# plumer/pbrs

Hardware: AMD Instinct MI355X
Metric: Msamples/s (higher is better)
Workload: dtype f32

## Files before the change

include/pbrs_gpu.h:

```cpp
#ifndef PBRS_GPU_H
#define PBRS_GPU_H

#include <stdint.h>

#ifdef __cplusplus
extern "C" {
#endif

#define PBRS_OK 0
#define PBRS_E_INVALID (-1)
#define PBRS_E_DEVICE (-2)
#define PBRS_E_NO_SCENE (-3)
#define PBRS_E_LIMIT (-4)

#define PBRS_LEAF_FLAG 0x80000000u
#define PBRS_TLAS_LEAF_KIND_SHIFT 8

typedef struct pbrs_node {
    float min[3];
    uint32_t a;
    float max[3];
    uint32_t b;
} pbrs_node;

// ... 97 lines not shown
} pbrs_area_light;

typedef struct pbrs_delta_light {
    uint32_t kind;
    float v[3];
    float color[3];
    float world_radius;
} pbrs_delta_light;

typedef struct pbrs_scene_desc {
    uint32_t n_tlas_nodes;
    const pbrs_node* tlas_nodes;
    uint32_t tlas_height;
    uint32_t n_instances;
    const pbrs_instance* instances;
    uint32_t n_shapes;
    const pbrs_shape* shapes;
    uint32_t n_meshes;
    const pbrs_mesh* meshes;
    uint32_t n_blas_nodes;
    const pbrs_node* blas_nodes;
    uint32_t n_triangles;
    const pbrs_tri_verts* tri_verts;
    const pbrs_tri_shade* tri_shade;
    uint32_t n_materials;
    const pbrs_material* materials;
    uint32_t n_bxdfs;
    const pbrs_bxdf* bxdfs;
    uint32_t n_area_lights;
    const pbrs_area_light* area_lights;
    uint32_t n_delta_lights;
    const pbrs_delta_light* delta_lights;
    float env_constant[3];
    uint32_t env_kind;
    uint32_t n_textures;
    const pbrs_texture* textures;
    uint32_t n_tex_floats;
    const float* tex_floats;
    uint32_t n_tex_words;
    const uint32_t* tex_words;
    uint32_t env_texture;
    float env_scale[3];
    uint32_t n_fourier_tables;
    const pbrs_fourier_table* fourier_tables;
} pbrs_scene_desc;

typedef struct pbrs_camera {
    float center[3];
    uint32_t width;
    float c[3];
    uint32_t height;
    float a[3];
    float pad0;
    float b[3];
    float pad1;
} pbrs_camera;

typedef struct pbrs_stats {
    uint64_t samples;
    uint64_t closest_rays;
    uint64_t shadow_rays;
    uint64_t shade_events;
    uint64_t tlas_nodes, blas_nodes, instances, instance_hits, triangles, tri_shading;
    uint64_t spheres, quads, cuboids, disks;
    uint64_t shadow_tlas_nodes, shadow_blas_nodes, shadow_instances, shadow_triangles, shadow_prims;
    uint64_t invalid_samples;
    float ms_raygen, ms_extend, ms_shade, ms_shadow, ms_accumulate, ms_total;
    uint32_t launches_extend, launches_shadow, launches_shade, passes;
    uint32_t kernel_features_extend, kernel_features_shadow;
    uint64_t paths_at_bounce[16];
    uint64_t shadow_rays_at_bounce[16];
} pbrs_stats;
#define PBRS_STATS_MAX_BOUNCES 16

typedef struct pbrs_ctx pbrs_ctx;

int pbrs_create(int device_ordinal, pbrs_ctx** out);
void pbrs_destroy(pbrs_ctx*);
const char* pbrs_last_error(const pbrs_ctx*);
int pbrs_set_stream(pbrs_ctx*, void* hip_stream);

int pbrs_set_pass_overlap(pbrs_ctx*, int enabled);

int pbrs_upload_scene(pbrs_ctx*, const pbrs_scene_desc*);

typedef struct pbrs_render_params {
    uint32_t x0, y0, w, h;
    uint32_t strata_x, strata_y;
    uint32_t max_depth;
    uint32_t samples_per_pass;
    uint64_t seed;
    uint32_t collect_counters;
    uint32_t time_stages;
    uint32_t band_rows, band_count, band_index;
    uint32_t integrator;
} pbrs_render_params;
#define PBRS_INTEGRATOR_PATH 0u
#define PBRS_INTEGRATOR_DIRECT 1u
#define PBRS_INTEGRATOR_MATERIALS 2u
#define PBRS_INTEGRATOR_NORMALS 3u

int pbrs_render_tile(pbrs_ctx*, const pbrs_camera*, const pbrs_render_params*, float* rgb_out_host, pbrs_stats* stats_out);
int pbrs_render_tile_device(pbrs_ctx*, const pbrs_camera*, const pbrs_render_params*, float* rgb_out_device, pbrs_stats* stats_out);
int pbrs_collect_stats(pbrs_ctx*, pbrs_stats* stats_out);

typedef struct pbrs_aov_buffers {
    float* albedo;
    float* normal;
    float* coverage;
    float* depth;
    uint32_t* instance;
    uint32_t* material;
    uint32_t* prim;
} pbrs_aov_buffers;
int pbrs_render_tile_aovs(pbrs_ctx*, const pbrs_camera*, const pbrs_render_params*, float* rgb_out_host, const pbrs_aov_buffers* aovs_host,
                          pbrs_stats* stats_out);
int pbrs_render_tile_aovs_device(pbrs_ctx*, const pbrs_camera*, const pbrs_render_params*, float* rgb_out_device,
                                 const pbrs_aov_buffers* aovs_device, pbrs_stats* stats_out);

enum pbrs_filter_kind { PBRS_FILTER_BOX = 0, PBRS_FILTER_TRIANGLE = 1, PBRS_FILTER_GAUSSIAN = 2, PBRS_FILTER_MITCHELL = 3, PBRS_FILTER_LANCZOS = 4 };
#define PBRS_FILTER_MAX_RADIUS 4.0f
typedef struct pbrs_pixel_filter {
    uint32_t kind;
    float radius[2];
    float a, b;
    uint32_t pad;
} pbrs_pixel_filter;
int pbrs_render_tile_filtered(pbrs_ctx*, const pbrs_camera*, const pbrs_render_params*, const pbrs_pixel_filter*, float* rgb_out_host,
                              pbrs_stats* stats_out);
int pbrs_render_tile_filtered_device(pbrs_ctx*, const pbrs_camera*, const pbrs_render_params*, const pbrs_pixel_filter*,
                                     float* rgb_out_device, pbrs_stats* stats_out);

#define PBRS_DENOISE_MAX_ITERATIONS 6
#define PBRS_DENOISE_DEMODULATE 1u
#define PBRS_DENOISE_ID_STOP 2u
typedef struct pbrs_denoise_params {
    uint32_t w, h;
    uint32_t iterations;
    uint32_t flags;
    float sigma_color, sigma_normal, sigma_depth;
    float albedo_floor;
} pbrs_denoise_params;
typedef struct pbrs_denoise_guides {
    const float* albedo;
    const float* normal;
    const float* depth;
    const uint32_t* instance;
} pbrs_denoise_guides;
int pbrs_denoise(pbrs_ctx*, const pbrs_denoise_params*, const float* rgb_in_host, const pbrs_denoise_guides* guides_host, float* rgb_out_host);
int pbrs_denoise_device(pbrs_ctx*, const pbrs_denoise_params*, const float* rgb_in_device, const pbrs_denoise_guides* guides_device,
                        float* rgb_out_device);

typedef struct pbrs_hit_record {
    float t;
    uint32_t inst;
    uint32_t prim;
    float b1, b2;
} pbrs_hit_record;
int pbrs_intersect_rays(pbrs_ctx*, uint32_t n, const float* origins, const float* dirs, const float* tmax,
                        pbrs_hit_record* hits_out, uint8_t* occluded_out);
typedef struct pbrs_intersect_info {
    uint32_t wide_any, wide_closest;
    uint32_t slow_any, slow_closest;
} pbrs_intersect_info;
int pbrs_last_intersect_info(const pbrs_ctx*, pbrs_intersect_info* out);
int pbrs_camera_rays(pbrs_ctx*, const pbrs_camera*, const pbrs_render_params*, uint32_t sample_index, float* origins_out,
// ... 344 lines not shown
```

pbrs_amd/api.py:

```python
import ctypes as C
import os
from types import SimpleNamespace

import numpy as np

from .abi import (AOV_NAMES, AOVS, BSDF_OPS, BSDF_QUERY_WORDS, BSDF_RESULT_WORDS, DENOISE_GUIDES, HIT_DTYPE, INTEGRATORS, MATTE_LAYERS, NUMERIC_FNS, NUMERIC_K_FNS, PASS_CHANNELS, PASSES,
                  SPATIAL_VARIANCE_PLANES, TEMPORAL_FRAME, TEMPORAL_GUIDES, TEMPORAL_HISTORY, VARIANCE, AovBuffers, BloomParams, Camera, CompareMaps, CompareParams, CompareResult,
                  DenoiseGuides, DenoiseParams, DespeckleIO, DespeckleParams, DespeckleResult, DofParams,
                  DenoiseVarGuides, DenoiseVarParams, DisplayIO, DisplayParams, HistoryClipParams, InstanceMotion, MatteBuffers, MatteParams, MotionBlurParams, Node, PassBuffers,
                  PixelFilter, RenderParams, SceneDesc, SpatialVarianceGuides, SpatialVarianceParams, Stats, TemporalFrame, TemporalGuides, TemporalHistory,
                  TemporalParams, UpsampleParams, _aov_names, _bloom_params, _DenoiseParamsMixin, _despeckle_params, _display_params, _dof_params, _history_clip, _matte_select, _motion_args, _motion_blur_params, _pass_names,
                  _reference_frame, _reference_frames, _temporal_struct, _upscale_params, lens, scaled_camera)
from .devmem import DeviceBuffers
from .libs import GPU_BLOOM_SYMBOLS, GPU_COMPARE_SYMBOLS, GPU_DESPECKLE_SYMBOLS, GPU_DOF_SYMBOLS, GPU_MOTION_BLUR_SYMBOLS, GPU_SYMBOLS, HOST_SYMBOLS, PbrsError, gpu_lib, hip_runtime, host_lib, lib_paths
from .spec import SceneSpec


def orbited(camera, about, axis, degrees):
    k = np.asarray(axis, dtype=np.float64)
    k = k / np.linalg.norm(k)
    t = np.radians(degrees)

    def rot(v):
        return v * np.cos(t) + np.cross(k, v) * np.sin(t) + k * np.dot(k, v) * (1.0 - np.cos(t))
    about = np.asarray(about, dtype=np.float64)
    out = Camera()
    out.width, out.height = camera.width, camera.height
    out.center[:] = [float(v) for v in about + rot(np.array(list(camera.center), dtype=np.float64) - about)]
    for n in ("c", "a", "b"):
        getattr(out, n)[:] = [float(v) for v in rot(np.array(list(getattr(camera, n)), dtype=np.float64))]
    return out


def instance_motion(scene, scene_prev):
    fwd, inv = scene.instance_transforms()
    fwd_p, inv_p = scene_prev.instance_transforms()
    if len(fwd) != len(fwd_p):
        raise ValueError(f"instance_motion: {len(fwd)} instances beside {len(fwd_p)} in the previous scene")
    table = (InstanceMotion * max(len(fwd), 1))()
    bottom = np.array([[0.0, 0.0, 0.0, 1.0]])
    for i in range(len(fwd)):
        r = table[i]
        if fwd[i].tobytes() == fwd_p[i].tobytes() and inv[i].tobytes() == inv_p[i].tobytes():
            m, n, r.flags = np.eye(3, 4), np.eye(3), InstanceMotion.IDENTITY
        else:
            m = (np.vstack([fwd_p[i].astype(np.float64), bottom]) @ np.vstack([inv[i].astype(np.float64), bottom]))[:3]
            n = (fwd[i, :, :3].astype(np.float64) @ inv_p[i, :, :3].astype(np.float64)).T
        for a in range(3):
            r.m[a][:] = [float(v) for v in m[a].astype(np.float32)]
            r.n[a][:] = [float(v) for v in n[a].astype(np.float32)]
    return table


def _guide_bytes(guides, w, h, suffix=""):
    return {n + suffix: DENOISE_GUIDES[n][0] * w * h * 4 for n in guides}


def _sequence_buffers(w, h, fw, fh, guides, motion_vectors, upscale, display, reference=False, despeckle=False, bloom=False, dof=False,
                      motion_blur=False):
    kept = [n for n in TEMPORAL_GUIDES if n in guides]
    sizes = {"rgb": 3 * w * h * 4, "out": 3 * w * h * 4, VARIANCE: w * h * 4, "acc_variance": w * h * 4}
    for k in ("0", "1"):
        sizes.update(_guide_bytes(kept, w, h, k))
        sizes.update({f"h_{n}{k}": ch * w * h * 4 for n, (ch, _) in TEMPORAL_HISTORY.items()})
    sizes.update(_guide_bytes([n for n in guides if n not in kept], w, h))
    if motion_vectors:
        sizes["motion"], sizes["prev_depth"] = 2 * w * h * 4, w * h * 4
    if upscale:
        sizes["up"] = 3 * fw * fh * 4
        sizes.update(_guide_bytes(guides, fw, fh, "_hi"))
    if display:
        sizes["display"], sizes["exposure"] = fw * fh * 4, 4
    if reference:
        sizes["reference"], sizes["compare"] = 3 * fw * fh * 4, C.sizeof(CompareResult)
    if despeckle:
        sizes["despeckled"], sizes["despeckle"] = 3 * w * h * 4, C.sizeof(DespeckleResult)
    if bloom:
        sizes["bloom"] = 3 * fw * fh * 4
    if dof:
        sizes["dof"] = 3 * fw * fh * 4
    if motion_blur:
        sizes["mblur"] = 3 * fw * fh * 4
        if upscale or not motion_vectors:
            sizes["mblur_motion"] = 2 * fw * fh * 4
    return sizes


class LoadedScene:

    def __init__(self, path):
        h = C.c_void_p()
        rc = host_lib().pbrs_host_load_pbrt(os.fsencode(path), C.byref(h))
        if rc != 0:
            raise PbrsError(f"pbrs_host_load_pbrt({path}) failed ({rc}): {host_lib().pbrs_host_load_error().decode()}")
        self._h = h
        self.spec = host_lib().pbrs_loaded_scene_spec(h).contents

# ... 37 lines not shown
    if ch == 3:
        img = np.concatenate([img, np.full((h, w, 1), 255, dtype=np.uint8)], axis=2)
    words = np.ascontiguousarray(img).view("<u4")
    rc = host_lib().pbrs_host_write_png_rgba8(os.fsencode(path), words.ctypes.data, w, h)
    if rc != 0:
        raise PbrsError(f"writing {path} failed ({rc}): {host_lib().pbrs_host_io_error().decode()}")


class HostScene:

    def __init__(self, scene_builder):
        self._sb = scene_builder
        self._spec = scene_builder.build()
        h = C.c_void_p()
        rc = host_lib().pbrs_host_scene_build(C.addressof(self._spec), C.byref(h))
        if rc != 0:
            raise PbrsError(f"pbrs_host_scene_build failed ({rc}): {host_lib().pbrs_host_last_error().decode()}")
        self._h = h
        self.desc = host_lib().pbrs_host_scene_desc(h).contents
        self.camera = host_lib().pbrs_host_scene_camera(h).contents
        self.width, self.height = self.camera.width, self.camera.height

    @property
    def stack_depth(self):
        return host_lib().pbrs_host_scene_stack_depth(self._h)

    @property
    def nbytes(self):
        d = self.desc
        return (32 * (d.n_tlas_nodes + d.n_blas_nodes) + 128 * d.n_instances + 48 * d.n_shapes + 32 * d.n_meshes +
                (48 + 64) * d.n_triangles + 32 * d.n_materials + 64 * d.n_bxdfs + 64 * d.n_area_lights + 32 * d.n_delta_lights +
                48 * d.n_textures + 4 * (d.n_tex_floats + d.n_tex_words) + 48 * d.n_fourier_tables)

    def instance_transforms(self):
        n = self.desc.n_instances
        if n == 0 or not self.desc.instances:
            return np.zeros((0, 3, 4), dtype=np.float32), np.zeros((0, 3, 4), dtype=np.float32)
        rec = np.ctypeslib.as_array(C.cast(self.desc.instances, C.POINTER(C.c_float)), shape=(n, 32))
        return rec[:, 12:24].reshape(n, 3, 4).copy(), rec[:, :12].reshape(n, 3, 4).copy()

    def nodes(self, which="tlas"):
        n, p = (self.desc.n_tlas_nodes, self.desc.tlas_nodes) if which == "tlas" else (self.desc.n_blas_nodes, self.desc.blas_nodes)
        if n == 0 or not p:
            return np.zeros((0, 8), dtype=np.uint32)
        return np.ctypeslib.as_array(C.cast(p, C.POINTER(C.c_uint32)), shape=(n, 8)).copy()

    def close(self):
        if getattr(self, "_h", None):
            host_lib().pbrs_host_scene_free(self._h)
            self._h = None

    def __del__(self):
        self.close()


class Context:

    def __init__(self, device=0):
        self._L = gpu_lib()
        h = C.c_void_p()
        rc = self._L.pbrs_create(device, C.byref(h))
        if rc != 0:
            raise PbrsError(f"pbrs_create(device={device}) failed ({rc}): no usable HIP device; there is no CPU fallback")
        self._h = h
        self.scene = None

    def _check(self, rc, what):
        if rc != 0:
            raise PbrsError(f"{what} failed ({rc}): {self._L.pbrs_last_error(self._h).decode()}")

    def close(self):
        if getattr(self, "_h", None):
            self._L.pbrs_destroy(self._h)
            self._h = None

    def __del__(self):
        self.close()

    def set_stream(self, hip_stream_ptr):
        self._check(self._L.pbrs_set_stream(self._h, C.c_void_p(hip_stream_ptr)), "pbrs_set_stream")

    def set_pass_overlap(self, enabled):
        self._check(self._L.pbrs_set_pass_overlap(self._h, int(bool(enabled))), "pbrs_set_pass_overlap")

    def upload(self, host_scene):
        self._check(self._L.pbrs_upload_scene(self._h, C.addressof(host_scene.desc)), "pbrs_upload_scene")
        self.scene = host_scene

    def _params(self, strata_x, strata_y, depth, seed, tile, samples_per_pass=0, counters=False, timing=False, bands=None,
                integrator="path"):
        x0, y0, w, h = tile or (0, 0, self.scene.width, self.scene.height)
        p = RenderParams()
        if bands:
            p.band_rows, p.band_count, p.band_index = bands
        p.x0, p.y0, p.w, p.h = x0, y0, w, h
        p.strata_x, p.strata_y, p.max_depth, p.samples_per_pass = strata_x, strata_y, depth, samples_per_pass
        p.seed, p.collect_counters, p.time_stages = seed, int(counters), int(timing)
        p.integrator = INTEGRATORS[integrator]
        return p

    def render(self, strata_x, strata_y, depth, seed, tile=None, samples_per_pass=0, counters=False, timing=False, bands=None,
               integrator="path"):
        p = self._params(strata_x, strata_y, depth, seed, tile, samples_per_pass, counters, timing, bands, integrator)
        out = np.empty((p.h, p.w, 3), dtype=np.float32)
        st = Stats()
        self._check(self._L.pbrs_render_tile(self._h, C.addressof(self.scene.camera), C.addressof(p), out.ctypes.data, C.addressof(st)),
                    "pbrs_render_tile")
        return out, st.as_dict()

    def render_device(self, rgb_device_ptr, strata_x, strata_y, depth, seed, tile=None, samples_per_pass=0, counters=False,
                      timing=False, bands=None, integrator="path"):
        p = self._params(strata_x, strata_y, depth, seed, tile, samples_per_pass, counters, timing, bands, integrator)
        self._check(self._L.pbrs_render_tile_device(self._h, C.addressof(self.scene.camera), C.addressof(p), C.c_void_p(rgb_device_ptr), None),
                    "pbrs_render_tile_device")

    @staticmethod
    def _aov_arrays(names, p):
        bufs, arrays = AovBuffers(), {}
        for n in names:
            ch, dt = AOVS.get(n, (1, np.float32))
            arrays[n] = np.empty((p.h, p.w, ch) if ch > 1 else (p.h, p.w), dtype=dt)
            if n != VARIANCE:
                setattr(bufs, n, arrays[n].ctypes.data)
        return bufs, arrays

    @staticmethod
    def _aov_device(aov_device_ptrs):
        ptrs = dict(aov_device_ptrs or {})
        _aov_names(ptrs)
        variance = ptrs.pop(VARIANCE, None)
        bufs = AovBuffers()
        for n, ptr in ptrs.items():
            setattr(bufs, n, ptr)
        return bufs, variance

    def _render_host(self, p, names, mp=None, mb=None, pb=None, camera=None):
        out = np.empty((p.h, p.w, 3), dtype=np.float32)
        bufs, arrays = self._aov_arrays(names, p)
        st = Stats()
        self._check(self._L.pbrs_render_tile_passes(self._h, C.addressof(camera or self.scene.camera), C.addressof(p), out.ctypes.data, C.addressof(bufs),
                                                    arrays[VARIANCE].ctypes.data if VARIANCE in names else None, C.addressof(mp) if mp else None,
                                                    C.addressof(mb) if mb else None, C.addressof(pb) if pb else None, C.addressof(st)),
                    "pbrs_render_tile_passes")
        return out, arrays, st.as_dict()

    def _render_device(self, p, rgb_device_ptr, bufs, variance, mp=None, mb=None, pb=None, camera=None):
        self._check(self._L.pbrs_render_tile_passes_device(self._h, C.addressof(camera or self.scene.camera), C.addressof(p), C.c_void_p(rgb_device_ptr),
                                                           C.addressof(bufs), C.c_void_p(variance), C.addressof(mp) if mp else None,
                                                           C.addressof(mb) if mb else None, C.addressof(pb) if pb else None, None),
                    "pbrs_render_tile_passes_device")

    def render_aovs(self, strata_x, strata_y, depth, seed, aovs=AOV_NAMES, tile=None, samples_per_pass=0, counters=False,
                    timing=False, bands=None, integrator="path", camera=None):
        names = _aov_names(aovs)
        return self._render_host(self._params(strata_x, strata_y, depth, seed, tile, samples_per_pass, counters, timing, bands, integrator), names,
                                 camera=camera)

    def render_aovs_device(self, rgb_device_ptr, aov_device_ptrs, strata_x, strata_y, depth, seed, tile=None, samples_per_pass=0,
                           counters=False, timing=False, bands=None, integrator="path"):
        bufs, variance = self._aov_device(aov_device_ptrs)
        self._render_device(self._params(strata_x, strata_y, depth, seed, tile, samples_per_pass, counters, timing, bands, integrator),
                            rgb_device_ptr, bufs, variance)

    def render_aovs_var_device(self, rgb_device_ptr, aov_device_ptrs, variance_device_ptr, strata_x, strata_y, depth, seed, tile=None,
                               samples_per_pass=0, counters=False, timing=False, bands=None, integrator="path"):
        unknown = [n for n in aov_device_ptrs if n not in AOVS]
# ... 780 lines not shown
```

pbrs_amd/csrc/device/extend.h:

```cpp
#pragma once
#include "path_state.h"
#include "traverse.h"

template <bool STATS>
PD void flush_counters(const Cnt<STATS>& cnt, GlobalCounters* g, bool valid, uint32_t rays, uint32_t hits) {
    if (!STATS) return;
    const WorkCounters& c = cnt.c;
    uint32_t v[12] = {c.tlas_nodes, c.blas_nodes, c.instances, c.instance_hits, c.triangles, c.tri_shading,
                      c.spheres,    c.quads,      c.cuboids,   c.disks,         rays,        hits};
    unsigned long long* out = reinterpret_cast<unsigned long long*>(g);
    for (int k = 0; k < 12; ++k) {
        uint32_t x = valid ? v[k] : 0u;
        for (int off = 32; off > 0; off >>= 1) x += __shfl_down(x, off, 64);
        if ((threadIdx.x & 63u) == 0 && x) atomicAdd(out + k, (unsigned long long)x);
    }
}

#ifndef PBRS_NODE_STEPS_LONG
#define PBRS_NODE_STEPS_LONG 3u
#endif
#ifndef PBRS_CHUNK_MAX
#define PBRS_CHUNK_MAX 512u
#endif
#ifndef PBRS_TRAV_WAVES
// ... 76 lines not shown
    const uint32_t want = (uint32_t)__popcll(mask), rank = lane_prefix(mask);
    const uint32_t avail = w.end - w.cur;
    uint32_t idx = (need && rank < avail) ? w.cur + rank : 0xffffffffu;
    if (want <= avail) {
        w.cur += want;
        return idx;
    }
    w.cur = w.end;
    const int leader = __ffsll((unsigned long long)mask) - 1;
    while (w.tried < PBRS_WORK_HEADS) {
        const uint32_t seg_lo = work_segment(n, w.head), seg_hi = work_segment(n, w.head + 1);
        uint32_t base = 0;
        if ((int)(threadIdx.x & 63u) == leader) base = atomicAdd(heads + w.head * PBRS_WORK_HEAD_STRIDE, w.chunk);
        base = __shfl(base, leader, 64);
        const uint32_t len = seg_hi - seg_lo;
        const uint32_t lo = seg_lo + (base < len ? base : len), hi = seg_lo + (base + w.chunk < len ? base + w.chunk : len);
        if (base + w.chunk >= len) {
            w.head = (w.head + 1u) % PBRS_WORK_HEADS;
            w.tried++;
        }
        if (lo == hi) continue;
        const uint32_t rest = want - avail, got = hi - lo;
        if (need && rank >= avail && rank - avail < got) idx = lo + (rank - avail);
        w.cur = lo + (rest < got ? rest : got);
        w.end = hi;
        break;
    }
    return idx;
}
PD void wave_append_slow(bool slow, uint32_t item, uint32_t* list, uint32_t* count) {
    const uint64_t m = __ballot(slow);
    if (m == 0) return;
    const int leader = __ffsll((unsigned long long)m) - 1;
    uint32_t base = 0;
    if ((int)(threadIdx.x & 63u) == leader) base = atomicAdd(count, (uint32_t)__popcll(m));
    base = __shfl(base, leader, 64);
    if (slow) list[base + lane_prefix(m)] = item;
}
#ifndef PBRS_WIDE_SHADOW_WAVES
#define PBRS_WIDE_SHADOW_WAVES 5
#endif
#ifndef PBRS_WIDE_NODE_STEPS
#define PBRS_WIDE_NODE_STEPS 2u
#endif
template <uint32_t ARITY, bool STATS, uint32_t FEAT>
struct AnySel {
    typedef AnyWalkW<FEAT> type;
};
template <bool STATS, uint32_t FEAT>
struct AnySel<0u, STATS, FEAT> {
    typedef AnyWalk<STATS, (FEAT & (PBRS_FEAT_ALL | PBRS_FEAT_LDS_TOP)), !STATS && !(FEAT & PBRS_FEAT_FLAT_TLAS)> type;
};
#define PBRS_WALK_ARITY(STATS, FEAT) ((STATS) ? 0u : ((FEAT) & PBRS_FEAT_WIDE) ? 4u : 0u)
#ifndef PBRS_NODE_STEPS_SHORT
#define PBRS_NODE_STEPS_SHORT 1u
#endif
#define PBRS_WALK_NSTEPS(FEAT, ARITY) \
    (!((FEAT) & PBRS_FEAT_LONG_WALKS) ? ((ARITY) == 0u ? PBRS_NODE_STEPS_SHORT : 1u) : (ARITY) == 4u ? PBRS_WIDE_NODE_STEPS : PBRS_NODE_STEPS_LONG)
PD DevScene stage_scene(const DevScene& G, uint32_t* lds_base) {
    DevScene S = G;
    uint4* dst = reinterpret_cast<uint4*>(__builtin_assume_aligned(lds_base + G.lds_off_words, 16));
    S.nodes = reinterpret_cast<const pbrs_node*>(dst);
    dst = stage_array(dst, G.nodes, G.lds_nodes * (uint32_t)(sizeof(pbrs_node) / 16));
    S.tv = reinterpret_cast<const pbrs_tri_verts*>(dst);
    dst = stage_array(dst, G.tv, G.lds_tris * (uint32_t)(sizeof(pbrs_tri_verts) / 16));
    S.inst = reinterpret_cast<const pbrs_instance*>(dst);
    dst = stage_array(dst, G.inst, G.lds_inst * (uint32_t)(sizeof(pbrs_instance) / 16));
    S.shapes = reinterpret_cast<const pbrs_shape*>(dst);
    stage_array(dst, G.shapes, G.lds_shapes * (uint32_t)(sizeof(pbrs_shape) / 16));
    __syncthreads();
    return S;
}
static_assert(sizeof(pbrs_node) % 16 == 0 && sizeof(pbrs_tri_verts) % 16 == 0 && sizeof(pbrs_instance) % 16 == 0 && sizeof(pbrs_shape) % 16 == 0, "stage_scene copies 16-byte pieces");

PD DevScene stage_top(const DevScene& G, uint32_t* lds_base) {
    DevScene S = G;
    uint4* dst = reinterpret_cast<uint4*>(__builtin_assume_aligned(lds_base + G.lds_off_words, 16));
    S.nodes_top = reinterpret_cast<const pbrs_node*>(dst);
    stage_array(dst, G.nodes, G.lds_nodes * (uint32_t)(sizeof(pbrs_node) / 16));
    __syncthreads();
    return S;
}

template <bool STATS, uint32_t FEAT>
__global__ void __launch_bounds__(256, STATS ? 3 : (FEAT & PBRS_FEAT_SHADING_CHECK) ? PBRS_TRAV_WAVES : PBRS_LEAN_EXTEND_WAVES)
    k_extend(DevScene G, PathState st, uint32_t set, const uint32_t* count, uint32_t n_direct, uint32_t* next, GlobalCounters* gc, const uint32_t* indirect,
             uint32_t* slow_list, uint32_t* slow_count, uint32_t split) {
    extern __shared__ __attribute__((aligned(16))) uint32_t lds_stack[];
    const DevScene S = (!STATS && (FEAT & PBRS_FEAT_LDS_SCENE)) ? stage_scene(G, lds_stack) : (!STATS && (FEAT & PBRS_FEAT_LDS_TOP)) ? stage_top(G, lds_stack) : G;
    const uint32_t n = count ? *count : n_direct;
    const float4* q0 = st.q[set][0];
    const float4* q1 = st.q[set][1];
    LaneStack stk{lds_stack + threadIdx.x, q0, q1, 0u};
    Cnt<STATS> cnt;
    cnt.init();
    uint32_t nrays = 0, nhit = 0;
    ClosestWalk<STATS, (FEAT & (PBRS_FEAT_ALL | PBRS_FEAT_LDS_TOP | PBRS_FEAT_EXTENT))> walk;
    walk.mode = PBRS_WALK_IDLE;
    PBRS_KP_DECL(walk);
    PBRS_TT_DECL;
    uint32_t item = 0;
    WaveWork work = wave_work_init(n);
    for (;;) {
        uint64_t live = __ballot(walk.mode == PBRS_WALK_NODE || walk.mode == PBRS_WALK_LEAF || walk.mode == PBRS_WALK_XFER);
        if ((uint32_t)__popcll(live) < S.refill_below) {
            PBRS_KP_WAVE(1);
            if (walk.mode == PBRS_WALK_DONE) {
                walk.finish(cnt);
                const Hit& h = walk.best;
                nhit += h.inst != 0xffffffffu ? 1u : 0u;
                uint32_t cls = (S.n_classes > 1u && h.inst != 0xffffffffu) ? S.inst[h.inst].pad[0] : 0u;
                if (split) {
                    cls = 1u;
                    if (h.inst == 0xffffffffu) {
                        const bool specular = (item >> 31) != 0u;
                        cls = (specular || ((split & PBRS_QSPLIT_ENV) && S.has_env != 0u)) ? 1u : 0u;
                    }
                }
                const uint32_t pos = item & 0x7fffffffu;
                if (!split || cls) st_stream(&st.hit[pos], make_float4(h.t, __uint_as_float(h.inst), __uint_as_float(h.prim), __uint_as_float(split ? 0u : cls)));
                if (S.n_classes > 1u || split) st.cls[pos] = (uint8_t)cls;
                walk.mode = PBRS_WALK_IDLE;
            }
            if (work.left()) {
                uint32_t idx = wave_fetch(work, walk.mode == PBRS_WALK_IDLE, next, n);
                if (idx != 0xffffffffu) {
                    if (indirect) idx = indirect[idx];
                    stk.item = idx;
                    const float4 a = q0[idx], b = q1[idx];
                    item = idx | (__float_as_uint(a.w) & 0x80000000u);
                    walk.start(S, xyz(a), xyz(b), pn_inf(), stk);
                    nrays++;
                    PBRS_KP_LANE(2, true);
                }
                walk.scan_wave(S, cnt);
                live = __ballot(walk.mode == PBRS_WALK_NODE || walk.mode == PBRS_WALK_LEAF || walk.mode == PBRS_WALK_XFER);
            }
            if (live == 0) break;
        }
        PBRS_TT(0);
        PBRS_STEP_WALK(walk, S, stk, cnt, PBRS_EXT_XFER_MIN, PBRS_EXT_LEAF_MIN, PBRS_WALK_NSTEPS(FEAT, 0u), ((FEAT & PBRS_FEAT_FULL_STEPS) != 0u));
    }
    flush_counters<STATS>(cnt, gc, true, nrays, nhit);
    if (!STATS) PBRS_KP_FLUSH(0, walk);
    if (!STATS) PBRS_TT_FLUSH(0);
}
```

pbrs_amd/csrc/device/path_state.h:

```cpp
#pragma once
#include "shapes.h"

struct PathState {
    float4* q[2][3];
    float4* hit;
    uint8_t* cls;
    uint32_t* perm;
    uint32_t* tile_hist;
    uint2* class_range;
    float4* L;
    float4* sr[3];
    float4* nee[3];
    uint8_t* occ[2];
};

struct RenderConst {
    pbrs_camera cam;
    uint32_t x0, y0, w, h;
    uint32_t strata_x, strata_y;
    uint32_t max_depth;
    uint32_t pass_first_sample;
    uint32_t n_pixels;
    uint32_t n_slots;
    uint32_t chunk_pixels;
    uint32_t tiles8_per_row;
    uint32_t band_rows, band_count, band_index;
    uint32_t integrator;
    uint64_t seed;
};

template <class T>
PD T& at(T* base, uint32_t slot) {
    static_assert(sizeof(T) == 4 || sizeof(T) == 1, "column element size");
    return *reinterpret_cast<T*>(reinterpret_cast<char*>(base) + (size_t)(uint32_t)(slot * (uint32_t)sizeof(T)));
}
PD float4 pack4(f3 v, uint32_t w) { return make_float4(v.x, v.y, v.z, __uint_as_float(w)); }
PD float4 pack4(f3 v, float w) { return make_float4(v.x, v.y, v.z, w); }
PD f3 xyz(float4 v) { return mk3(v.x, v.y, v.z); }
#define PBRS_SLOT_MASK 0x3fffffffu
PD float4 ld_stream(const float4* p) {
    const pbrs_f4v v = __builtin_nontemporal_load(reinterpret_cast<const pbrs_f4v*>(p));
    return make_float4(v.x, v.y, v.z, v.w);
}
PD void st_stream(float4* p, float4 v) {
    pbrs_f4v w;
    w.x = v.x, w.y = v.y, w.z = v.z, w.w = v.w;
    __builtin_nontemporal_store(w, reinterpret_cast<pbrs_f4v*>(p));
}

PD void sample_of_slot(uint32_t slot, uint32_t n_pixels, uint32_t k_count, uint32_t chunk, uint32_t& k, uint32_t& pix) {
    const uint32_t per_chunk = chunk * k_count;
    const uint32_t c = slot / per_chunk, rem = slot - c * per_chunk, first = c * chunk;
    const uint32_t size = n_pixels - first < chunk ? n_pixels - first : chunk;
    k = rem / size;
    pix = first + (rem - k * size);
}
PD uint32_t slot_of_sample(uint32_t k, uint32_t pix, uint32_t n_pixels, uint32_t k_count, uint32_t chunk) {
    const uint32_t c = pix / chunk, first = c * chunk;
    const uint32_t size = n_pixels - first < chunk ? n_pixels - first : chunk;
    return c * chunk * k_count + k * size + (pix - first);
}

PD uint32_t pixel_of_order(uint32_t q, uint32_t w, uint32_t tiles8_per_row) {
    if (tiles8_per_row == 0u) return q;
    const uint32_t t = q >> 6, r = q & 63u;
    const uint32_t ty = t / tiles8_per_row, tx = t - ty * tiles8_per_row;
    return (ty * 8u + (r >> 3)) * w + tx * 8u + (r & 7u);
}
PD uint32_t order_of_pixel(uint32_t pix, uint32_t w, uint32_t tiles8_per_row) {
    if (tiles8_per_row == 0u) return pix;
    const uint32_t y = pix / w, x = pix - y * w;
    return (((y >> 3) * tiles8_per_row + (x >> 3)) << 6) + ((y & 7u) << 3) + (x & 7u);
}

struct GlobalCounters {
    unsigned long long tlas_nodes, blas_nodes, instances, instance_hits, triangles, tri_shading, spheres, quads, cuboids, disks, rays, hits;
};

PD uint4* stage_array(uint4* dst, const void* src_, uint32_t n16) {
    const uint4* src = reinterpret_cast<const uint4*>(src_);
    for (uint32_t i = threadIdx.x; i < n16; i += PBRS_TRAVERSAL_BLOCK) dst[i] = src[i];
    return dst + n16;
}
```

pbrs_amd/csrc/device/raygen.h:

```cpp
#pragma once
#include "path_state.h"

__global__ void __launch_bounds__(256) k_raygen(PathState st, RenderConst rc, uint32_t* rng_hi0) {
    uint32_t slot = blockIdx.x * blockDim.x + threadIdx.x;
    if (slot >= rc.n_slots) return;
    uint32_t k, pix;
    sample_of_slot(slot, rc.n_pixels, rc.n_slots / rc.n_pixels, rc.chunk_pixels, k, pix);
    pix = pixel_of_order(pix, rc.w, rc.tiles8_per_row);
    uint32_t col = rc.x0 + pix % rc.w, vrow = pix / rc.w;
    uint32_t row = rc.y0 + (rc.band_count > 1 ? ((vrow / rc.band_rows) * rc.band_count + rc.band_index) * rc.band_rows + vrow % rc.band_rows : vrow);
    uint32_t i = rc.pass_first_sample + k;
    uint64_t rng = pn_rng_init(rc.seed, row * rc.cam.width + col, i);
    float r0 = pn_rng_f32(&rng), r1 = pn_rng_f32(&rng);
    float jx = ((float)(i / rc.strata_y) + r0) / (float)rc.strata_x;
    float jy = ((float)(i % rc.strata_y) + r1) / (float)rc.strata_y;
    if (rc.integrator >= PBRS_INTEGRATOR_MATERIALS) jx = jy = 0.0f;
    float x = (float)col + pn_fract(jx);
    float y = (float)row + pn_fract(jy);
    f3 dir = ld3(rc.cam.c) + ld3(rc.cam.a) * x + ld3(rc.cam.b) * y;
    st_stream(&st.q[0][0][slot], pack4(ld3(rc.cam.center), slot));
    st_stream(&st.q[0][1][slot], pack4(dir, (uint32_t)rng));
    __builtin_nontemporal_store((uint32_t)(rng >> 32), &rng_hi0[slot]);
}
```

pbrs_amd/csrc/device/scene.h:

```cpp
#pragma once
#include <stddef.h>
#include <stdint.h>

#include "../../../include/pbrs_gpu.h"

constexpr uint32_t kBlock = 256;
constexpr size_t kLdsBytesPerCU = 160 * 1024;

struct pbrs_wnode;
struct DevScene {
    const pbrs_node* nodes;
    const pbrs_instance* inst;
    const pbrs_shape* shapes;
    const pbrs_mesh* meshes;
    const pbrs_tri_verts* tv;
    const pbrs_tri_shade* ts;
    const pbrs_material* mats;
    const pbrs_bxdf* bxdfs;
    const pbrs_area_light* alights;
    const pbrs_delta_light* dlights;
    uint32_t n_area, n_delta;
    float env[3];
    uint32_t has_env;
    uint32_t fast_slab;
    uint32_t exact_extent;
    uint32_t flat_off, n_flat;
    uint32_t features;
    uint32_t refill_below;
    uint32_t refill_below_shadow;
    const pbrs_texture* textures;
    const float* tex_floats;
    const uint32_t* tex_words;
    uint32_t env_kind, env_texture;
    float env_scale[3];
    const pbrs_fourier_table* fourier;
    uint32_t n_classes;
    const pbrs_wnode* wnodes;
    uint32_t wide_cap;
    uint32_t lds_off_words, lds_nodes, lds_tris, lds_inst, lds_shapes;
    const pbrs_node* nodes_top;
    uint32_t n_inst, n_shapes, n_tris, n_mats, n_bxdfs;
    uint32_t n_wnodes;
};

#define PBRS_INSTANCE_TRANSLATION 0x100u
#define PBRS_FEAT_ANALYTIC 1u
#define PBRS_FEAT_SHADING_CHECK 2u
#define PBRS_FEAT_FLAT_TLAS 4u
#define PBRS_FEAT_ALL 7u
#define PBRS_FEAT_EXTENT 256u
#define PBRS_FEAT_LONG_WALKS 8u
#define PBRS_FEAT_WIDE 16u
#define PBRS_FEAT_LDS_TOP 128u
#define PBRS_FEAT_LDS_SCENE 64u
#define PBRS_FEAT_FULL_STEPS 32u
#define PBRS_SKIP_INST_MASK 0x00ffffffu
#define PBRS_SKIP_FLAT_SHIFT 24
#define PBRS_FLAT_TLAS_MIN 2u
#ifndef PBRS_FLAT_TLAS_MAX
#define PBRS_FLAT_TLAS_MAX 20u
#endif
#ifndef PBRS_FLAT_TLAS_MAX_ANYHIT
#define PBRS_FLAT_TLAS_MAX_ANYHIT 32u
#endif

struct pbrs_wnode {
    float lo[3][4];
    float hi[3][4];
    uint32_t child[4];
    uint32_t pad[4];
};
#ifndef PBRS_WIDE_STACK_MAX
#define PBRS_WIDE_STACK_MAX 16
#endif
#ifndef PBRS_WIDE_MIN_LEVELS
#define PBRS_WIDE_MIN_LEVELS 4u
#endif
#define PBRS_WREF_LEAF 0x80000000u
#define PBRS_WREF_NONE 0xffffffffu
#define PBRS_WREF_INDEX 0x07ffffffu
#define PBRS_WREF_AXIS_SHIFT 27
#define PBRS_WREF_PACKED 0x04000000u
#define PBRS_WREF_TRI_BITS 24
#define PBRS_WREF_TRI 0x00ffffffu
#define PBRS_WREF_COUNT_SHIFT 24
#define PBRS_WREF_COUNT_MAX 4u
static_assert((PBRS_WREF_PACKED & PBRS_WREF_INDEX) == PBRS_WREF_PACKED && PBRS_WREF_PACKED < (1u << PBRS_WREF_AXIS_SHIFT), "the packed flag lies inside the index bits, below the axes");
static_assert(PBRS_WREF_TRI == (1u << PBRS_WREF_TRI_BITS) - 1u && PBRS_WREF_COUNT_SHIFT == PBRS_WREF_TRI_BITS, "first triangle: the low bits, the count above them");
static_assert(((PBRS_WREF_COUNT_MAX - 1u) << PBRS_WREF_COUNT_SHIFT) < PBRS_WREF_PACKED && (PBRS_WREF_PACKED >> PBRS_WREF_COUNT_SHIFT) == PBRS_WREF_COUNT_MAX,
              "two bits of count - 1 between the triangle index and the flag");
static_assert((PBRS_WREF_PACKED | ((PBRS_WREF_COUNT_MAX - 1u) << PBRS_WREF_COUNT_SHIFT) | PBRS_WREF_TRI) == PBRS_WREF_INDEX, "flag, count and triangle fill the 27 bits exactly");
static_assert(PBRS_WREF_TRI_BITS >= 24, "a mesh of 2^24 triangles (indices 0 .. 2^24 - 1) packs");
static_assert((PBRS_WREF_LEAF | PBRS_WREF_INDEX | (15u << PBRS_WREF_AXIS_SHIFT)) == 0xffffffffu && PBRS_WREF_LEAF == (1u << 31), "leaf bit, four axis bits, 27 index bits");
#define PBRS_WIDE_UNUSED_PLANE 1152921504606846976.0f

#ifndef PBRS_REFILL_BELOW_SHORT
#define PBRS_REFILL_BELOW_SHORT 20u
#endif
#ifndef PBRS_REFILL_BELOW_LONG
#define PBRS_REFILL_BELOW_LONG 48u
#endif
#ifndef PBRS_REFILL_BELOW_LONG_SHADOW
#define PBRS_REFILL_BELOW_LONG_SHADOW 40u
#endif
#define PBRS_LONG_WALK_HEIGHT 12u

#define PBRS_SHADE_LAMBERT 1u
#define PBRS_SHADE_LIGHT_SPHERE 2u
#define PBRS_SHADE_LIGHT_TRIANGLE 4u
#define PBRS_SHADE_FOURIER 8u
#define PBRS_SHADE_FOURIER_ONLY 16u
#define PBRS_SHADE_LDS_RECORDS 32u
// ... 12 lines not shown
```

pbrs_amd/csrc/device/traverse.h:

```cpp
#pragma once
#include "shapes.h"

#include "probes.h"

struct RaySpace {
    f3 o, d;
    f3 nr;
    bool fast;
};
PD uint32_t dir_in_range(float x) {
    uint32_t e = (pn_bits(x) >> 23) & 0xffu;
    return (e - (127u - 40u) <= 80u) ? 1u : 0u;
}
PD uint32_t origin_in_range(float x) {
    uint32_t u = pn_bits(x) & 0x7fffffffu;
    uint32_t e = u >> 23;
    return ((u == 0u) | (e - (127u - 60u) <= 100u)) ? 1u : 0u;
}
PD RaySpace make_space(f3 o, f3 d, bool scene_ok) {
    RaySpace r;
    r.o = o;
    r.d = d;
    r.fast = ((scene_ok ? 1u : 0u) & dir_in_range(d.x) & dir_in_range(d.y) & dir_in_range(d.z) & origin_in_range(o.x) &
              origin_in_range(o.y) & origin_in_range(o.z)) != 0u;
    r.nr = gray(0.0f);
    if (r.fast) r.nr = mk3(-(1.0f / d.x), -(1.0f / d.y), -(1.0f / d.z));
    return r;
}
PD RaySpace reload_world(const DevScene& S, LaneStack stk) {
    const float4 a = stk.ro[stk.item], b = stk.rd[stk.item];
    return make_space(mk3(a.x, a.y, a.z), mk3(b.x, b.y, b.z), S.fast_slab != 0);
}
#define PBRS_SPACE_WORLD 0u
#define PBRS_SPACE_MOVED 1u
#define PBRS_SPACE_TRANSLATED 2u
PD void leave_instance(const DevScene& S, LaneStack stk, uint32_t moved, RaySpace& C) {
    if (moved == PBRS_SPACE_TRANSLATED && C.fast) {
        const float4 a = stk.ro[stk.item];
        C.o = mk3(a.x, a.y, a.z);
    } else if (moved != PBRS_SPACE_WORLD) {
        C = reload_world(S, stk);
    }
}
PD bool slab_rs(const pbrs_node& n, const RaySpace& R, float t_max, float& t_low, float& hi_el) {
    if (!R.fast) return slab_test(nmin(n), nmax(n), R.o, R.d, t_max);
    float t0x = qdiv(R.o.x - n.min[0], R.d.x, R.nr.x), t0y = qdiv(R.o.y - n.min[1], R.d.y, R.nr.y), t0z = qdiv(R.o.z - n.min[2], R.d.z, R.nr.z);
    float t1x = qdiv(R.o.x - n.max[0], R.d.x, R.nr.x), t1y = qdiv(R.o.y - n.max[1], R.d.y, R.nr.y), t1z = qdiv(R.o.z - n.max[2], R.d.z, R.nr.z);
    float lo_el = __builtin_fmaxf(__builtin_fmaxf(__builtin_fminf(t0x, t1x), __builtin_fminf(t0y, t1y)), __builtin_fminf(t0z, t1z));
    hi_el = __builtin_fminf(__builtin_fminf(__builtin_fmaxf(t0x, t1x), __builtin_fmaxf(t0y, t1y)), __builtin_fmaxf(t0z, t1z));
    t_low = __builtin_fmaxf(lo_el, 0.0f);
    float t_high = __builtin_fminf(hi_el, t_max);
    return t_low <= t_high;
}
PD bool slab_rs(const pbrs_node& n, const RaySpace& R, float t_max) {
    float t_low = 0.0f, hi_el = 0.0f;
    return slab_rs(n, R, t_max, t_low, hi_el);
}
#include "split_planes.h"
#include "wide.h"

struct InstHead {
    uint32_t flags, blas_root, mesh_flags, wide_root;
};
static_assert(offsetof(pbrs_instance, flags) == 108 && offsetof(pbrs_instance, blas_root) == 112 && offsetof(pbrs_instance, mesh_flags) == 116 &&
                  offsetof(pbrs_instance, pad) == 120 && sizeof(pbrs_instance) == 128 && alignof(pbrs_instance) <= 16,
              "pbrs_instance layout (load_inst_head, wide root in pad[1], shading class in pad[0])");
static_assert(sizeof(pbrs_node) == 32 && offsetof(pbrs_node, a) == 12 && offsetof(pbrs_node, max) == 16 && offsetof(pbrs_node, b) == 28, "pbrs_node layout (load_node)");
static_assert(sizeof(pbrs_wnode) == 128 && offsetof(pbrs_wnode, hi) == 48 && offsetof(pbrs_wnode, child) == 96, "pbrs_wnode layout (wide_test)");
static_assert(sizeof(pbrs_tri_verts) == 48, "pbrs_tri_verts layout (load_tri)");
PD InstHead load_inst_head(const pbrs_instance& in) {
    uint32_t f = in.flags;
    uint4 r = *reinterpret_cast<const uint4*>(&in.blas_root);
    asm volatile("" : "+v"(f), "+v"(r.x), "+v"(r.y), "+v"(r.w));
    return {f, r.x, r.y, r.w};
}
PD uint32_t enter_instance(const DevScene& S, const pbrs_instance& in, uint32_t in_flags, RaySpace& C, bool need_slab, LaneStack stk) {
    if ((in_flags & PBRS_INSTANCE_IDENTITY) && C.fast && C.o.x != 0.0f && C.o.y != 0.0f && C.o.z != 0.0f) return PBRS_SPACE_WORLD;
    f3 oo = xf_apply(in.inv, C.o, 1.0f);
    if (need_slab && (in_flags & PBRS_INSTANCE_TRANSLATION) && C.fast) {
        C.o = oo;
        if (!(origin_in_range(oo.x) & origin_in_range(oo.y) & origin_in_range(oo.z))) {
            C.fast = false;
            C.nr = gray(0.0f);
        }
// ... 51 lines not shown
    PD uint32_t k() const { return (tag >> 8) & 3u; }
    PD uint32_t pos(uint32_t j) const { return off[j] + lane_prefix(has[j]); }
    PD uint32_t from_owner(uint32_t v) const { return (uint32_t)__builtin_amdgcn_ds_bpermute((int)(tag << 2), (int)v); }
    PD float from_owner(float v) const { return __uint_as_float(from_owner(__float_as_uint(v))); }
    PD f3 from_owner(f3 v) const { return mk3(from_owner(v.x), from_owner(v.y), from_owner(v.z)); }
    PD float from_helper(uint32_t at, float v) const {
        return __uint_as_float((uint32_t)__builtin_amdgcn_ds_bpermute((int)(at << 2), (int)__float_as_uint(v)));
    }
};

struct FlatScan {
    PD static uint32_t pull(uint32_t from, uint32_t v) { return (uint32_t)__builtin_amdgcn_ds_bpermute((int)(from << 2), (int)v); }
    PD static float pull(uint32_t from, float v) { return __uint_as_float(pull(from, __float_as_uint(v))); }
    struct Exact {
        RaySpace O;
        float t;
        PD Exact(const RaySpace& R, float t_max) : O(R), t(t_max) {}
        PD Exact from(uint32_t owner) const {
            Exact y = *this;
            y.O.o = mk3(pull(owner, O.o.x), pull(owner, O.o.y), pull(owner, O.o.z));
            y.O.d = mk3(pull(owner, O.d.x), pull(owner, O.d.y), pull(owner, O.d.z));
            y.O.nr = mk3(pull(owner, O.nr.x), pull(owner, O.nr.y), pull(owner, O.nr.z));
            y.O.fast = true;
            y.t = pull(owner, t);
            return y;
        }
        PD bool test(const pbrs_node& n) const { return slab_rs(n, O, t); }
    };
    struct Filter {
        f3 o, r;
        PD Filter(const RaySpace& R, float) : o(R.o), r(-R.nr) {}
        PD Filter from(uint32_t owner) const {
            Filter y = *this;
            y.o = mk3(pull(owner, o.x), pull(owner, o.y), pull(owner, o.z));
            y.r = mk3(pull(owner, r.x), pull(owner, r.y), pull(owner, r.z));
            return y;
        }
        PD bool test(const pbrs_node& n) const {
            return pn_slab_filter(r.x > 0.0f ? n.min[0] : n.max[0], r.y > 0.0f ? n.min[1] : n.max[1], r.z > 0.0f ? n.min[2] : n.max[2],
                                  r.x > 0.0f ? n.max[0] : n.min[0], r.y > 0.0f ? n.max[1] : n.min[1], r.z > 0.0f ? n.max[2] : n.min[2], o.x, o.y, o.z,
                                  r.x, r.y, r.z, pn_inf()) != 0;
        }
    };
    template <class Ray>
    PD static uint32_t scan(const DevScene& S, bool fresh, const RaySpace& R, float t_max, uint32_t& tested) {
        const uint64_t m = __ballot(fresh);
        if (m == 0) return 0u;
        const uint32_t lane = threadIdx.x & 63u;
        const uint32_t H = (S.n_flat + 1u) >> 1;
        const uint32_t total = (uint32_t)__popcll(m) * H;
        const uint32_t rank = lane_prefix(m);
        const uint32_t list = (uint32_t)__builtin_amdgcn_ds_permute((int)((fresh ? rank : 63u) << 2), (int)lane);
        const uint32_t magic = (65536u + H - 1u) / H;
        const Ray mine_ray(R, t_max);
        uint32_t mine = 0;
        for (uint32_t base = 0; base < total; base += 64u) {
            const uint32_t p = base + lane;
            const bool valid = p < total;
            const uint32_t r = (p * magic) >> 16, h = p - r * H;
            const Ray O = mine_ray.from(pull(r, list));
            bool pass0 = false, pass1 = false;
            if (valid) {
                pass0 = O.test(load_node(S.nodes + S.flat_off + h));
                tested += 1u;
                if (h + H < S.n_flat) {
                    pass1 = O.test(load_node(S.nodes + S.flat_off + h + H));
                    tested += 1u;
                }
            }
            const uint64_t w0 = __ballot(pass0), w1 = __ballot(pass1);
            const int sft = (int)(rank * H) - (int)base;
            if (fresh && sft > -(int)H && sft < 64) {
                const uint64_t a = sft >= 0 ? w0 >> sft : w0 << -sft, b = sft >= 0 ? w1 >> sft : w1 << -sft;
                const uint32_t keep = (1u << H) - 1u;
                mine |= ((uint32_t)a & keep) | (((uint32_t)b & keep) << H);
            }
        }
        return mine;
    }
    PD static uint32_t run(const DevScene& S, bool fresh, const RaySpace& R, float t_max, uint32_t& tested) { return scan<Exact>(S, fresh, R, t_max, tested); }
    PD static uint32_t run_filter(const DevScene& S, bool fresh, const RaySpace& R, uint32_t& tested) { return scan<Filter>(S, fresh, R, pn_inf(), tested); }
};

template <bool STATS, uint32_t FEAT>
struct ClosestWalk {
    RaySpace C;
    Hit best;
    float t_max, lt, mt, mb1, mb2;
    uint32_t mprim, cur_inst;
    uint32_t inst_info;
    uint32_t leaf_a, leaf_end;
    int sp, blas_base;
    uint32_t cand;
    bool in_blas, moved;
    uint32_t mode;
    static constexpr bool EXT = (FEAT & PBRS_FEAT_EXTENT) != 0u;
    float win;
    bool win_has;
    PBRS_TP_FIELDS

    PD void start(const DevScene& S, f3 o, f3 d, float tmax, LaneStack stk) {
        C = make_space(o, d, S.fast_slab != 0);
        win = 0.0f;
        win_has = false;
        moved = false;
        best.t = pn_inf();
        best.inst = 0xffffffffu;
        best.prim = 0;
        best.b1 = best.b2 = 0.0f;
        in_blas = false;
        t_max = tmax;
        lt = tmax;
        mt = pn_inf();
        mprim = cur_inst = inst_info = leaf_a = leaf_end = 0;
        mb1 = mb2 = 0.0f;
        blas_base = 0;
        cand = 0;
        if ((FEAT & PBRS_FEAT_FLAT_TLAS) && !EXT && S.n_flat != 0u && C.fast) {
            sp = 0;
            mode = PBRS_WALK_SCAN;
        } else {
            stk.put(0, 0u);
            sp = 1;
            mode = PBRS_WALK_NODE;
        }
    }
    PD void scan_wave(const DevScene& S, Cnt<STATS>& cnt) {
        if (!(FEAT & PBRS_FEAT_FLAT_TLAS) || EXT) return;
        uint32_t tested = 0;
        const uint32_t mine = FlatScan::run_filter(S, mode == PBRS_WALK_SCAN, C, tested);
        if (STATS) cnt.c.tlas_nodes += tested;
        if (mode == PBRS_WALK_SCAN) {
            cand = mine;
            mode = PBRS_WALK_NODE;
        }
    }

    static constexpr bool CULL = PBRS_SPLIT_PLANE_CULL != 0 && !STATS && !EXT && !(FEAT & PBRS_FEAT_LDS_TOP);
    PD uint32_t cull_children(const pbrs_node& X, float dk, float t_low, float hi_el) const {
        const int k = (int)(X.b & 3u);
        const float lo = comp(nmin(X), k), hi = comp(nmax(X), k);
        const float step = pbrs_plane_step(lo, hi);
        const float pd = pbrs_plane_down(pbrs_plane_qd(X.b), step, lo), pu = pbrs_plane_up(pbrs_plane_qu(X.b), step, hi);
        const bool pos = dk > 0.0f;
        const float ok = comp(C.o, k), nrk = comp(C.nr, k);
        const float e_near = qdiv(ok - (pos ? pu : pd), dk, nrk), e_far = qdiv(ok - (pos ? pd : pu), dk, nrk);
        const float T = __builtin_fminf(hi_el, mt);
        return (e_near < t_low ? 0u : 1u) | (e_far > T ? 0u : 2u);
    }
    PD void push_children(LaneStack stk, bool left_first, uint32_t left, uint32_t right, uint32_t keep) {
        const uint32_t far = left_first ? right : left, near = left_first ? left : right;
        if constexpr (!CULL) {
            stk.put(sp++, far);
            stk.put(sp++, near);
        } else {
            stk.put(sp, far);
            sp += (int)(keep >> 1);
            stk.put(sp, near);
            sp += (int)(keep & 1u);
        }
    }

    PD void node_step(const DevScene& S, LaneStack stk, Cnt<STATS>& cnt) {
        PBRS_TP(0);
        if (in_blas && sp == blas_base) {
            mode = exit_mode();
            return;
        }
// ... 78 lines not shown
        float t_low = 0.0f, hi_el = 0.0f;
        if (!slab_rs(node, F, lt, t_low, hi_el)) {
            PBRS_TP(2);
            return;
        }
        if (!(node.b & PBRS_LEAF_FLAG)) {
            const float dk = comp(C.d, (int)(node.b & 3u));
            bool left_first = !in_blas || dk > 0.0f;
            uint32_t left = ni + 1, right = node.a;
            uint32_t keep = 3u;
            if constexpr (CULL) {
                if (in_blas) keep = cull_children(node, dk, t_low, hi_el);
            }
            push_children(stk, left_first, left, right, keep);
            lt = in_blas ? mt : lt;
        } else if (in_blas) {
            PBRS_TP(3);
            PBRS_TP(4);
            leaf_a = node.a;
            leaf_end = node.a + (node.b & ~PBRS_LEAF_FLAG);
            if (leaf_end != leaf_a) mode = PBRS_WALK_LEAF;
            else lt = mt;
        } else {
            cur_inst = node.a;
            inst_info = (node.b >> PBRS_TLAS_LEAF_KIND_SHIFT) & 7u;
            mode = PBRS_WALK_XFER;
        }
    }

    PD void meet_best(Cnt<STATS>& cnt) {
        if (mt < pn_inf() || (inst_info & 0x80000000u)) {
            CNT(instance_hits);
            if constexpr (EXT) {
                if (!win_has || !(win < mt)) win = mt;
                win_has = true;
            }
            if (!(best.t < mt)) {
                best.t = mt;
                best.inst = cur_inst;
                best.prim = mprim;
                best.b1 = mb1;
                best.b2 = mb2;
                if constexpr (!EXT) t_max = mt;
            }
        }
    }
    PD uint32_t exit_mode() const {
        const bool nothing_above = blas_base == 0 && (!(FEAT & PBRS_FEAT_FLAT_TLAS) || cand == 0u);
        return nothing_above ? PBRS_WALK_DONE : PBRS_WALK_XFER;
    }
    PD void finish(Cnt<STATS>& cnt) {
        if (in_blas) {
            in_blas = false;
            meet_best(cnt);
        }
    }
    PD void xfer_step(const DevScene& S, LaneStack stk, Cnt<STATS>& cnt) {
        mode = PBRS_WALK_NODE;
        if (in_blas) {
            PBRS_TP(7);
            in_blas = false;
            leave_instance(S, stk, !moved ? PBRS_SPACE_WORLD : (inst_info & 0x40000000u) ? PBRS_SPACE_TRANSLATED : PBRS_SPACE_MOVED, C);
            meet_best(cnt);
            lt = t_max;
            return;
        }
        const pbrs_instance& in = S.inst[cur_inst];
        CNT(instances);
        PBRS_TP(6);
        const uint32_t kind = inst_info;
        if ((FEAT & PBRS_FEAT_ANALYTIC) && kind != PBRS_SHAPE_MESH && kind != PBRS_SHAPE_TRIANGLE) {
            analytic_visit(S, in, kind, cnt);
            return;
        }
        const InstHead H = load_inst_head(in);
        const uint32_t space = enter_instance(S, in, H.flags, C, kind == PBRS_SHAPE_MESH, stk);
        moved = space != PBRS_SPACE_WORLD;
        in_blas = true;
        blas_base = sp;
        lt = t_max;
        mt = pn_inf();
        if (kind == PBRS_SHAPE_MESH) {
            inst_info = kind | (H.mesh_flags << 3) | (space == PBRS_SPACE_TRANSLATED ? 0x40000000u : 0u);
            stk.put(sp++, H.blas_root);
        } else if (kind == PBRS_SHAPE_TRIANGLE) {
            inst_info = kind | (PBRS_MESH_SHADING_OK_MASK << 3);
            leaf_a = H.blas_root;
            leaf_end = H.blas_root + 1u;
            mode = PBRS_WALK_LEAF;
        }
    }

    PD void analytic_visit(const DevScene& S, const pbrs_instance& in, uint32_t kind, Cnt<STATS>& cnt) {
        if (!(FEAT & PBRS_FEAT_ANALYTIC)) return;
        const f3 o = xf_apply(in.inv, C.o, 1.0f), d = xf_apply(in.inv, C.d, 0.0f);
        const float ext = t_max;
        const float* p = S.shapes[in.shape_index].p;
        float t = 0.0f, b1 = 0.0f, b2 = 0.0f;
        bool hit = false;
        switch (kind) {
            case PBRS_SHAPE_SPHERE:
                CNT(spheres);
                hit = sphere_hit_t(ld3(p), p[3], o, d, ext, t);
                break;
            case PBRS_SHAPE_QUAD: {
                CNT(quads);
                float u, v;
                f3 n;
                hit = quad_hit(ld3(p), ld3(p + 3), ld3(p + 6), o, d, ext, t, u, v, n);
                break;
            }
            case PBRS_SHAPE_CUBOID: {
                CNT(cuboids);
                int axis;
                float bound;
                hit = cuboid_hit(ld3(p), ld3(p + 3), o, d, ext, t, axis, bound);
                break;
            }
            case PBRS_SHAPE_DISK:
                CNT(disks);
                hit = disk_hit_t(ld3(p), ld3(p + 3), ld3(p + 6), o, d, ext, t);
                break;
            default:
                break;
        }
        inst_info = kind | (hit ? 0x80000000u : 0u);
        mt = hit ? t : pn_inf();
        mprim = 0;
        mb1 = b1;
        mb2 = b2;
        meet_best(cnt);
        lt = t_max;
    }

    PD void leaf_wave(const DevScene& S, Cnt<STATS>& cnt) {
        const bool tri_leaf = mode == PBRS_WALK_LEAF;
        TriShare sh;
        sh.build(tri_leaf ? leaf_end - leaf_a : 0u);
        if (sh.has[0] == 0) return;
        const f3 ho = sh.from_owner(C.o), hd = sh.from_owner(C.d);
        const float hlt = sh.from_owner(lt);
        const uint32_t hti = sh.from_owner(leaf_a) + sh.k();
        const uint32_t hinfo = (STATS || (FEAT & PBRS_FEAT_SHADING_CHECK)) ? sh.from_owner(inst_info) : 0u;
        const float hmt = (FEAT & PBRS_FEAT_SHADING_CHECK) ? sh.from_owner(mt) : 0.0f;
        float rt = pn_inf(), rb1 = 0.0f, rb2 = 0.0f;
        if (sh.helper()) {
            PBRS_TP(5);
            pbrs_tri_verts tv = load_tri(S.tv + hti);
            CNT(triangles);
            TriHit h;
            constexpr bool need_bary = STATS || (FEAT & PBRS_FEAT_SHADING_CHECK) != 0u;
            bool hit = mesh_tri_hit_t<need_bary>(tv, ho, hd, hlt, S.fast_slab != 0u, h);
            if (hit && (hinfo & 7u) == PBRS_SHAPE_MESH) CNT(tri_shading);
            if ((FEAT & PBRS_FEAT_SHADING_CHECK) && hit && h.t < hmt && !((hinfo >> 3) & PBRS_MESH_SHADING_OK_MASK)) {
                f3 n, dpdu;
                hit = mesh_tri_shading(tv, S.ts[hti], hd, h, n, dpdu);
            }
            if (hit) {
                rt = h.t;
                rb1 = h.b1;
                rb2 = h.b2;
            }
        }
        uint32_t win = 0xffffffffu, win_tri = 0;
#pragma unroll
        for (uint32_t j = 0; j < 4u; ++j) {
// ... 440 lines not shown
```

pbrs_amd/csrc/host/kernel_choice.cpp:

```cpp
#include "kernel_choice.h"

#include <algorithm>

namespace pbrs {

KernelChoice choose_kernels(const SceneFacts& f, const DevOverrides& dev) {
    KernelChoice p;
    const bool long_walks = dev.long_walks.value_or(f.long_walks);
    const bool full_steps = dev.full_steps.value_or(f.full_steps);
    const uint32_t steps = long_walks ? PBRS_FEAT_LONG_WALKS | (full_steps ? PBRS_FEAT_FULL_STEPS : 0u) : 0u;
    p.wide_shadow = f.tlas_scanned && f.wide_ok && dev.wide_shadow;
    const bool lds_scene = dev.lds_scene && !p.wide_shadow && !full_steps && f.stack_bytes + f.scene_bytes <= kLdsBytesPerCU / 8;
    const bool lds_top = dev.lds_top && !lds_scene && !f.tlas_scanned && !full_steps && f.stack_bytes + f.top_bytes + 512 <= kLdsBytesPerCU / 7;
    p.lds_staging = lds_scene ? PBRS_FEAT_LDS_SCENE : lds_top ? PBRS_FEAT_LDS_TOP : 0u;
    const size_t stack = std::max(f.stack_bytes, dev.lds_min);
    const size_t staged = stack + (lds_scene ? f.scene_bytes : lds_top ? f.top_bytes : 0u);
    if (f.exact_extent) {
        p.extend[0] = {kExtentFeatures, stack};
        p.extend[1] = {kStatsKey | kExtentFeatures, stack};
    } else {
        p.extend[0] = {(f.features & PBRS_FEAT_ALL) | steps | p.lds_staging, staged};
        p.extend[1] = {kStatsKey | PBRS_FEAT_ALL, stack};
    }
    const uint32_t shadow_feat = (f.features & PBRS_FEAT_ANALYTIC) | (f.tlas_scanned ? PBRS_FEAT_FLAT_TLAS : 0u) | steps;
    if (p.wide_shadow) {
        p.shadow[0] = {shadow_feat | PBRS_FEAT_WIDE, f.wide_stack_bytes};
        p.shadow_slow = {shadow_feat, stack};
    } else {
        p.shadow[0] = {shadow_feat | p.lds_staging, staged};
    }
    p.shadow[1] = {kStatsKey | kShadowStatsFeatures, stack};
    p.split_queue = f.n_classes <= 1u && dev.split_queue;

    const uint32_t shade_lds = f.shade_lds & dev.shade_lds;
    const uint32_t path_lds = (shade_lds == PBRS_SHADE_LDS_ALL || shade_lds == PBRS_SHADE_LDS_RECORDS) ? shade_lds : 0u;
    const size_t path_lds_bytes = path_lds == PBRS_SHADE_LDS_ALL ? f.shade_rec_bytes + f.shade_tri_bytes : path_lds ? f.shade_rec_bytes : 0u;
    uint32_t spec = f.lambert ? (PBRS_SHADE_LAMBERT | f.light_spec) & dev.shade_spec : 0u;
    if (!(spec & PBRS_SHADE_LAMBERT)) spec = 0u;
    auto shade = [](IntegratorChoice& ip, uint32_t integ, bool tex, uint32_t sp, size_t lds, uint32_t range) {
        ip.shade[ip.n_shade++] = ShadeKey{integ, tex, sp, lds, range};
    };
    auto path_untextured = [&](IntegratorChoice& ip, uint32_t sp, uint32_t range) { shade(ip, PBRS_INTEGRATOR_PATH, false, sp | path_lds, path_lds_bytes, range); };
    const bool sorted = f.n_classes > 1u && dev.sort_classes;
    for (uint32_t i = PBRS_INTEGRATOR_PATH; i <= PBRS_INTEGRATOR_DIRECT; ++i) {
        IntegratorChoice& ip = p.integ[i];
        const bool path = i == PBRS_INTEGRATOR_PATH;
        const bool split = sorted && path && f.lambert_class && dev.split_lambert && !f.textured && !f.fourier;
        const bool fsplit = sorted && f.fourier && f.fourier_class && dev.split_fourier;
        ip.order = (split || fsplit) ? IntegratorChoice::CLASS_MAJOR : sorted ? IntegratorChoice::CLASS_SORT : IntegratorChoice::NO_ORDER;
        ip.last_class = split ? f.lambert_class : fsplit ? f.fourier_class : 0u;
        if (fsplit) {
            shade(ip, i, false, PBRS_SHADE_FOURIER_ALONE, 0, f.fourier_class);
            shade(ip, i, f.textured, 0u, 0, PBRS_MAX_CLASSES);
        } else if (f.fourier && f.fourier_class && f.n_classes == 1u) {
            shade(ip, i, false, PBRS_SHADE_FOURIER_ALONE, 0, 0u);
        } else if (f.fourier) {
            shade(ip, i, true, PBRS_SHADE_FOURIER, 0, 0u);
        } else if (f.textured) {
            shade(ip, i, true, 0u, 0, 0u);
        } else if (!path) {
            shade(ip, i, false, 0u, 0, 0u);
        } else if (split) {
            path_untextured(ip, PBRS_SHADE_LAMBERT | f.light_spec, f.lambert_class);
            path_untextured(ip, 0u, PBRS_MAX_CLASSES);
        } else {
            path_untextured(ip, spec, 0u);
        }
    }
    shade(p.integ[PBRS_INTEGRATOR_MATERIALS], PBRS_INTEGRATOR_MATERIALS, false, 0u, 0, 0u);
    shade(p.integ[PBRS_INTEGRATOR_NORMALS], PBRS_INTEGRATOR_NORMALS, false, 0u, 0, 0u);
    return p;
}

}
```

pbrs_amd/csrc/host/kernel_choice.h:

```cpp
#pragma once
#include <cstddef>
#include <cstdint>
#include <optional>

#include "../device/scene.h"

namespace pbrs {

struct DevOverrides {
    bool overlap_passes = true;
    bool sort_classes = true;
    bool split_lambert = true;
    bool split_fourier = true;
    bool split_queue = true;
    bool wide_shadow = true;
    bool lds_scene = true;
    bool lds_top = true;
    bool raygen_tiles8 = true;
    uint32_t shade_spec = ~0u;
    uint32_t shade_lds = ~0u;
    std::optional<bool> long_walks, full_steps;
    std::optional<uint32_t> overlap_from, refill_below;
    std::optional<uint32_t> raygen_chunk;
    size_t lds_min = 0;
};

struct SceneFacts {
    uint32_t features = 0;
    bool tlas_scanned = false;
    bool exact_extent = false;
    bool long_walks = false;
    bool full_steps = false;
    bool wide_ok = false;
    size_t stack_bytes = 0;
    size_t wide_stack_bytes = 0;
    size_t scene_bytes = 0;
    size_t top_bytes = 0;
    uint32_t n_classes = 0;
    uint32_t lambert_class = 0;
    uint32_t fourier_class = 0;
    bool textured = false;
    bool fourier = false;
    bool lambert = false;
    uint32_t light_spec = 0;
    uint32_t shade_lds = 0;
    size_t shade_rec_bytes = 0, shade_tri_bytes = 0;
};

constexpr uint32_t kStatsKey = 512u;
constexpr uint32_t kTraversalKeys = 2u * kStatsKey;
constexpr uint32_t kExtentFeatures = PBRS_FEAT_ANALYTIC | PBRS_FEAT_SHADING_CHECK | PBRS_FEAT_EXTENT;
constexpr uint32_t kShadowStatsFeatures = PBRS_FEAT_ANALYTIC | PBRS_FEAT_FLAT_TLAS;
constexpr bool extend_key_ok(uint32_t k) {
    const uint32_t f = k & ~kStatsKey;
    if (f & PBRS_FEAT_EXTENT) return f == kExtentFeatures;
    if (k & kStatsKey) return f == PBRS_FEAT_ALL;
    if (f & PBRS_FEAT_WIDE) return false;
    if ((f & PBRS_FEAT_FULL_STEPS) && !(f & PBRS_FEAT_LONG_WALKS)) return false;
    if ((f & PBRS_FEAT_LDS_SCENE) && (f & PBRS_FEAT_FULL_STEPS)) return false;
    if ((f & PBRS_FEAT_LDS_TOP) && (f & (PBRS_FEAT_LDS_SCENE | PBRS_FEAT_FULL_STEPS | PBRS_FEAT_FLAT_TLAS))) return false;
    return true;
}
constexpr bool shadow_key_ok(uint32_t k) {
    const uint32_t f = k & ~kStatsKey;
    if (k & kStatsKey) return f == kShadowStatsFeatures;
    if (f & (PBRS_FEAT_SHADING_CHECK | PBRS_FEAT_EXTENT)) return false;
    if ((f & PBRS_FEAT_FULL_STEPS) && !(f & PBRS_FEAT_LONG_WALKS)) return false;
    if ((f & PBRS_FEAT_LDS_SCENE) && (f & (PBRS_FEAT_WIDE | PBRS_FEAT_FULL_STEPS))) return false;
    if ((f & PBRS_FEAT_LDS_TOP) && (f & (PBRS_FEAT_LDS_SCENE | PBRS_FEAT_WIDE | PBRS_FEAT_FULL_STEPS | PBRS_FEAT_FLAT_TLAS))) return false;
    if ((f & PBRS_FEAT_WIDE) && !(f & PBRS_FEAT_FLAT_TLAS)) return false;
    return true;
}

#define PBRS_SHADE_LDS_ALL (PBRS_SHADE_LDS_RECORDS | PBRS_SHADE_LDS_TRIS)
#define PBRS_SHADE_FOURIER_ALONE (PBRS_SHADE_FOURIER | PBRS_SHADE_FOURIER_ONLY)
#define PBRS_SHADE_KERNELS(X)                                                                                                            \
                                                                                         \
    X(PBRS_INTEGRATOR_PATH, false, 0u)                                                                                                   \
    X(PBRS_INTEGRATOR_PATH, false, PBRS_SHADE_LAMBERT)                                                                                   \
    X(PBRS_INTEGRATOR_PATH, false, PBRS_SHADE_LAMBERT | PBRS_SHADE_LIGHT_SPHERE)                                                         \
    X(PBRS_INTEGRATOR_PATH, false, PBRS_SHADE_LAMBERT | PBRS_SHADE_LIGHT_TRIANGLE)                                                       \
    X(PBRS_INTEGRATOR_PATH, false, PBRS_SHADE_LDS_RECORDS)                                                                               \
    X(PBRS_INTEGRATOR_PATH, false, PBRS_SHADE_LDS_RECORDS | PBRS_SHADE_LAMBERT)                                                          \
    X(PBRS_INTEGRATOR_PATH, false, PBRS_SHADE_LDS_RECORDS | PBRS_SHADE_LAMBERT | PBRS_SHADE_LIGHT_SPHERE)                                \
    X(PBRS_INTEGRATOR_PATH, false, PBRS_SHADE_LDS_RECORDS | PBRS_SHADE_LAMBERT | PBRS_SHADE_LIGHT_TRIANGLE)                              \
    X(PBRS_INTEGRATOR_PATH, false, PBRS_SHADE_LDS_ALL)                                                                                   \
    X(PBRS_INTEGRATOR_PATH, false, PBRS_SHADE_LDS_ALL | PBRS_SHADE_LAMBERT)                                                              \
    X(PBRS_INTEGRATOR_PATH, false, PBRS_SHADE_LDS_ALL | PBRS_SHADE_LAMBERT | PBRS_SHADE_LIGHT_SPHERE)                                    \
    X(PBRS_INTEGRATOR_PATH, false, PBRS_SHADE_LDS_ALL | PBRS_SHADE_LAMBERT | PBRS_SHADE_LIGHT_TRIANGLE)                                  \
                                                                    \
    X(PBRS_INTEGRATOR_PATH, true, 0u)                                                                                                    \
    X(PBRS_INTEGRATOR_PATH, true, PBRS_SHADE_FOURIER)                                                                                    \
    X(PBRS_INTEGRATOR_PATH, false, PBRS_SHADE_FOURIER_ALONE)                                                                             \
    X(PBRS_INTEGRATOR_DIRECT, false, 0u)                                                                                                 \
    X(PBRS_INTEGRATOR_DIRECT, true, 0u)                                                                                                  \
    X(PBRS_INTEGRATOR_DIRECT, true, PBRS_SHADE_FOURIER)                                                                                  \
    X(PBRS_INTEGRATOR_DIRECT, false, PBRS_SHADE_FOURIER_ALONE)                                                                           \
                                                                                                                   \
    X(PBRS_INTEGRATOR_MATERIALS, false, 0u)                                                                                              \
    X(PBRS_INTEGRATOR_NORMALS, false, 0u)

struct TraversalKey {
    uint32_t key = 0;
    size_t lds = 0;
};
struct ShadeKey {
    uint32_t integ = 0;
    bool tex = false;
    uint32_t spec = 0;
    size_t lds = 0;
    uint32_t range = 0;
};
struct IntegratorChoice {
    enum Order { NO_ORDER, CLASS_SORT, CLASS_MAJOR } order = NO_ORDER;
    uint32_t last_class = 0;
    uint32_t n_shade = 0;
    ShadeKey shade[2];
};
struct KernelChoice {
    TraversalKey extend[2];
    TraversalKey shadow[2];
    bool wide_shadow = false;
    TraversalKey shadow_slow;
    bool split_queue = false;
    uint32_t lds_staging = 0;
    IntegratorChoice integ[PBRS_INTEGRATOR_NORMALS + 1];
};

KernelChoice choose_kernels(const SceneFacts& f, const DevOverrides& dev);

}
```

pbrs_amd/csrc/host/scene_prepare.cpp:

```cpp
#include "scene_prepare.h"

#include <algorithm>
#include <cstring>
#include <map>
#include <string>

#include "../../../include/pbrs_numeric.h"
#include "../../../include/pbrs_scene_spec.h"
#include "../device/split_planes.h"

namespace pbrs {
namespace {

SceneCheck refuse(int code, const char* message) { return SceneCheck{code, message, SceneLevels{}}; }

void tree_heights(const pbrs_node* nodes, uint32_t n, std::vector<uint32_t>& h) {
    h.assign(n, 1u);
    for (uint32_t i = n; i-- > 0;)
        if (!(nodes[i].b & PBRS_LEAF_FLAG)) h[i] = std::max(h[i + 1], h[nodes[i].a]) + 1u;
}

SceneLevels scene_levels(const pbrs_scene_desc& d) {
    SceneLevels l;
    std::vector<uint32_t> th, bh;
    tree_heights(d.tlas_nodes, d.n_tlas_nodes, th);
    tree_heights(d.blas_nodes, d.n_blas_nodes, bh);
    l.tlas = th[0];
    for (uint32_t i = 0; i < d.n_meshes; ++i) l.max_blas = std::max(l.max_blas, bh[d.meshes[i].root]);
    for (uint32_t i = 0; i < d.n_instances; ++i)
        if (d.instances[i].shape_kind == PBRS_SHAPE_MESH) l.max_blas = std::max(l.max_blas, bh[d.instances[i].blas_root]);
    l.stack = std::max(l.tlas, l.tlas - 1u + l.max_blas);
    bool has_quad = false, has_mesh = false;
    for (uint32_t i = 0; i < d.n_instances; ++i) {
        has_quad = has_quad || d.instances[i].shape_kind == PBRS_SHAPE_QUAD;
        has_mesh = has_mesh || d.instances[i].shape_kind == PBRS_SHAPE_MESH;
    }
    l.exact_extent = has_quad && has_mesh;
    if (l.exact_extent) l.stack += l.tlas + 1u;
    return l;
}

bool tlas_scanned(const pbrs_scene_desc& d) { return d.n_instances >= PBRS_FLAT_TLAS_MIN && d.n_instances <= PBRS_FLAT_TLAS_MAX_ANYHIT; }

uint32_t build_wide(const std::vector<pbrs_node>& nodes, uint32_t x, std::vector<pbrs_wnode>& out, uint32_t level, uint32_t& levels) {
    const uint32_t me = (uint32_t)out.size();
    out.push_back(pbrs_wnode{});
    levels = std::max(levels, level + 1u);
    uint32_t slot_node[4] = {0, 0, 0, 0};
    uint32_t used = 0, info = nodes[x].b & 3u;
    const uint32_t child[2] = {x + 1u, nodes[x].a};
    for (uint32_t s = 0; s < 2; ++s) {
        const pbrs_node& ch = nodes[child[s]];
        if (ch.b & PBRS_LEAF_FLAG) {
            slot_node[2 * s] = child[s];
            used |= 1u << (2 * s);
        } else {
            info |= (ch.b & 3u) << (2 + 2 * s);
            slot_node[2 * s] = child[s] + 1u;
            slot_node[2 * s + 1] = ch.a;
            used |= 3u << (2 * s);
        }
    }
    pbrs_wnode w{};
    for (uint32_t k = 0; k < 4; ++k) {
        w.child[k] = PBRS_WREF_NONE;
        if (!((used >> k) & 1u)) {
            for (int a = 0; a < 3; ++a) w.lo[a][k] = PBRS_WIDE_UNUSED_PLANE, w.hi[a][k] = -PBRS_WIDE_UNUSED_PLANE;
            continue;
        }
        const pbrs_node& n = nodes[slot_node[k]];
        for (int a = 0; a < 3; ++a) {
            w.lo[a][k] = n.min[a];
            w.hi[a][k] = n.max[a];
        }
        w.child[k] = (n.b & PBRS_LEAF_FLAG) ? (PBRS_WREF_LEAF | slot_node[k]) : build_wide(nodes, slot_node[k], out, level + 1u, levels);
    }
    w.child[0] |= (info & 15u) << PBRS_WREF_AXIS_SHIFT;
    w.child[2] |= ((info >> 4) & 3u) << PBRS_WREF_AXIS_SHIFT;
    out[me] = w;
    return me;
}

bool coord_ok(float b) {
    const uint32_t u = pn_bits(b) & 0x7fffffffu, e = u >> 23;
    return u == 0u || (e >= 127u - 60u && e <= 127u + 40u);
}

uint32_t split_planes(const std::vector<pbrs_node>& nodes, uint32_t x) {
    const pbrs_node &X = nodes[x], &L = nodes[x + 1u], &R = nodes[X.a];
    for (int a = 0; a < 3; ++a) {
        const bool inside = X.min[a] <= L.min[a] && L.min[a] <= L.max[a] && L.max[a] <= X.max[a] && X.min[a] <= R.min[a] && R.min[a] <= R.max[a] && R.max[a] <= X.max[a];
        if (!inside) return 0u;
    }
    const uint32_t k = X.b & 3u;
    const float lo = X.min[k], hi = X.max[k], step = pbrs_plane_step(lo, hi);
    if (!(step > 0.0f) || !pn_isfinite(step)) return 0u;
    uint32_t qd = 0u, qu = 0u;
    for (uint32_t bit = 1u << (PBRS_PLANE_BITS - 1u); bit; bit >>= 1) {
        if (pbrs_plane_down(qd | bit, step, lo) <= R.min[k]) qd |= bit;
        if (pbrs_plane_up(qu | bit, step, hi) >= L.max[k]) qu |= bit;
    }
    if (!coord_ok(pbrs_plane_down(qd, step, lo))) qd = 0u;
    if (!coord_ok(pbrs_plane_up(qu, step, hi))) qu = 0u;
    return pbrs_plane_pack(qd, qu);
}

bool is_light_instance(const pbrs_scene_desc& d, const pbrs_area_light& L, const pbrs_instance& in) {
    const uint32_t k = L.shape_kind;
    if (!(k == PBRS_SHAPE_SPHERE || k == PBRS_SHAPE_DISK || k == PBRS_SHAPE_QUAD) || in.shape_kind != k || in.shape_index >= d.n_shapes) return false;
    for (int r = 0; r < 3; ++r)
        for (int c = 0; c < 4; ++c) {
            const uint32_t one = pn_bits(r == c ? 1.0f : 0.0f);
            if (pn_bits(in.inv[r][c]) != one || pn_bits(in.fwd[r][c]) != one) return false;
        }
    const float* p = d.shapes[in.shape_index].p;
    for (uint32_t j = 0, n = k == PBRS_SHAPE_SPHERE ? 4u : 9u; j < n; ++j)
        if (pn_bits(p[j]) != pn_bits(L.p[j])) return false;
    return true;
}

}

SceneCheck check_scene(const pbrs_scene_desc& d) {
    if (d.n_tlas_nodes == 0 || d.n_instances == 0) return refuse(PBRS_E_INVALID, "scene without instances");
    for (uint32_t i = 0; i < d.n_tlas_nodes; ++i) {
        const pbrs_node& n = d.tlas_nodes[i];
        if (n.b & PBRS_LEAF_FLAG) {
            if (n.a >= d.n_instances) return refuse(PBRS_E_INVALID, "tlas leaf references a missing instance");
        } else if (n.a >= d.n_tlas_nodes || i + 1 >= d.n_tlas_nodes) {
            return refuse(PBRS_E_INVALID, "tlas child out of range");
        } else if (n.a <= i) {
            return refuse(PBRS_E_INVALID, "tlas nodes are not in pre-order");
        }
    }
    for (uint32_t i = 0; i < d.n_blas_nodes; ++i) {
        const pbrs_node& n = d.blas_nodes[i];
        if (n.b & PBRS_LEAF_FLAG) {
            uint32_t cnt = n.b & ~PBRS_LEAF_FLAG;
            if ((uint64_t)n.a + cnt > d.n_triangles) return refuse(PBRS_E_INVALID, "blas leaf range out of range");
        } else if (n.a >= d.n_blas_nodes || i + 1 >= d.n_blas_nodes || (n.b & 3u) > 2u) {
            return refuse(PBRS_E_INVALID, "blas child out of range");
        } else if (n.a <= i) {
            return refuse(PBRS_E_INVALID, "blas nodes are not in pre-order");
        }
    }
    for (uint32_t i = 0; i < d.n_meshes; ++i)
        if (d.meshes[i].root >= d.n_blas_nodes) return refuse(PBRS_E_INVALID, "mesh root out of range");
    for (uint32_t i = 0; i < d.n_instances; ++i) {
        const pbrs_instance& in = d.instances[i];
        if (in.material >= d.n_materials) return refuse(PBRS_E_INVALID, "instance material out of range");
        if (in.shape_kind > PBRS_SHAPE_MESH) return refuse(PBRS_E_INVALID, "unknown shape kind");
        if (in.shape_kind == PBRS_SHAPE_MESH ? in.shape_index >= d.n_meshes : in.shape_index >= d.n_shapes)
            return refuse(PBRS_E_INVALID, "instance shape out of range");
        if (in.shape_kind == PBRS_SHAPE_MESH ? in.blas_root >= d.n_blas_nodes : (in.shape_kind == PBRS_SHAPE_TRIANGLE && in.blas_root >= d.n_triangles))
            return refuse(PBRS_E_INVALID, "instance blas_root out of range");
    }
    for (uint32_t i = 0; i < d.n_materials; ++i) {
        const pbrs_material& m = d.materials[i];
        if (m.n_bxdfs > PBRS_MAX_BXDFS || (uint64_t)m.first_bxdf + m.n_bxdfs > d.n_bxdfs) return refuse(PBRS_E_INVALID, "material lobes out of range");
        if (m.vis_bxdf > d.n_bxdfs) return refuse(PBRS_E_INVALID, "material visualiser record out of range");
    }
    for (uint32_t i = 0; i < d.n_bxdfs; ++i) {
        const uint32_t t = d.bxdfs[i].tex & ~PBRS_BXDF_TEX_DROP_IF_BLACK;
        if (t > d.n_textures) return refuse(PBRS_E_INVALID, "lobe texture out of range");
        if (d.bxdfs[i].kind > PBRS_BXDF_FOURIER) return refuse(PBRS_E_INVALID, "unknown lobe kind");
        if (d.bxdfs[i].kind == PBRS_BXDF_FOURIER && d.bxdfs[i].intrusion >= d.n_fourier_tables) return refuse(PBRS_E_INVALID, "Fourier lobe table out of range");
    }
    for (uint32_t i = 0; i < d.n_fourier_tables; ++i) {
        const pbrs_fourier_table& t = d.fourier_tables[i];
        const uint64_t n = t.n_mu, nn = n * n, nf = d.n_tex_floats, nw = d.n_tex_words;
        if (n < 3 || (t.n_channels != 1 && t.n_channels != 3)) return refuse(PBRS_E_INVALID, "Fourier table: sizes");
        if (t.mu + n > nf || t.cdf + nn > nf || t.a0 + nn > nf || (uint64_t)t.a + t.n_coeffs > nf || (uint64_t)t.recip + t.m_max > nf ||
            t.a_offset + nn > nw || t.m_lookup + nn > nw)
            return refuse(PBRS_E_INVALID, "Fourier table: arrays out of range");
        for (uint64_t k = 0; k < n; ++k) {
            const float m0 = d.tex_floats[t.mu + k];
            if (!pn_isfinite(m0) || (k + 1 < n && !(m0 < d.tex_floats[t.mu + k + 1]))) return refuse(PBRS_E_INVALID, "Fourier table: mu is not finite and strictly ascending");
        }
        for (uint64_t k = 0; k < nn; ++k) {
            const uint64_t off = d.tex_words[t.a_offset + k], len = d.tex_words[t.m_lookup + k];
            if (len > t.m_max || off + len * t.n_channels > t.n_coeffs) return refuse(PBRS_E_INVALID, "Fourier table: series out of range");
        }
    }
    for (uint32_t i = 0; i < d.n_textures; ++i) {
        const pbrs_texture& t = d.textures[i];
        if (t.kind == PBRS_TEX_PERLIN) {
            if ((uint64_t)t.data + 768 > d.n_tex_floats || (uint64_t)t.perm + 768 > d.n_tex_words) return refuse(PBRS_E_INVALID, "perlin tables out of range");
// ... 67 lines not shown
            if (mt.n_bxdfs == 0) continue;
            std::string sig;
            for (uint32_t k = 0; k < mt.n_bxdfs; ++k) {
                const pbrs_bxdf& bx = d.bxdfs[mt.first_bxdf + k];
                sig += (char)('a' + bx.kind);
                sig += (char)('a' + (bx.kind == PBRS_BXDF_SPECULAR ? bx.intrusion : 0u));
                sig += (char)('a' + (bx.kind == PBRS_BXDF_DIFFUSE ? bx.oren_nayar : bx.fresnel));
                sig += (char)('a' + (bx.kind == PBRS_BXDF_MICROFACET && bx.alpha_x != bx.alpha_y ? 1 : 0));
                sig += bx.tex ? 't' : '-';
            }
            size_t at = 0;
            while (at < sigs.size() && sigs[at] != sig) ++at;
            if (at == sigs.size()) sigs.push_back(sig);
            mat_class[m] = (uint32_t)std::min<size_t>(at + 1, PBRS_MAX_CLASSES - 1);
        }
        S.n_classes = (uint32_t)std::min<size_t>(sigs.size(), PBRS_MAX_CLASSES - 1);
        const std::string lam_sig = {(char)('a' + PBRS_BXDF_DIFFUSE), 'a', 'a', 'a', '-'};
        for (size_t at = 0; at < sigs.size() && at + 1 < PBRS_MAX_CLASSES - 1; ++at)
            if (sigs[at] == lam_sig) f.lambert_class = (uint32_t)at + 1;
        const std::string fou_sig = {(char)('a' + PBRS_BXDF_FOURIER), 'a', 'a', 'a', '-'};
        for (size_t at = 0; at < sigs.size() && at + 1 < PBRS_MAX_CLASSES - 1; ++at)
            if (sigs[at] == fou_sig) f.fourier_class = (uint32_t)at + 1;
    }
    for (pbrs_instance& in : inst) {
        in.pad[0] = mat_class[in.material];
        if (in.shape_kind == PBRS_SHAPE_MESH) in.blas_root += (uint32_t)blas_off;
        bool linear_identity = true;
        for (int r = 0; r < 3; ++r)
            for (int k = 0; k < 3; ++k) linear_identity = linear_identity && pn_bits(in.inv[r][k]) == pn_bits(r == k ? 1.0f : 0.0f);
        in.flags &= ~PBRS_INSTANCE_TRANSLATION;
        if (linear_identity) in.flags |= PBRS_INSTANCE_TRANSLATION;
    }
    for (pbrs_instance& in : inst) in.pad[1] = PBRS_WREF_NONE;
    S.wide_cap = 4u;
    if (scan && S.fast_slab != 0u) {
        std::vector<pbrs_wnode>& wide = P.wide;
        std::map<uint32_t, uint32_t> wide_of_root;
        uint32_t levels = 0;
        for (pbrs_instance& in : inst) {
            if (in.shape_kind != PBRS_SHAPE_MESH || (nodes[in.blas_root].b & PBRS_LEAF_FLAG)) continue;
            auto it = wide_of_root.find(in.blas_root);
            if (it == wide_of_root.end()) it = wide_of_root.emplace(in.blas_root, build_wide(nodes, in.blas_root, wide, 0u, levels)).first;
            in.pad[1] = it->second;
        }
        if (levels >= PBRS_WIDE_MIN_LEVELS && wide.size() * sizeof(pbrs_wnode) < (1ull << 32) && nodes.size() <= PBRS_WREF_PACKED) {
            P.walk_bytes += wide.size() * sizeof(pbrs_wnode);
            P.tri_leaf.assign(d.n_triangles, 0xffffffffu);
            for (size_t i = blas_off; i < nodes.size(); ++i)
                if (nodes[i].b & PBRS_LEAF_FLAG)
                    for (uint32_t t = nodes[i].a, end = t + (nodes[i].b & ~PBRS_LEAF_FLAG); t < end; ++t) P.tri_leaf[t] = (uint32_t)i;
            P.walk_bytes += P.tri_leaf.size() * sizeof(uint32_t);
            S.n_wnodes = (uint32_t)wide.size();
            S.wide_cap = std::max(4u, std::min(3u * levels + 1u, (uint32_t)PBRS_WIDE_STACK_MAX));
            P.wide_levels = levels;
        } else {
            wide.clear();
            for (pbrs_instance& in : inst) in.pad[1] = PBRS_WREF_NONE;
        }
    }

    S.n_area = d.n_area_lights;
    S.n_delta = d.n_delta_lights;
    S.env_kind = d.env_kind;
    S.env_texture = d.env_texture;
    std::memcpy(S.env_scale, d.env_scale, sizeof S.env_scale);
    std::memcpy(S.env, d.env_constant, sizeof S.env);
    S.has_env = (d.env_kind != PBRS_ENV_CONSTANT || !(S.env[0] <= 0.0f && S.env[1] <= 0.0f && S.env[2] <= 0.0f)) ? 1u : 0u;
    S.refill_below = lv.max_blas >= PBRS_LONG_WALK_HEIGHT ? PBRS_REFILL_BELOW_LONG : PBRS_REFILL_BELOW_SHORT;
    S.refill_below_shadow = lv.max_blas >= PBRS_LONG_WALK_HEIGHT ? PBRS_REFILL_BELOW_LONG_SHADOW : PBRS_REFILL_BELOW_SHORT;
    if (dev.refill_below) S.refill_below = S.refill_below_shadow = *dev.refill_below;
    f.long_walks = (S.n_flat ? 0u : lv.tlas) + lv.max_blas >= PBRS_LONG_WALK_HEIGHT;
    f.full_steps = S.fast_slab == 0u;
    f.tlas_scanned = S.n_flat != 0u;
    S.features = (S.n_flat != 0u && d.n_instances <= PBRS_FLAT_TLAS_MAX) ? PBRS_FEAT_FLAT_TLAS : 0u;
    f.wide_ok = S.fast_slab != 0u && P.wide_levels >= PBRS_WIDE_MIN_LEVELS;
    for (uint32_t i = 0; i < d.n_instances; ++i) {
        const pbrs_instance& in = d.instances[i];
        if (in.shape_kind == PBRS_SHAPE_MESH) {
            if (!(in.mesh_flags & PBRS_MESH_SHADING_OK_MASK)) S.features |= PBRS_FEAT_SHADING_CHECK;
        } else if (in.shape_kind != PBRS_SHAPE_TRIANGLE) {
            S.features |= PBRS_FEAT_ANALYTIC;
        }
    }
    f.features = S.features;
    f.exact_extent = lv.exact_extent;
    f.n_classes = S.n_classes;
    P.has_vis_records = d.n_materials > 0;
    for (uint32_t i = 0; i < d.n_materials; ++i) P.has_vis_records = P.has_vis_records && d.materials[i].vis_bxdf != 0;
    for (uint32_t i = 0; i < d.n_bxdfs; ++i) {
        f.textured = f.textured || (d.bxdfs[i].tex & ~PBRS_BXDF_TEX_DROP_IF_BLACK) != 0;
        f.fourier = f.fourier || d.bxdfs[i].kind == PBRS_BXDF_FOURIER;
    }
    f.lambert = !f.textured;
    for (uint32_t i = 0; i < d.n_materials && f.lambert; ++i) {
        const pbrs_material& m = d.materials[i];
        f.lambert = m.n_bxdfs <= 1;
        for (uint32_t k = 0; k < m.n_bxdfs && f.lambert; ++k) {
            const pbrs_bxdf& bx = d.bxdfs[m.first_bxdf + k];
            f.lambert = bx.kind == PBRS_BXDF_DIFFUSE && bx.oren_nayar == 0 && bx.tex == 0;
        }
    }
    if (d.n_area_lights) {
        const uint32_t k0 = d.area_lights[0].shape_kind;
        bool same = true;
        for (uint32_t i = 1; i < d.n_area_lights; ++i) same = same && d.area_lights[i].shape_kind == k0;
        if (same && k0 == PBRS_SHAPE_SPHERE) f.light_spec = PBRS_SHADE_LIGHT_SPHERE;
        if (same && k0 == PBRS_SHAPE_TRIANGLE) f.light_spec = PBRS_SHADE_LIGHT_TRIANGLE;
    }
    P.light_link.assign(d.n_area_lights, 0u);
    for (uint32_t l = 0; l < d.n_area_lights; ++l)
        for (uint32_t i = 0; i < d.n_instances && i + 1u <= PBRS_SKIP_INST_MASK; ++i) {
            if (!is_light_instance(d, d.area_lights[l], d.instances[i])) continue;
            uint32_t leaf = 0u;
            for (uint32_t k = S.n_flat; k-- > 0u;)
                if (nodes[S.flat_off + k].a == i) leaf = k + 1u;
            P.light_link[l] = (i + 1u) | leaf << PBRS_SKIP_FLAT_SHIFT;
            break;
        }
    f.stack_bytes = (size_t)lv.stack * kBlock * sizeof(uint32_t);
    f.wide_stack_bytes = (size_t)S.wide_cap * kBlock * sizeof(uint32_t);
    f.scene_bytes = nodes.size() * sizeof(pbrs_node) + (size_t)d.n_triangles * sizeof(pbrs_tri_verts) + (size_t)d.n_instances * sizeof(pbrs_instance) +
                    (size_t)d.n_shapes * sizeof(pbrs_shape);
    f.top_bytes = (size_t)d.n_tlas_nodes * sizeof(pbrs_node);
    S.n_inst = d.n_instances; S.n_shapes = d.n_shapes; S.n_tris = d.n_triangles; S.n_mats = d.n_materials; S.n_bxdfs = d.n_bxdfs;
    f.shade_rec_bytes = (size_t)d.n_instances * sizeof(pbrs_instance) + (size_t)d.n_shapes * sizeof(pbrs_shape) + (size_t)d.n_materials * sizeof(pbrs_material) +
                        (size_t)d.n_bxdfs * sizeof(pbrs_bxdf) + (size_t)d.n_area_lights * sizeof(pbrs_area_light) + (size_t)d.n_delta_lights * sizeof(pbrs_delta_light);
    f.shade_tri_bytes = (size_t)d.n_triangles * (sizeof(pbrs_tri_verts) + sizeof(pbrs_tri_shade));
    const size_t budget = 16u << 10;
    f.shade_lds = f.shade_rec_bytes + f.shade_tri_bytes <= budget ? PBRS_SHADE_LDS_ALL : f.shade_rec_bytes <= budget ? PBRS_SHADE_LDS_RECORDS : 0u;
    return P;
}

uint32_t pack_wide_leaves(PreparedScene& P) {
    uint32_t packed = 0;
    for (pbrs_wnode& w : P.wide)
        for (uint32_t k = 0; k < 4; ++k) {
            const uint32_t ref = w.child[k];
            if (ref == PBRS_WREF_NONE || !(ref & PBRS_WREF_LEAF)) continue;
            const uint32_t ni = ref & PBRS_WREF_INDEX;
            const pbrs_node& n = P.nodes[ni];
            const uint32_t cnt = n.b & ~PBRS_LEAF_FLAG;
            if (cnt == 0u || cnt > PBRS_WREF_COUNT_MAX || n.a > PBRS_WREF_TRI) continue;
            bool own = true;
            for (uint32_t j = 0; j < cnt; ++j) own = own && P.tri_leaf[n.a + j] == ni;
            if (!own) continue;
            w.child[k] = (ref & ~PBRS_WREF_INDEX) | PBRS_WREF_PACKED | (cnt - 1u) << PBRS_WREF_COUNT_SHIFT | n.a;
            ++packed;
        }
    return packed;
}

void write_light_links(const PreparedScene& P, std::vector<pbrs_area_light>& lights) {
    for (size_t l = 0; l < lights.size() && l < P.light_link.size(); ++l) {
        const uint32_t inst = P.light_link[l] & PBRS_SKIP_INST_MASK, leaf = P.light_link[l] >> PBRS_SKIP_FLAT_SHIFT;
        std::memcpy(&lights[l].pad[0], &inst, sizeof inst);
        std::memcpy(&lights[l].pad[1], &leaf, sizeof leaf);
    }
}

}
```

pbrs_amd/csrc/host/scene_prepare.h:

```cpp
#pragma once
#include <cstdint>
#include <vector>

#include "../device/scene.h"
#include "kernel_choice.h"

namespace pbrs {

struct SceneLevels {
    uint32_t tlas = 0;
    uint32_t max_blas = 0;
    uint32_t stack = 0;
    bool exact_extent = false;
};
struct SceneCheck {
    int code = PBRS_OK;
    const char* message = nullptr;
    SceneLevels levels;
};
SceneCheck check_scene(const pbrs_scene_desc& d);

struct PreparedScene {
    DevScene S{};
    std::vector<pbrs_node> nodes;
    std::vector<uint32_t> node_planes;
    std::vector<pbrs_instance> inst;
    std::vector<pbrs_wnode> wide;
    std::vector<uint32_t> tri_leaf;
    std::vector<uint32_t> light_link;
    uint32_t wide_levels = 0;
    SceneFacts facts;
    uint32_t stack_depth = 0;
    bool has_vis_records = false;
    uint64_t walk_bytes = 0;
};
PreparedScene prepare_scene(const pbrs_scene_desc& d, const SceneLevels& levels, const DevOverrides& dev);
uint32_t pack_wide_leaves(PreparedScene& P);
void write_light_links(const PreparedScene& P, std::vector<pbrs_area_light>& lights);

}
```

pbrs_amd/csrc/kernel_tables.h:

```cpp
#pragma once
#include <cstdint>

#include "device/path_state.h"
#include "host/kernel_choice.h"

#pragma GCC visibility push(hidden)
namespace pbrs {

typedef void (*extend_fn_t)(DevScene, PathState, uint32_t, const uint32_t*, uint32_t, uint32_t*, GlobalCounters*, const uint32_t*, uint32_t*, uint32_t*, uint32_t);
typedef void (*shadow_fn_t)(DevScene, PathState, const uint32_t*, uint32_t*, GlobalCounters*, const uint32_t*, uint32_t*, uint32_t*);
typedef void (*shade_fn_t)(DevScene, PathState, RenderConst, uint32_t, const uint32_t*, uint32_t, uint32_t*, uint32_t*, unsigned long long*, uint32_t, const uint2*,
                           const uint32_t*);
typedef void (*intersect_fn_t)(DevScene, uint32_t, const float4*, const float4*, const float*, pbrs_hit_record*, uint8_t*, uint32_t*);
typedef void (*bsdf_eval_fn_t)(DevScene, uint32_t, uint32_t, const uint32_t*, uint32_t*);

const extend_fn_t* extend_fns();
const shadow_fn_t* shadow_fns();
intersect_fn_t intersect_fn(bool wide_any);

shade_fn_t shade_fn(const ShadeKey& key);
bsdf_eval_fn_t bsdf_eval_fn(bool lambert, bool fourier);

}
#pragma GCC visibility pop
```

pbrs_amd/csrc/pbrs_gpu.hip:

```cpp
#include <hip/hip_runtime.h>

#include <algorithm>
#include <cmath>
#include <cstdio>
#include <cstdlib>
#include <cstring>
#include <utility>
#include <mutex>
#include <optional>
#include <string>
#include <vector>

#include "../../include/pbrs_gpu.h"
#include "device/raygen.h"
#include "device/class_sort.h"
#include "device/accumulate.h"
#include "device/dev_kernels.h"
#include "kernel_tables.h"
#include "host/scene_prepare.h"
#include "host/arg_checks.h"
#include "host/pass_plan.h"
#include "device/aov.h"
#include "device/film.h"
#include "device/denoise.h"
#include "device/moments.h"
#include "device/matte.h"
#include "device/passes.h"
#include "device/temporal.h"
#include "device/spatial_variance.h"
#include "device/display.h"
#include "device/upsample.h"
#include "device/compare.h"
#include "device/despeckle.h"
#include "device/bloom.h"
#include "device/dof.h"
#include "device/motion_blur.h"

using namespace pbrs;

namespace {

#ifndef PBRS_SPLIT_KEEP_PERCENT
#define PBRS_SPLIT_KEEP_PERCENT 85u
#endif

struct StageEvent {
    int stage;
    hipEvent_t a, b;
};

#ifdef PBRS_DEV_OVERRIDES
const char* dev_env(const char* name) { return std::getenv(name); }

DevOverrides read_dev_overrides() {
    DevOverrides o;
    auto flag = [](const char* name, bool& v) {
        if (const char* e = dev_env(name)) v = std::atoi(e) != 0;
    };
    flag("PBRS_OVERLAP_PASSES", o.overlap_passes);
    flag("PBRS_SORT_CLASSES", o.sort_classes);
    flag("PBRS_SPLIT_LAMBERT", o.split_lambert);
    flag("PBRS_SPLIT_FOURIER", o.split_fourier);
    flag("PBRS_SPLIT_QUEUE", o.split_queue);
    flag("PBRS_LDS_SCENE", o.lds_scene);
    flag("PBRS_LDS_TOP", o.lds_top);
    flag("PBRS_RAYGEN_TILES8", o.raygen_tiles8);
    if (const char* e = dev_env("PBRS_WIDE")) o.wide_shadow = (std::atoi(e) & 2) != 0;
    if (const char* e = dev_env("PBRS_SHADE_SPEC")) o.shade_spec = (uint32_t)std::atoi(e);
    if (const char* e = dev_env("PBRS_SHADE_LDS")) o.shade_lds = (uint32_t)std::atoi(e);
    if (const char* e = dev_env("PBRS_LONG_WALKS")) o.long_walks = std::atoi(e) != 0;
    if (const char* e = dev_env("PBRS_FULL_STEPS")) o.full_steps = std::atoi(e) != 0;
    if (const char* e = dev_env("PBRS_OVERLAP_FROM")) o.overlap_from = (uint32_t)std::atoi(e);
    if (const char* e = dev_env("PBRS_REFILL_BELOW")) o.refill_below = (uint32_t)std::atoi(e);
    if (const char* e = dev_env("PBRS_RAYGEN_CHUNK")) {
        const long v = std::atol(e);
        o.raygen_chunk = v > 0 ? (uint32_t)v : 0xffffffffu;
    }
    if (const char* e = dev_env("PBRS_LDS_MIN")) o.lds_min = (size_t)std::atol(e);
    return o;
}
#endif

struct IntegratorPlan {
    IntegratorChoice choice;
    shade_fn_t shade[2] = {};
};
struct KernelPlan {
    KernelChoice choice;
    extend_fn_t extend[2] = {};
    shadow_fn_t shadow[2] = {};
    shadow_fn_t shadow_slow = nullptr;
    IntegratorPlan integ[PBRS_INTEGRATOR_NORMALS + 1];
};
uint32_t reported_features(const TraversalKey& k) { return (k.key & ~kStatsKey) | ((k.key & kStatsKey) ? 0x80000000u : 0u); }

struct DeviceBuffer {
    void* p = nullptr;
    size_t cap_bytes = 0;
    int grow(pbrs_ctx* c, size_t bytes, const char* what);
    template <class T>
    T* as() const { return static_cast<T*>(p); }
};
enum BufferId {
    BUF_AOV_STATE, BUF_AOV_OUT,
    BUF_FILTER_SUM,
    BUF_DENOISE, BUF_DENOISE_VAR, BUF_DENOISE_STAGE, BUF_DENOISE_VAR_STAGE,
    BUF_MOMENT_STATE, BUF_VARIANCE_OUT,
    BUF_MATTE_STATE, BUF_MATTE_OUT, BUF_MATTE_SELECT,
    BUF_PASS_STATE, BUF_PASS_OUT, BUF_PASS_DIRECT, BUF_PASS_DIRECT_SET1,
    BUF_TEMPORAL_STAGE,
    BUF_MOTION_TABLE, BUF_MOTION_STAGE,
    BUF_SPATIAL_STAGE,
    BUF_DISPLAY, BUF_DISPLAY_STAGE,
    BUF_UPSAMPLE_STAGE,
    BUF_COMPARE, BUF_COMPARE_STAGE,
    BUF_DESPECKLE_STAGE,
    BUF_DESPECKLE,
    BUF_BLOOM, BUF_BLOOM_STAGE,
    BUF_DOF_STAGE,
    BUF_MOTION_BLUR_STAGE,
    N_BUFFERS
};

}

struct pbrs_ctx {
    int device = 0;
    hipStream_t own_stream = nullptr;
    hipStream_t stream = nullptr;
    std::string error;

    bool has_scene = false;
    std::vector<void*> scene_allocs;
    DevScene S{};
    uint32_t stack_depth = 0;

    struct PassSet {
        void* state_mem = nullptr;
        size_t cap_slots = 0;
        PathState st{};
        uint32_t* neeq = nullptr;
        uint32_t* rng_hi0 = nullptr;
        uint32_t* slow = nullptr;
        uint32_t* counters = nullptr;
        float4* direct = nullptr;
        hipEvent_t accumulated = nullptr;
        hipEvent_t late = nullptr;
        bool in_flight = false;
    } pass_set[2];
    int cur_set = 0;
    hipStream_t main_stream = nullptr;
    hipStream_t second_stream = nullptr;
    bool overlap_passes = true;
    uint32_t overlap_from = 2;
    size_t cap_pixels = 0;
    float* sum = nullptr;
    float* rgb_dev = nullptr;
    GlobalCounters* gcnt = nullptr;
    unsigned long long* nonfinite = nullptr;
    unsigned long long* bounce_acc = nullptr;

    std::vector<StageEvent> events;
    size_t events_used = 0;
    std::vector<hipEvent_t> total_ev;
    pbrs_stats pending{};
    bool pending_counters = false, pending_times = false;
    DevOverrides dev;
    KernelPlan plan;
    int split_decision = 0;
    unsigned long long* split_host = nullptr;
    hipEvent_t split_ev = nullptr;
    bool split_probe_in_flight = false;
    bool has_vis_records = false;
    bool lambert_scene = false, fourier_scene = false;
    std::vector<uint32_t> material_flags;
    uint64_t pending_closest = 0;
    pbrs_intersect_info last_intersect{};
    DeviceBuffer buf[N_BUFFERS];
};

namespace {

#define HIPCHK(ctx, expr)                                                                             \
    do {                                                                                              \
        hipError_t e_ = (expr);                                                                       \
        if (e_ != hipSuccess) {                                                                       \
            (ctx)->error = std::string(#expr) + ": " + hipGetErrorString(e_);                         \
            (void)hipGetLastError();  \
            return PBRS_E_DEVICE;                                                                     \
        }                                                                                             \
    } while (0)

struct CallAllocs {
    std::vector<void*> held;
    CallAllocs() = default;
    CallAllocs(const CallAllocs&) = delete;
    CallAllocs& operator=(const CallAllocs&) = delete;
    ~CallAllocs() {
        for (void* p : held) (void)hipFree(p);
    }
    template <class T>
    hipError_t alloc(T** p, size_t bytes) {
        void* q = nullptr;
        const hipError_t e = hipMalloc(&q, bytes);
        if (e == hipSuccess) held.push_back(q);
        *p = static_cast<T*>(q);
        return e;
    }
};

int fail(pbrs_ctx* c, int code, const char* msg) {
    c->error = msg;
    return code;
}
int fail(pbrs_ctx* c, const Refusal& r) { return r.code ? fail(c, r.code, r.message) : PBRS_OK; }

int enter(pbrs_ctx* c, const Refusal& r) {
    if (!c) return PBRS_E_INVALID;
    if (r.code) return fail(c, r);
    HIPCHK(c, hipSetDevice(c->device));
    return PBRS_OK;
}

template <class T>
int upload(pbrs_ctx* c, const T* src, size_t n, const T** dst) {
    *dst = nullptr;
    size_t bytes = (n ? n : 1) * sizeof(T);
    void* p = nullptr;
    HIPCHK(c, hipMalloc(&p, bytes));
    c->scene_allocs.push_back(p);
    if (n) HIPCHK(c, hipMemcpy(p, src, n * sizeof(T), hipMemcpyHostToDevice));
    *dst = static_cast<const T*>(p);
    return PBRS_OK;
}

// ... 170 lines not shown
    if (rc) return rc;
    HIPCHK(c, hipStreamSynchronize(c->stream));
    return PBRS_OK;
}

constexpr size_t kDenoiseBytesPerPixel = 3 * sizeof(float4) + sizeof(uint32_t);

struct RenderTargets {
    float* rgb = nullptr;
    pbrs_aov_buffers aovs{};
    float* variance = nullptr;
    bool want_matte = false;
    const pbrs_matte_params* matte = nullptr;
    pbrs_matte_buffers matte_out{};
    pbrs_pass_buffers passes{};
    const FilterConst* filt = nullptr;

    bool want_aovs() const {
        const pbrs_aov_buffers& a = aovs;
        return a.albedo || a.normal || a.coverage || a.depth || a.instance || a.material || a.prim;
    }
    bool want_passes() const { return passes.direct || passes.indirect || passes.direct_variance || passes.indirect_variance; }
    WantedOutputs wanted() const { return {want_aovs(), variance != nullptr, want_passes(), want_matte, matte, matte_out.ids && matte_out.coverage}; }
};

SceneState scene_state(const pbrs_ctx* c) { return {c->has_scene, c->has_vis_records}; }

int pass_size(pbrs_ctx* c, const pbrs_render_params* p, uint32_t& K, bool with_direct = false) {
    std::optional<uint64_t> free_bytes;
    size_t free_b = 0, total_b = 0;
    if (p->samples_per_pass == 0 && hipMemGetInfo(&free_b, &total_b) == hipSuccess) free_bytes = free_b;
    K = samples_per_pass((uint64_t)p->w * p->h, (uint64_t)p->strata_x * p->strata_y, p->samples_per_pass, with_direct,
                         (uint64_t)c->pass_set[0].cap_slots + c->pass_set[1].cap_slots,
                         (uint64_t)c->buf[BUF_PASS_DIRECT].cap_bytes + c->buf[BUF_PASS_DIRECT_SET1].cap_bytes, free_bytes);
    if ((uint64_t)p->w * p->h * K >= (1ull << 28)) return fail(c, PBRS_E_LIMIT, "tile x samples_per_pass above 2^28 paths");
    return PBRS_OK;
}

struct Timer {
    pbrs_ctx* c;
    bool on;
    int begin(int stage) {
        if (!on) return 0;
        if (c->events_used == c->events.size()) {
            StageEvent e{};
            if (hipEventCreate(&e.a) != hipSuccess || hipEventCreate(&e.b) != hipSuccess) return -1;
            c->events.push_back(e);
        }
        StageEvent& e = c->events[c->events_used];
        e.stage = stage;
        return hipEventRecord(e.a, c->stream) == hipSuccess ? 0 : -1;
    }
    int end() {
        if (!on) return 0;
        StageEvent& e = c->events[c->events_used++];
        return hipEventRecord(e.b, c->stream) == hipSuccess ? 0 : -1;
    }
};

RenderConst make_const(const pbrs_ctx* c, const pbrs_camera* cam, const pbrs_render_params* p) {
    RenderConst rc{};
    rc.cam = *cam;
    rc.x0 = p->x0; rc.y0 = p->y0; rc.w = p->w; rc.h = p->h;
    rc.strata_x = p->strata_x; rc.strata_y = p->strata_y;
    rc.max_depth = p->max_depth;
    rc.n_pixels = p->w * p->h;
    rc.band_rows = p->band_rows; rc.band_count = p->band_count; rc.band_index = p->band_index;
    rc.seed = p->seed;
    rc.integrator = p->integrator;
    rc.chunk_pixels = c->dev.raygen_chunk.value_or(4096u);
    if (rc.chunk_pixels > rc.n_pixels) rc.chunk_pixels = rc.n_pixels;
    rc.tiles8_per_row = (c->dev.raygen_tiles8 && p->w % 8u == 0u && p->h % 8u == 0u) ? p->w / 8u : 0u;
    return rc;
}

bool bind_kernels(const KernelChoice& ch, KernelPlan& p) {
    p = KernelPlan{};
    p.choice = ch;
    for (int s = 0; s < 2; ++s) {
        p.extend[s] = extend_fns()[ch.extend[s].key];
        p.shadow[s] = shadow_fns()[ch.shadow[s].key];
    }
    if (ch.wide_shadow) p.shadow_slow = shadow_fns()[ch.shadow_slow.key];
    bool ok = p.extend[0] && p.extend[1] && p.shadow[0] && p.shadow[1] && (!ch.wide_shadow || p.shadow_slow);
    for (uint32_t i = 0; i <= PBRS_INTEGRATOR_NORMALS; ++i) {
        IntegratorPlan& ip = p.integ[i];
        ip.choice = ch.integ[i];
        for (uint32_t k = 0; k < ip.choice.n_shade; ++k) {
            ip.shade[k] = shade_fn(ip.choice.shade[k]);
            ok = ok && ip.shade[k];
        }
    }
    return ok;
}

void poll_split_probe(pbrs_ctx* c) {
    if (!c->split_probe_in_flight || hipEventQuery(c->split_ev) != hipSuccess) {
        (void)hipGetLastError();
        return;
    }
    c->split_probe_in_flight = false;
    c->split_decision = (c->split_host[0] * 100ull <= c->split_host[1] * PBRS_SPLIT_KEEP_PERCENT) ? 1 : 2;
}

struct MatteKernels {
    void (*fold)(const pbrs_instance*, PathState, uint32_t*, uint32_t, uint32_t, uint32_t, uint32_t, uint32_t);
    void (*finalize)(const uint32_t*, uint32_t, uint32_t, uint32_t, float, uint32_t*, float*, float*);
};
#define PBRS_MATTE_KERNELS(N) {k_matte<N>, k_matte_finalize<N>}
constexpr MatteKernels kMatte[PBRS_MATTE_MAX_SLOTS] = {PBRS_MATTE_KERNELS(1), PBRS_MATTE_KERNELS(2), PBRS_MATTE_KERNELS(3), PBRS_MATTE_KERNELS(4),
                                                       PBRS_MATTE_KERNELS(5), PBRS_MATTE_KERNELS(6), PBRS_MATTE_KERNELS(7), PBRS_MATTE_KERNELS(8)};
#undef PBRS_MATTE_KERNELS

int run_pass(pbrs_ctx* c, RenderConst rc, uint32_t first, uint32_t kc, bool stats, Timer& tm, bool handoff, const RenderTargets& t) {
    pbrs_ctx::PassSet& set = cur(c);
    if (handoff && set.in_flight) HIPCHK(c, hipStreamWaitEvent(c->stream, set.accumulated, 0));
    auto to_late_stream = [&]() -> hipError_t {
        hipError_t e = hipEventRecord(set.late, c->stream);
        c->stream = c->second_stream;
        return e != hipSuccess ? e : hipStreamWaitEvent(c->stream, set.late, 0);
    };
    const uint32_t P = rc.n_pixels;
    const PassShape shape = pass_shape(P, kc);
    const uint32_t N = shape.n_slots, grid = shape.grid, pgrid = shape.pgrid, n_tiles = shape.n_tiles;
    rc.pass_first_sample = first;
    rc.n_slots = N;
    uint32_t* act = set.counters + kCounters.act;
    unsigned long long* ns = reinterpret_cast<unsigned long long*>(set.counters + kCounters.ns);
    uint32_t* slows = set.counters + kCounters.slows;
    uint32_t* xhead = set.counters + kCounters.xhead;
    uint32_t* shead = set.counters + kCounters.shead;
    uint32_t* shead2 = set.counters + kCounters.shead2;
    uint32_t* neeq = set.neeq;
    const KernelPlan& plan = c->plan;
    const KernelChoice& choice = plan.choice;
    const IntegratorPlan& ip = plan.integ[rc.integrator];
    const TraversalKey &xk = choice.extend[stats], &sk = choice.shadow[stats];
    DevScene xS = c->S;
    if (!(xS.features & PBRS_FEAT_FLAT_TLAS)) xS.n_flat = 0u;
    HIPCHK(c, hipMemsetAsync(set.counters, 0, kCounters.words * sizeof(uint32_t), c->stream));
    if (tm.begin(0)) return fail(c, PBRS_E_DEVICE, "event record failed");
    hipLaunchKernelGGL(k_raygen, dim3(grid), dim3(kBlock), 0, c->stream, set.st, rc, set.rng_hi0);
    tm.end();
    poll_split_probe(c);
    const uint32_t n_bounces = bounce_count(rc.integrator, rc.max_depth);
    if (n_bounces == 0) HIPCHK(c, hipMemsetAsync(set.st.L, 0, (size_t)N * sizeof(float4), c->stream));
    const bool probe_split = c->split_decision == 0 && !c->split_probe_in_flight && rc.integrator == PBRS_INTEGRATOR_PATH && choice.split_queue && n_bounces > 0;
    for (uint32_t b = 0; b < n_bounces; ++b) {
        if (handoff && b == c->overlap_from) HIPCHK(c, to_late_stream());
        const uint32_t* cnt_in = b == 0 ? nullptr : act + b;
        const BouncePlan bp = bounce_plan(rc.integrator, choice.split_queue, ip.choice, c->split_decision, b);
        const uint32_t qsplit = bp.split;
        if (tm.begin(1)) return fail(c, PBRS_E_DEVICE, "event record failed");
        hipLaunchKernelGGL(plan.extend[stats], dim3(pgrid), dim3(kBlock), xk.lds, c->stream, xS, set.st, b & 1u, cnt_in, N, xhead + b * kHeadWords, c->gcnt, nullptr,
                           nullptr, nullptr, qsplit);
        c->pending.kernel_features_extend = reported_features(xk);
        tm.end();
        if (b == 0 && t.want_aovs())
            hipLaunchKernelGGL(k_aov, dim3((P + kBlock - 1) / kBlock), dim3(kBlock), 0, c->stream, c->S, set.st, c->buf[BUF_AOV_STATE].as<float>(), P, kc,
                               rc.chunk_pixels, qsplit);
        if (b == 0 && t.want_matte)
            hipLaunchKernelGGL(kMatte[t.matte->slots - 1u].fold, dim3((P + kBlock - 1) / kBlock), dim3(kBlock), 0, c->stream, c->S.inst, set.st,
                               c->buf[BUF_MATTE_STATE].as<uint32_t>(), P, kc, rc.chunk_pixels, qsplit, t.matte->key);
        if (tm.begin(2)) return fail(c, PBRS_E_DEVICE, "event record failed");
        if (bp.order == IntegratorChoice::CLASS_MAJOR) {
            const bool two = bp.n_classes == 2u;
            if (two) hipLaunchKernelGGL(k_class_count<2u>, dim3(n_tiles), dim3(kBlock), 0, c->stream, set.st, cnt_in, N);
            else hipLaunchKernelGGL(k_class_count<PBRS_MAX_CLASSES>, dim3(n_tiles), dim3(kBlock), 0, c->stream, set.st, cnt_in, N);
            hipLaunchKernelGGL(k_class_scan, dim3(1), dim3(64 * PBRS_MAX_CLASSES), 0, c->stream, set.st, cnt_in, N, bp.last,
                               (qsplit && probe_split) ? c->bounce_acc + 2 * PBRS_STATS_MAX_BOUNCES : nullptr);
            if (two) hipLaunchKernelGGL(k_class_scatter<2u>, dim3(n_tiles), dim3(kBlock), 0, c->stream, set.st, cnt_in, N, bp.zero_dropped);
            else hipLaunchKernelGGL(k_class_scatter<PBRS_MAX_CLASSES>, dim3(n_tiles), dim3(kBlock), 0, c->stream, set.st, cnt_in, N, bp.zero_dropped);
        } else if (bp.order == IntegratorChoice::CLASS_SORT) {
            hipLaunchKernelGGL(k_class_sort, dim3(n_tiles), dim3(kBlock), 0, c->stream, set.st, cnt_in, N);
        }
        for (uint32_t k = 0; k < ip.choice.n_shade; ++k) {
            const uint2* range = bp.shade_range[k] ? set.st.class_range + bp.shade_range[k] : nullptr;
            hipLaunchKernelGGL(ip.shade[k], dim3(grid), dim3(kBlock), ip.choice.shade[k].lds, c->stream, c->S, set.st, rc, b, cnt_in, N, act + b + 1, neeq, ns + b,
                               bp.sorted, range, set.rng_hi0);
        }
        tm.end();
        if (tm.begin(3)) return fail(c, PBRS_E_DEVICE, "event record failed");
        hipLaunchKernelGGL(plan.shadow[stats], dim3(pgrid), dim3(kBlock), sk.lds, c->stream, c->S, set.st, reinterpret_cast<const uint32_t*>(ns + b),
                           shead + b * kHeadWords, c->gcnt + 1, nullptr, set.slow, slows + b);
        c->pending.kernel_features_shadow = reported_features(sk);
        if (choice.wide_shadow && !stats)
            hipLaunchKernelGGL(plan.shadow_slow, dim3(shape.slow_grid), dim3(kBlock), choice.shadow_slow.lds, c->stream, c->S, set.st, slows + b, shead2 + b * kHeadWords,
                               c->gcnt + 1, set.slow, nullptr, nullptr);
        hipLaunchKernelGGL(k_nee_resolve, dim3(shape.sgrid), dim3(kBlock), 0, c->stream, set.st, neeq, reinterpret_cast<const uint32_t*>(ns + b));
        tm.end();
        if (b == 0 && t.want_passes()) hipLaunchKernelGGL(k_pass_direct, dim3(grid), dim3(kBlock), 0, c->stream, set.st.L, set.direct, N);
    }
    if (probe_split) {
        unsigned long long* acc = c->bounce_acc + 2 * PBRS_STATS_MAX_BOUNCES;
        HIPCHK(c, hipMemcpyAsync(c->split_host, acc, 2 * sizeof(unsigned long long), hipMemcpyDeviceToHost, c->stream));
        HIPCHK(c, hipEventRecord(c->split_ev, c->stream));
        HIPCHK(c, hipMemsetAsync(acc, 0, 2 * sizeof(unsigned long long), c->stream));
        c->split_probe_in_flight = true;
    }
    if (stats)
        hipLaunchKernelGGL(k_sum_bounce_counts, dim3(1), dim3(64), 0, c->stream, act, ns, N, n_bounces, c->bounce_acc);
    if (handoff && c->stream != c->second_stream) HIPCHK(c, to_late_stream());
    if (tm.begin(4)) return fail(c, PBRS_E_DEVICE, "event record failed");
    if (const FilterConst* filt = t.filt)
        hipLaunchKernelGGL(k_filter_accumulate, dim3((filt->w + PBRS_FILTER_CELL - 1) / PBRS_FILTER_CELL, (filt->h + PBRS_FILTER_CELL - 1) / PBRS_FILTER_CELL),
                           dim3(kBlock), filter_lds_bytes(filt->hx, filt->hy), c->stream, set.st, c->buf[BUF_FILTER_SUM].as<float>(), rc, *filt, kc, c->nonfinite);
    else
        hipLaunchKernelGGL(k_accumulate, dim3((P + kBlock - 1) / kBlock), dim3(kBlock), 0, c->stream, set.st, c->sum, P, kc, rc.chunk_pixels, rc.w, rc.tiles8_per_row, c->nonfinite);
    if (t.variance)
        hipLaunchKernelGGL(k_moments, dim3((P + kBlock - 1) / kBlock), dim3(kBlock), 0, c->stream, set.st, c->buf[BUF_MOMENT_STATE].as<float>(), P, kc, rc.chunk_pixels);
    if (t.want_passes())
        hipLaunchKernelGGL(k_pass_fold, dim3((P + kBlock - 1) / kBlock), dim3(kBlock), 0, c->stream, set.st.L, set.direct,
                           c->buf[BUF_PASS_STATE].as<float>(), P, kc, rc.chunk_pixels);
    tm.end();
    if (handoff) {
        HIPCHK(c, hipEventRecord(set.accumulated, c->stream));
        set.in_flight = true;
    }
    HIPCHK(c, hipGetLastError());
    return PBRS_OK;
}

int render_common(pbrs_ctx* c, const pbrs_camera* cam, const pbrs_render_params* p, uint32_t K, const RenderTargets& t) {
    const uint32_t P = p->w * p->h;
    const uint32_t spp = p->strata_x * p->strata_y;
    const FilterConst* filt = t.filt;
    float* aov = t.want_aovs() ? c->buf[BUF_AOV_STATE].as<float>() : nullptr;
    float* moments = t.variance ? c->buf[BUF_MOMENT_STATE].as<float>() : nullptr;
    uint32_t* matte = t.want_matte ? c->buf[BUF_MATTE_STATE].as<uint32_t>() : nullptr;
    float* pass_state = t.want_passes() ? c->buf[BUF_PASS_STATE].as<float>() : nullptr;
    float* filter_sum = c->buf[BUF_FILTER_SUM].as<float>();
    RenderConst rc = make_const(c, cam, p);
    const bool stats = p->collect_counters != 0;
    Timer tm{c, p->time_stages != 0};
    c->events_used = 0;
    c->pending = pbrs_stats{};
    c->pending_counters = stats;
    c->pending_times = p->time_stages != 0;
    c->pending.samples = (uint64_t)P * spp;
    if (stats) HIPCHK(c, hipMemsetAsync(c->gcnt, 0, 2 * sizeof(GlobalCounters), c->stream));
    if (stats) HIPCHK(c, hipMemsetAsync(c->bounce_acc, 0, 2 * PBRS_STATS_MAX_BOUNCES * sizeof(unsigned long long), c->stream));
    HIPCHK(c, hipMemsetAsync(c->nonfinite, 0, sizeof(unsigned long long), c->stream));
    if (c->pending_times) HIPCHK(c, hipEventRecord(c->total_ev[0], c->stream));
    if (filt) HIPCHK(c, hipMemsetAsync(filter_sum, 0, 4 * (size_t)filt->w * filt->h * sizeof(float), c->stream));
    else HIPCHK(c, hipMemsetAsync(c->sum, 0, 3 * (size_t)P * sizeof(float), c->stream));
    if (aov) HIPCHK(c, hipMemsetAsync(aov, 0, PBRS_AOV_STATE_WORDS * (size_t)P * sizeof(float), c->stream));
    if (moments) HIPCHK(c, hipMemsetAsync(moments, 0, PBRS_MOMENT_STATE_WORDS * (size_t)P * sizeof(float), c->stream));
    if (matte) HIPCHK(c, hipMemsetAsync(matte, 0, PBRS_MATTE_STATE_WORDS(t.matte->slots) * (size_t)P * sizeof(uint32_t), c->stream));
    if (pass_state) HIPCHK(c, hipMemsetAsync(pass_state, 0, PBRS_PASS_STATE_WORDS * (size_t)P * sizeof(float), c->stream));
    uint32_t passes = 0;
    bool two = c->overlap_passes && !stats && spp > K;
    if (two && (ensure_work(c, c->pass_set[1], (size_t)P * K, P) || ensure_direct(c, 1, (size_t)P * K, pass_state != nullptr))) {
        two = false;
        c->error.clear();
    }
    for (uint32_t first = 0; first < spp; first += K) {
        uint32_t kc = spp - first < K ? spp - first : K;
        if (two) use_pass_set(c, (int)(passes & 1u));
        const int rcode = run_pass(c, rc, first, kc, stats, tm, two, t);
        if (rcode) {
            use_pass_set(c, 0);
            return rcode;
        }
        ++passes;
    }
    if (two) {
        const hipEvent_t last = cur(c).accumulated;
        use_pass_set(c, 0);
        HIPCHK(c, hipStreamWaitEvent(c->main_stream, last, 0));
    }
    if (filt) {
        const uint32_t PT = filt->w * filt->h;
        hipLaunchKernelGGL(k_filter_finalize, dim3((PT + kBlock - 1) / kBlock), dim3(kBlock), 0, c->stream, filter_sum, t.rgb, PT);
    } else {
        hipLaunchKernelGGL(k_finalize, dim3((P + kBlock - 1) / kBlock), dim3(kBlock), 0, c->stream, c->sum, t.rgb, P, 1.0f / (float)spp);
    }
    if (aov)
        hipLaunchKernelGGL(k_aov_finalize, dim3((P + kBlock - 1) / kBlock), dim3(kBlock), 0, c->stream, aov, c->S.inst, P, rc.w, rc.tiles8_per_row,
                           1.0f / (float)spp, t.aovs);
    if (moments)
        hipLaunchKernelGGL(k_moments_finalize, dim3((P + kBlock - 1) / kBlock), dim3(kBlock), 0, c->stream, moments, P, rc.w, rc.tiles8_per_row, t.variance);
    if (matte)
        hipLaunchKernelGGL(kMatte[t.matte->slots - 1u].finalize, dim3((P + kBlock - 1) / kBlock), dim3(kBlock), 0, c->stream, matte, P, rc.w,
                           rc.tiles8_per_row, 1.0f / (float)spp, t.matte_out.ids, t.matte_out.coverage, t.matte_out.residual);
    if (pass_state)
        hipLaunchKernelGGL(k_pass_finalize, dim3((P + kBlock - 1) / kBlock), dim3(kBlock), 0, c->stream, pass_state, P, rc.w, rc.tiles8_per_row,
                           1.0f / (float)spp, t.passes);
    if (c->pending_times) HIPCHK(c, hipEventRecord(c->total_ev[1], c->stream));
    HIPCHK(c, hipGetLastError());
    c->pending.passes = passes;
    c->pending.launches_extend = c->pending.launches_shade = c->pending.launches_shadow = passes * bounce_count(rc.integrator, rc.max_depth);
    return PBRS_OK;
}

int collect(pbrs_ctx* c, pbrs_stats* out) {
    HIPCHK(c, hipStreamSynchronize(c->stream));
    pbrs_stats s = c->pending;
    {
        unsigned long long bad = 0;
        HIPCHK(c, hipMemcpy(&bad, c->nonfinite, sizeof bad, hipMemcpyDeviceToHost));
        s.invalid_samples = bad;
    }
    if (c->pending_counters) {
        GlobalCounters g[2];
        HIPCHK(c, hipMemcpy(g, c->gcnt, sizeof g, hipMemcpyDeviceToHost));
        s.closest_rays = g[0].rays;
        s.shade_events = g[0].hits;
        s.tlas_nodes = g[0].tlas_nodes; s.blas_nodes = g[0].blas_nodes; s.instances = g[0].instances;
        s.instance_hits = g[0].instance_hits; s.triangles = g[0].triangles; s.tri_shading = g[0].tri_shading;
        s.spheres = g[0].spheres; s.quads = g[0].quads; s.cuboids = g[0].cuboids; s.disks = g[0].disks;
        s.shadow_rays = g[1].rays;
        s.shadow_tlas_nodes = g[1].tlas_nodes; s.shadow_blas_nodes = g[1].blas_nodes; s.shadow_instances = g[1].instances;
        s.shadow_triangles = g[1].triangles;
        s.shadow_prims = g[1].spheres + g[1].quads + g[1].cuboids + g[1].disks;
        unsigned long long per_bounce[2 * PBRS_STATS_MAX_BOUNCES];
        HIPCHK(c, hipMemcpy(per_bounce, c->bounce_acc, sizeof per_bounce, hipMemcpyDeviceToHost));
        for (uint32_t b = 0; b < PBRS_STATS_MAX_BOUNCES; ++b) {
            s.paths_at_bounce[b] = per_bounce[b];
            s.shadow_rays_at_bounce[b] = per_bounce[PBRS_STATS_MAX_BOUNCES + b];
        }
    }
    if (c->pending_times) {
        float* acc[5] = {&s.ms_raygen, &s.ms_extend, &s.ms_shade, &s.ms_shadow, &s.ms_accumulate};
        for (size_t i = 0; i < c->events_used; ++i) {
            float ms = 0.0f;
            HIPCHK(c, hipEventElapsedTime(&ms, c->events[i].a, c->events[i].b));
            *acc[c->events[i].stage] += ms;
        }
        HIPCHK(c, hipEventElapsedTime(&s.ms_total, c->total_ev[0], c->total_ev[1]));
    }
    if (out) *out = s;
    return PBRS_OK;
}

std::mutex g_kernel_cfg_mutex;
bool g_kernel_cfg_done[64] = {};
int configure_kernels(pbrs_ctx* c) {
    std::lock_guard<std::mutex> lock(g_kernel_cfg_mutex);
    if (c->device < 64 && g_kernel_cfg_done[c->device]) return PBRS_OK;
    const int cap = (int)(kLdsBytesPerCU / 2);
    std::vector<const void*> traversal_kernels = {reinterpret_cast<const void*>(intersect_fn(false)), reinterpret_cast<const void*>(intersect_fn(true))};
    for (uint32_t k = 0; k < kTraversalKeys; ++k) {
        if (extend_fns()[k]) traversal_kernels.push_back(reinterpret_cast<const void*>(extend_fns()[k]));
        if (shadow_fns()[k]) traversal_kernels.push_back(reinterpret_cast<const void*>(shadow_fns()[k]));
    }
    for (const void* k : traversal_kernels) HIPCHK(c, hipFuncSetAttribute(k, hipFuncAttributeMaxDynamicSharedMemorySize, cap));
    if (c->device < 64) g_kernel_cfg_done[c->device] = true;
    return PBRS_OK;
}

int filter_setup(pbrs_ctx* c, const pbrs_camera* cam, const pbrs_render_params* p, const pbrs_pixel_filter* f, FilterConst& fc, pbrs_render_params& region) {
    const int rc = fail(c, check_filter(p, f));
    if (rc) return rc;
    fc = FilterConst{};
    fc.kind = f->kind;
    fc.rx = f->radius[0], fc.ry = f->radius[1], fc.a = f->a, fc.b = f->b;
    fc.hx = pf_halo(fc.rx), fc.hy = pf_halo(fc.ry);
    fc.x0 = p->x0, fc.y0 = p->y0, fc.w = p->w, fc.h = p->h;
    region = *p;
    region.x0 = p->x0 > fc.hx ? p->x0 - fc.hx : 0u;
    region.y0 = p->y0 > fc.hy ? p->y0 - fc.hy : 0u;
    region.w = std::min(p->x0 + p->w + fc.hx, cam->width) - region.x0;
    region.h = std::min(p->y0 + p->h + fc.hy, cam->height) - region.y0;
    return fail(c, check_params(scene_state(c), cam, &region));
}

int render(pbrs_ctx* c, const pbrs_camera* cam, const pbrs_render_params* p, const pbrs_pixel_filter* filter, RenderTargets t, bool host, pbrs_stats* stats_out) {
    HIPCHK(c, hipSetDevice(c->device));
    FilterConst fc;
    pbrs_render_params region;
    int rc = fail(c, check_params(scene_state(c), cam, p));
    if (rc) return rc;
    const size_t PT = (size_t)p->w * p->h;
    if (filter) {
        if ((rc = filter_setup(c, cam, p, filter, fc, region))) return rc;
        t.filt = &fc;
        p = &region;
    }
    if ((rc = fail(c, check_targets(p, t.wanted())))) return rc;
    const size_t P = (size_t)p->w * p->h;
    const pbrs_aov_buffers& a = t.aovs;
    Staged aovs[] = {{nullptr, 3, a.albedo}, {nullptr, 3, a.normal}, {nullptr, 1, a.coverage}, {nullptr, 1, a.depth}, {nullptr, 1, a.instance},
                     {nullptr, 1, a.material}, {nullptr, 1, a.prim}};
    Staged variance[] = {{nullptr, 1, t.variance}};
    const size_t slots = t.want_matte ? t.matte->slots : 0;
    Staged matte[] = {{nullptr, slots, t.matte_out.ids}, {nullptr, slots, t.matte_out.coverage}, {nullptr, 1, t.matte_out.residual}};
    Staged passes[] = {{nullptr, 3, t.passes.direct}, {nullptr, 3, t.passes.indirect}, {nullptr, 1, t.passes.direct_variance},
                       {nullptr, 1, t.passes.indirect_variance}};
    float* const rgb_host = t.rgb;
    if (t.filt) rc = c->buf[BUF_FILTER_SUM].grow(c, 4 * PT * sizeof(float), "the filter sums");
    if (t.want_aovs()) {
        if (!rc) rc = c->buf[BUF_AOV_STATE].grow(c, PBRS_AOV_STATE_WORDS * P * sizeof(float), "the AOV state");
        if (!rc && host) rc = stage(c, BUF_AOV_OUT, "the AOV buffers", aovs, P);
    }
    if (t.variance) {
        if (!rc) rc = c->buf[BUF_MOMENT_STATE].grow(c, PBRS_MOMENT_STATE_WORDS * P * sizeof(float), "the variance AOV's moments");
        if (!rc && host) rc = stage(c, BUF_VARIANCE_OUT, "the variance buffer", variance, P);
    }
    if (t.want_matte) {
        if (!rc) rc = c->buf[BUF_MATTE_STATE].grow(c, PBRS_MATTE_STATE_WORDS(slots) * P * sizeof(uint32_t), "the matte state");
        if (!rc && host) rc = stage(c, BUF_MATTE_OUT, "the matte buffers", matte, P);
    }
    if (t.want_passes()) {
        if (!rc) rc = c->buf[BUF_PASS_STATE].grow(c, PBRS_PASS_STATE_WORDS * P * sizeof(float), "the light passes' state");
        if (!rc && host) rc = stage(c, BUF_PASS_OUT, "the light pass buffers", passes, P);
    }
    uint32_t K = 0;
    if (!rc) rc = pass_size(c, p, K, t.want_passes());
    if (!rc) rc = ensure_work(c, cur(c), P * K, P);
    if (!rc) rc = ensure_direct(c, c->cur_set, P * K, t.want_passes());
    if (rc) return rc;
    if (host) {
        t.rgb = c->rgb_dev;
        t.aovs = {aovs[0].as<float>(), aovs[1].as<float>(), aovs[2].as<float>(), aovs[3].as<float>(), aovs[4].as<uint32_t>(), aovs[5].as<uint32_t>(), aovs[6].as<uint32_t>()};
        t.variance = variance[0].as<float>();
        t.matte_out = {matte[0].as<uint32_t>(), matte[1].as<float>(), matte[2].as<float>()};
        t.passes = {passes[0].as<float>(), passes[1].as<float>(), passes[2].as<float>(), passes[3].as<float>()};
    }
    rc = render_common(c, cam, p, K, t);
    if (rc) return rc;
    if (!host) return stats_out ? collect(c, stats_out) : PBRS_OK;
    HIPCHK(c, hipMemcpyAsync(rgb_host, t.rgb, 3 * PT * sizeof(float), hipMemcpyDeviceToHost, c->stream));
    if ((rc = copy_staged(c, variance, P, hipMemcpyDeviceToHost))) return rc;
    if ((rc = copy_staged(c, aovs, P, hipMemcpyDeviceToHost))) return rc;
    if ((rc = copy_staged(c, matte, P, hipMemcpyDeviceToHost))) return rc;
    if ((rc = copy_staged(c, passes, P, hipMemcpyDeviceToHost))) return rc;
// ... 23 lines not shown
    int n = 0;
    if (hipGetDeviceCount(&n) != hipSuccess || n <= 0 || device_ordinal < 0 || device_ordinal >= n) return PBRS_E_DEVICE;
    pbrs_ctx* c = new pbrs_ctx();
    c->device = device_ordinal;
    bool ok = hipSetDevice(device_ordinal) == hipSuccess && hipStreamCreateWithFlags(&c->own_stream, hipStreamNonBlocking) == hipSuccess;
    c->stream = c->main_stream = c->own_stream;
    {
        int least = 0, greatest = 0;
        ok = ok && hipDeviceGetStreamPriorityRange(&least, &greatest) == hipSuccess &&
             hipStreamCreateWithPriority(&c->second_stream, hipStreamNonBlocking, greatest) == hipSuccess;
    }
    ok = ok && hipEventCreateWithFlags(&c->pass_set[0].accumulated, hipEventDisableTiming) == hipSuccess &&
         hipEventCreateWithFlags(&c->pass_set[1].accumulated, hipEventDisableTiming) == hipSuccess &&
         hipEventCreateWithFlags(&c->pass_set[0].late, hipEventDisableTiming) == hipSuccess &&
         hipEventCreateWithFlags(&c->pass_set[1].late, hipEventDisableTiming) == hipSuccess;
#ifdef PBRS_DEV_OVERRIDES
    c->dev = read_dev_overrides();
#endif
    c->overlap_passes = c->dev.overlap_passes;
    for (int k = 0; ok && k < 2; ++k) {
        hipEvent_t ev = nullptr;
        ok = hipEventCreate(&ev) == hipSuccess;
        if (ok) c->total_ev.push_back(ev);
    }
    for (pbrs_ctx::PassSet& set : c->pass_set) ok = ok && hipMalloc(reinterpret_cast<void**>(&set.counters), kCounters.words * sizeof(uint32_t)) == hipSuccess;
    ok = ok && hipMalloc(reinterpret_cast<void**>(&c->gcnt), 2 * sizeof(GlobalCounters)) == hipSuccess &&
         hipMalloc(reinterpret_cast<void**>(&c->nonfinite), sizeof(unsigned long long)) == hipSuccess &&
         hipMalloc(reinterpret_cast<void**>(&c->bounce_acc), (2 * PBRS_STATS_MAX_BOUNCES + 2) * sizeof(unsigned long long)) == hipSuccess &&
         hipMemset(c->bounce_acc, 0, (2 * PBRS_STATS_MAX_BOUNCES + 2) * sizeof(unsigned long long)) == hipSuccess &&
         hipMemset(c->nonfinite, 0, sizeof(unsigned long long)) == hipSuccess &&
         hipHostMalloc(reinterpret_cast<void**>(&c->split_host), 2 * sizeof(unsigned long long), hipHostMallocDefault) == hipSuccess &&
         hipEventCreateWithFlags(&c->split_ev, hipEventDisableTiming) == hipSuccess;
    ok = ok && configure_kernels(c) == PBRS_OK;
    if (!ok) {
        pbrs_destroy(c);
        return PBRS_E_DEVICE;
    }
    *out = c;
    return PBRS_OK;
}

void pbrs_destroy(pbrs_ctx* c) {
    if (!c) return;
    (void)hipSetDevice(c->device);
    if (c->stream) (void)hipStreamSynchronize(c->stream);
    if (c->second_stream) (void)hipStreamSynchronize(c->second_stream);
    free_scene(c);
    free_work(c);
    for (DeviceBuffer& b : c->buf)
        if (b.p) (void)hipFree(b.p);
    for (pbrs_ctx::PassSet& set : c->pass_set)
        if (set.counters) (void)hipFree(set.counters);
    for (int k = 0; k < 2; ++k)
        if (c->pass_set[k].accumulated) (void)hipEventDestroy(c->pass_set[k].accumulated);
    for (int k = 0; k < 2; ++k)
        if (c->pass_set[k].late) (void)hipEventDestroy(c->pass_set[k].late);
    if (c->second_stream) (void)hipStreamDestroy(c->second_stream);
    if (c->gcnt) (void)hipFree(c->gcnt);
    if (c->nonfinite) (void)hipFree(c->nonfinite);
    if (c->bounce_acc) (void)hipFree(c->bounce_acc);
    if (c->split_host) (void)hipHostFree(c->split_host);
    if (c->split_ev) (void)hipEventDestroy(c->split_ev);
    for (auto& e : c->events) {
        (void)hipEventDestroy(e.a);
        (void)hipEventDestroy(e.b);
    }
    for (auto& e : c->total_ev) (void)hipEventDestroy(e);
    if (c->own_stream) (void)hipStreamDestroy(c->own_stream);
    delete c;
}

const char* pbrs_last_error(const pbrs_ctx* c) { return c ? c->error.c_str() : "null context"; }

int pbrs_set_stream(pbrs_ctx* c, void* hip_stream) {
    if (!c) return PBRS_E_INVALID;
    c->main_stream = hip_stream ? static_cast<hipStream_t>(hip_stream) : c->own_stream;
    c->stream = c->main_stream;
    return PBRS_OK;
}

int pbrs_set_pass_overlap(pbrs_ctx* c, int enabled) {
    if (!c) return PBRS_E_INVALID;
    c->overlap_passes = enabled != 0;
    return PBRS_OK;
}

int pbrs_upload_scene(pbrs_ctx* c, const pbrs_scene_desc* d) {
    if (!c || !d) return PBRS_E_INVALID;
    HIPCHK(c, hipSetDevice(c->device));
    const SceneCheck chk = check_scene(*d);
    if (chk.code != PBRS_OK) return fail(c, chk.code, chk.message);
    PreparedScene P = prepare_scene(*d, chk.levels, c->dev);
    const KernelChoice choice = choose_kernels(P.facts, c->dev);
    KernelPlan plan;
    if (!bind_kernels(choice, plan)) return fail(c, PBRS_E_DEVICE, "no kernel instantiation for this scene's feature set");
    (void)hipStreamSynchronize(c->stream);
    (void)hipStreamSynchronize(c->second_stream);
    free_scene(c);
    c->plan = plan;
    DevScene S = P.S;
    int rc;
    for (size_t i = 0; i < P.nodes.size(); ++i) P.nodes[i].b |= P.node_planes[i];
    if ((rc = upload(c, P.nodes.data(), P.nodes.size(), &S.nodes))) return rc;
    pack_wide_leaves(P);
    if (!P.wide.empty() && (rc = upload_wide(c, P, &S.wnodes))) return rc;
    if ((rc = upload(c, P.inst.data(), P.inst.size(), &S.inst))) return rc;
    if ((rc = upload(c, d->shapes, d->n_shapes, &S.shapes))) return rc;
    if ((rc = upload(c, d->meshes, d->n_meshes, &S.meshes))) return rc;
    if ((rc = upload(c, d->tri_verts, d->n_triangles, &S.tv))) return rc;
    if ((rc = upload(c, d->tri_shade, d->n_triangles, &S.ts))) return rc;
    if ((rc = upload(c, d->materials, d->n_materials, &S.mats))) return rc;
    if ((rc = upload(c, d->bxdfs, d->n_bxdfs, &S.bxdfs))) return rc;
    {
        std::vector<pbrs_area_light> lights(d->area_lights, d->area_lights + d->n_area_lights);
        write_light_links(P, lights);
        if ((rc = upload(c, lights.data(), lights.size(), &S.alights))) return rc;
    }
    if ((rc = upload(c, d->delta_lights, d->n_delta_lights, &S.dlights))) return rc;
    if ((rc = upload(c, d->textures, d->n_textures, &S.textures))) return rc;
    if ((rc = upload(c, d->tex_floats, d->n_tex_floats, &S.tex_floats))) return rc;
    if ((rc = upload(c, d->tex_words, d->n_tex_words, &S.tex_words))) return rc;
    if ((rc = upload(c, d->fourier_tables, d->n_fourier_tables, &S.fourier))) return rc;
    const bool lds_scene = choice.lds_staging == PBRS_FEAT_LDS_SCENE;
    S.lds_off_words = P.stack_depth * kBlock;
    S.lds_nodes = lds_scene ? (uint32_t)P.nodes.size() : choice.lds_staging == PBRS_FEAT_LDS_TOP ? d->n_tlas_nodes : 0u;
    S.lds_tris = lds_scene ? d->n_triangles : 0u;
    S.lds_inst = lds_scene ? d->n_instances : 0u;
    S.lds_shapes = lds_scene ? d->n_shapes : 0u;
    c->S = S;
    c->overlap_from = c->dev.overlap_from.value_or(P.walk_bytes <= (4ull << 20) ? 2u : 4u);
    c->has_vis_records = P.has_vis_records;
    c->lambert_scene = P.facts.lambert;
    c->fourier_scene = P.facts.fourier;
    c->material_flags.resize(d->n_materials);
    for (uint32_t i = 0; i < d->n_materials; ++i) c->material_flags[i] = d->materials[i].flags;
    c->stack_depth = P.stack_depth;
    c->has_scene = true;
    c->split_decision = 0;
    c->split_probe_in_flight = false;
    return PBRS_OK;
}

int pbrs_render_tile_passes_device(pbrs_ctx* c, const pbrs_camera* cam, const pbrs_render_params* p, float* rgb_out_device,
                                   const pbrs_aov_buffers* aovs_device, float* variance_device, const pbrs_matte_params* params,
                                   const pbrs_matte_buffers* matte_device, const pbrs_pass_buffers* passes_device, pbrs_stats* stats_out) {
    if (!c) return PBRS_E_INVALID;
    if (!rgb_out_device) return fail(c, PBRS_E_INVALID, "null output");
    return render(c, cam, p, nullptr, make_targets(rgb_out_device, aovs_device, variance_device, params, matte_device, passes_device), false, stats_out);
}

int pbrs_render_tile_matte_device(pbrs_ctx* c, const pbrs_camera* cam, const pbrs_render_params* p, float* rgb_out_device,
                                  const pbrs_aov_buffers* aovs_device, float* variance_device, const pbrs_matte_params* params,
                                  const pbrs_matte_buffers* matte_device, pbrs_stats* stats_out) {
    return pbrs_render_tile_passes_device(c, cam, p, rgb_out_device, aovs_device, variance_device, params, matte_device, nullptr, stats_out);
}

int pbrs_render_tile_aovs_var_device(pbrs_ctx* c, const pbrs_camera* cam, const pbrs_render_params* p, float* rgb_out_device,
                                     const pbrs_aov_buffers* aovs_device, float* variance_device, pbrs_stats* stats_out) {
    return pbrs_render_tile_matte_device(c, cam, p, rgb_out_device, aovs_device, variance_device, nullptr, nullptr, stats_out);
}

int pbrs_render_tile_aovs_device(pbrs_ctx* c, const pbrs_camera* cam, const pbrs_render_params* p, float* rgb_out_device, const pbrs_aov_buffers* aovs_device,
                                 pbrs_stats* stats_out) {
    return pbrs_render_tile_matte_device(c, cam, p, rgb_out_device, aovs_device, nullptr, nullptr, nullptr, stats_out);
}

int pbrs_render_tile_device(pbrs_ctx* c, const pbrs_camera* cam, const pbrs_render_params* p, float* rgb_out_device, pbrs_stats* stats_out) {
    return pbrs_render_tile_matte_device(c, cam, p, rgb_out_device, nullptr, nullptr, nullptr, nullptr, stats_out);
}

int pbrs_render_tile_passes(pbrs_ctx* c, const pbrs_camera* cam, const pbrs_render_params* p, float* rgb_out_host, const pbrs_aov_buffers* aovs_host,
                            float* variance_host, const pbrs_matte_params* params, const pbrs_matte_buffers* matte_host, const pbrs_pass_buffers* passes_host,
                            pbrs_stats* stats_out) {
    if (!c) return PBRS_E_INVALID;
    if (!rgb_out_host) return fail(c, PBRS_E_INVALID, "null output");
    return render(c, cam, p, nullptr, make_targets(rgb_out_host, aovs_host, variance_host, params, matte_host, passes_host), true, stats_out);
}

int pbrs_render_tile_matte(pbrs_ctx* c, const pbrs_camera* cam, const pbrs_render_params* p, float* rgb_out_host, const pbrs_aov_buffers* aovs_host,
                           float* variance_host, const pbrs_matte_params* params, const pbrs_matte_buffers* matte_host, pbrs_stats* stats_out) {
    return pbrs_render_tile_passes(c, cam, p, rgb_out_host, aovs_host, variance_host, params, matte_host, nullptr, stats_out);
}

int pbrs_render_tile_aovs_var(pbrs_ctx* c, const pbrs_camera* cam, const pbrs_render_params* p, float* rgb_out_host, const pbrs_aov_buffers* aovs_host,
                              float* variance_host, pbrs_stats* stats_out) {
    return pbrs_render_tile_matte(c, cam, p, rgb_out_host, aovs_host, variance_host, nullptr, nullptr, stats_out);
}

int pbrs_render_tile_aovs(pbrs_ctx* c, const pbrs_camera* cam, const pbrs_render_params* p, float* rgb_out_host, const pbrs_aov_buffers* aovs_host,
                          pbrs_stats* stats_out) {
    return pbrs_render_tile_matte(c, cam, p, rgb_out_host, aovs_host, nullptr, nullptr, nullptr, stats_out);
}

int pbrs_render_tile(pbrs_ctx* c, const pbrs_camera* cam, const pbrs_render_params* p, float* rgb_out_host, pbrs_stats* stats_out) {
    return pbrs_render_tile_matte(c, cam, p, rgb_out_host, nullptr, nullptr, nullptr, nullptr, stats_out);
}

int pbrs_render_tile_filtered_device(pbrs_ctx* c, const pbrs_camera* cam, const pbrs_render_params* p, const pbrs_pixel_filter* f,
                                     float* rgb_out_device, pbrs_stats* stats_out) {
    if (!c) return PBRS_E_INVALID;
    if (!rgb_out_device) return fail(c, PBRS_E_INVALID, "null output");
    if (!f) return fail(c, PBRS_E_INVALID, "null pixel filter");
    return render(c, cam, p, f, make_targets(rgb_out_device, nullptr, nullptr, nullptr, nullptr, nullptr), false, stats_out);
}

int pbrs_render_tile_filtered(pbrs_ctx* c, const pbrs_camera* cam, const pbrs_render_params* p, const pbrs_pixel_filter* f, float* rgb_out_host,
                              pbrs_stats* stats_out) {
    if (!c) return PBRS_E_INVALID;
    if (!rgb_out_host) return fail(c, PBRS_E_INVALID, "null output");
    if (!f) return fail(c, PBRS_E_INVALID, "null pixel filter");
    return render(c, cam, p, f, make_targets(rgb_out_host, nullptr, nullptr, nullptr, nullptr, nullptr), true, stats_out);
}

static_assert(sizeof(pbrs_denoise_params) == 32, "pbrs_denoise_params is 32 B");
static_assert(sizeof(pbrs_denoise_var_params) == 32, "pbrs_denoise_var_params is 32 B");

namespace {

using DenoiseKernel = void (*)(const float4*, const float4*, const uint32_t*, float4*, DenoiseConst);
// ... 897 lines not shown
    float *d_x = nullptr, *d_y = nullptr, *d_r = nullptr;
    CallAllocs mem;
    HIPCHK(c, mem.alloc(&d_x, (size_t)n * 4));
    HIPCHK(c, mem.alloc(&d_r, (size_t)n * 4));
    HIPCHK(c, hipMemcpyAsync(d_x, x, (size_t)n * 4, hipMemcpyHostToDevice, c->stream));
    if (y) {
        HIPCHK(c, mem.alloc(&d_y, (size_t)n * 4));
        HIPCHK(c, hipMemcpyAsync(d_y, y, (size_t)n * 4, hipMemcpyHostToDevice, c->stream));
    }
    hipLaunchKernelGGL(k_numeric_eval, dim3((n + kBlock - 1) / kBlock), dim3(kBlock), 0, c->stream, fn, n, d_x, d_y, d_r);
    HIPCHK(c, hipGetLastError());
    HIPCHK(c, hipMemcpyAsync(out, d_r, (size_t)n * 4, hipMemcpyDeviceToHost, c->stream));
    HIPCHK(c, hipStreamSynchronize(c->stream));
    return PBRS_OK;
}

int pbrs_numeric_eval_k(pbrs_ctx* c, uint32_t fn, uint32_t n, uint32_t k, const uint32_t* ops, uint32_t* out) {
    if (!c) return PBRS_E_INVALID;
    if (n == 0) return PBRS_OK;
    if (!ops || !out || fn > PN_PROBE_K_LAST || k > PN_PROBE_MAX_K || k < pn_probe_k_operands(fn))
        return fail(c, PBRS_E_INVALID, "bad numeric_eval_k arguments");
    HIPCHK(c, hipSetDevice(c->device));
    uint32_t *d_ops = nullptr, *d_r = nullptr;
    CallAllocs mem;
    HIPCHK(c, mem.alloc(&d_ops, (size_t)n * k * 4));
    HIPCHK(c, mem.alloc(&d_r, (size_t)n * 4));
    HIPCHK(c, hipMemcpyAsync(d_ops, ops, (size_t)n * k * 4, hipMemcpyHostToDevice, c->stream));
    hipLaunchKernelGGL(k_numeric_eval_k, dim3((n + kBlock - 1) / kBlock), dim3(kBlock), 0, c->stream, fn, n, k, d_ops, d_r);
    HIPCHK(c, hipGetLastError());
    HIPCHK(c, hipMemcpyAsync(out, d_r, (size_t)n * 4, hipMemcpyDeviceToHost, c->stream));
    HIPCHK(c, hipStreamSynchronize(c->stream));
    return PBRS_OK;
}

int pbrs_bsdf_eval(pbrs_ctx* c, uint32_t op, uint32_t lambert, uint32_t n, const uint32_t* queries, uint32_t* results) {
    if (!c) return PBRS_E_INVALID;
    if (n == 0) return PBRS_OK;
    if (!c->has_scene) return fail(c, PBRS_E_INVALID, "bsdf_eval: no scene uploaded");
    if (!queries || !results) return fail(c, PBRS_E_INVALID, "bsdf_eval: null queries or results");
    if (op > PBRS_BSDF_SAMPLE_SPECULAR) return fail(c, PBRS_E_INVALID, "bsdf_eval: unknown op");
    if (lambert && !c->lambert_scene) return fail(c, PBRS_E_INVALID, "bsdf_eval: the Lambert variant needs a scene whose every lobe is an untextured Lambertian");
    for (uint32_t i = 0; i < n; ++i) {
        const uint32_t m = queries[(size_t)i * PBRS_BSDF_QUERY_WORDS];
        if (m >= c->material_flags.size()) return fail(c, PBRS_E_INVALID, "bsdf_eval: material index out of range");
        if (c->material_flags[m] & PBRS_MATERIAL_TEXTURED)
            return fail(c, PBRS_E_INVALID, "bsdf_eval: textured materials are out of scope (a query carries no uv or position)");
        if (op == PBRS_BSDF_SAMPLE) {
            float u;
            std::memcpy(&u, queries + (size_t)i * PBRS_BSDF_QUERY_WORDS + 13, sizeof u);
            if (!(u >= 0.0f && u < 1.0f)) return fail(c, PBRS_E_INVALID, "bsdf_eval: u outside [0, 1) would pick a lobe the material does not have");
        }
    }
    const bsdf_eval_fn_t fn = bsdf_eval_fn(lambert != 0, c->fourier_scene);
    if (!fn) return fail(c, PBRS_E_DEVICE, "bsdf_eval: no kernel instantiation for this scene");
    HIPCHK(c, hipSetDevice(c->device));
    uint32_t *d_q = nullptr, *d_r = nullptr;
    CallAllocs mem;
    const size_t q_bytes = (size_t)n * PBRS_BSDF_QUERY_WORDS * 4, r_bytes = (size_t)n * PBRS_BSDF_RESULT_WORDS * 4;
    HIPCHK(c, mem.alloc(&d_q, q_bytes));
    HIPCHK(c, mem.alloc(&d_r, r_bytes));
    HIPCHK(c, hipMemcpyAsync(d_q, queries, q_bytes, hipMemcpyHostToDevice, c->stream));
    hipLaunchKernelGGL(fn, dim3((n + kBlock - 1) / kBlock), dim3(kBlock), 0, c->stream, c->S, op, n, d_q, d_r);
    HIPCHK(c, hipGetLastError());
    HIPCHK(c, hipMemcpyAsync(results, d_r, r_bytes, hipMemcpyDeviceToHost, c->stream));
    HIPCHK(c, hipStreamSynchronize(c->stream));
    return PBRS_OK;
}

int pbrs_render_sample_radiance(pbrs_ctx* c, const pbrs_camera* cam, const pbrs_render_params* p, uint32_t sample_index, float* rgb_out_host) {
    if (!c) return PBRS_E_INVALID;
    HIPCHK(c, hipSetDevice(c->device));
    int rc = fail(c, check_params(scene_state(c), cam, p));
    if (rc) return rc;
    if (!rgb_out_host) return fail(c, PBRS_E_INVALID, "null output");
    const uint32_t P = p->w * p->h;
    uint32_t K;
    if ((rc = pass_size(c, p, K))) return rc;
    rc = ensure_work(c, cur(c), P, P);
    if (rc) return rc;
    RenderConst k = make_const(c, cam, p);
    k.tiles8_per_row = 0u;
    Timer tm{c, false};
    HIPCHK(c, hipMemsetAsync(c->sum, 0, 3 * (size_t)P * sizeof(float), c->stream));
    rc = run_pass(c, k, sample_index, 1, false, tm, false, RenderTargets{});
    if (rc) return rc;
    hipLaunchKernelGGL(k_export_radiance, dim3((P + kBlock - 1) / kBlock), dim3(kBlock), 0, c->stream, cur(c).st, P, c->rgb_dev);
    HIPCHK(c, hipGetLastError());
    HIPCHK(c, hipMemcpyAsync(rgb_out_host, c->rgb_dev, 3 * (size_t)P * sizeof(float), hipMemcpyDeviceToHost, c->stream));
    HIPCHK(c, hipStreamSynchronize(c->stream));
    return PBRS_OK;
}

}
```

pbrs_amd/csrc/traverse.hip:

```cpp
#include <hip/hip_runtime.h>

#include <utility>

#include "kernel_tables.h"

#ifdef PBRS_PROBE_TIME
__device__ unsigned long long g_trav_time[2][8];
#endif
#ifdef PBRS_PROBE_TRAV
__device__ unsigned long long g_trav_probe[2][24];
#endif
#define PBRS_TRAVERSAL_PROBES_DEFINED
#include "device/extend.h"
#include "device/intersect.h"
#include "device/shadow.h"

using namespace pbrs;

namespace {

template <uint32_t K>
constexpr extend_fn_t extend_fn_of() {
    if constexpr (extend_key_ok(K)) return &k_extend<(K & kStatsKey) != 0u, (K & ~kStatsKey)>;
    else return nullptr;
}
template <uint32_t K>
constexpr shadow_fn_t shadow_fn_of() {
    if constexpr (shadow_key_ok(K)) return &k_shadow<(K & kStatsKey) != 0u, (K & ~kStatsKey)>;
    else return nullptr;
}
template <uint32_t... K>
const extend_fn_t* extend_table(std::integer_sequence<uint32_t, K...>) {
    static const extend_fn_t t[sizeof...(K)] = {extend_fn_of<K>()...};
    return t;
}
template <uint32_t... K>
const shadow_fn_t* shadow_table(std::integer_sequence<uint32_t, K...>) {
    static const shadow_fn_t t[sizeof...(K)] = {shadow_fn_of<K>()...};
    return t;
}

}

namespace pbrs {

const extend_fn_t* extend_fns() { return extend_table(std::make_integer_sequence<uint32_t, kTraversalKeys>{}); }
const shadow_fn_t* shadow_fns() { return shadow_table(std::make_integer_sequence<uint32_t, kTraversalKeys>{}); }
intersect_fn_t intersect_fn(bool wide_any) { return wide_any ? &k_intersect_rays<true> : &k_intersect_rays<false>; }

}

extern "C" {

#ifdef PBRS_PROBE_TIME
int pbrs_debug_trav_time(unsigned long long* out16) {
    if (hipDeviceSynchronize() != hipSuccess) return -1;
    if (hipMemcpyFromSymbol(out16, HIP_SYMBOL(g_trav_time), 16 * sizeof(unsigned long long)) != hipSuccess) return -1;
    unsigned long long zero[16] = {0};
    return hipMemcpyToSymbol(HIP_SYMBOL(g_trav_time), zero, sizeof zero) == hipSuccess ? 0 : -1;
}
#endif
#ifdef PBRS_PROBE_TRAV
int pbrs_debug_trav_probe(unsigned long long* out48) {
    if (hipDeviceSynchronize() != hipSuccess) return -1;
    if (hipMemcpyFromSymbol(out48, HIP_SYMBOL(g_trav_probe), 48 * sizeof(unsigned long long)) != hipSuccess) return -1;
    unsigned long long zero[48] = {0};
    return hipMemcpyToSymbol(HIP_SYMBOL(g_trav_probe), zero, sizeof zero) == hipSuccess ? 0 : -1;
}
#endif

}
```

pbrs_amd/libs.py:

```python
import ctypes as C
import os

from .abi import Camera, SceneDesc
from .spec import SceneSpec

_LIBDIR = os.path.join(os.path.dirname(os.path.abspath(__file__)), "lib")


class PbrsError(RuntimeError):
    pass


P, U32, INT, STR = C.c_void_p, C.c_uint32, C.c_int, C.c_char_p


def _table(functions, with_device=()):
    full = {n: v if isinstance(v, tuple) else (v, INT) for n, v in {**functions, **dict(with_device)}.items()}
    return {**full, **{n + "_device": full[n] for n in with_device}}


GPU_FUNCTIONS = _table({
    "pbrs_create": [INT, C.POINTER(P)],
    "pbrs_destroy": [P],
    "pbrs_last_error": ([P], STR),
    "pbrs_set_stream": [P, P],
    "pbrs_set_pass_overlap": [P, INT],
    "pbrs_upload_scene": [P, P],
    "pbrs_collect_stats": [P, P],
    "pbrs_intersect_rays": [P, U32] + [P] * 5,
    "pbrs_last_intersect_info": [P, P],
    "pbrs_camera_rays": [P, P, P, U32, P, P],
    "pbrs_numeric_eval": [P, U32, U32, P, P, P],
    "pbrs_numeric_eval_k": [P, U32, U32, U32, P, P],
    "pbrs_bsdf_eval": [P, U32, U32, U32, P, P],
    "pbrs_render_sample_radiance": [P, P, P, U32, P],
    "pbrs_display_params_default": ([U32, U32, P], None),
    "pbrs_upsample_params_default": ([U32, U32, U32, P], None),
}, with_device={
    "pbrs_render_tile": [P] * 5,
    "pbrs_render_tile_aovs": [P] * 6,
    "pbrs_render_tile_filtered": [P] * 6,
    "pbrs_denoise": [P] * 5,
    "pbrs_render_tile_aovs_var": [P] * 7,
    "pbrs_denoise_var": [P] * 6,
    "pbrs_render_tile_matte": [P] * 9,
    "pbrs_matte_mask": [P, U32, U32, U32, P, P, P, U32, P],
    "pbrs_render_tile_passes": [P] * 10,
    "pbrs_combine_passes": [P, U32, U32, P, P, P],
    "pbrs_temporal_accumulate": [P] * 9,
    "pbrs_temporal_accumulate_motion": [P] * 10 + [U32],
    "pbrs_temporal_accumulate_clip": [P] * 10 + [U32, P],
    "pbrs_motion_vectors": [P, U32, U32] + [P] * 5 + [U32, P, P],
    "pbrs_spatial_variance": [P] * 7,
    "pbrs_display": [P] * 5,
    "pbrs_upsample": [P] * 7,
})
GPU_COMPARE_FUNCTIONS = _table({
    "pbrsx_compare_params_default": ([U32, U32, P], None),
}, with_device={
    "pbrsx_compare": [P] * 6,
})
GPU_DESPECKLE_FUNCTIONS = _table({
    "pbrsi_despeckle_params_default": ([U32, U32, P], None),
}, with_device={
    "pbrsi_despeckle": [P] * 4,
})
GPU_BLOOM_FUNCTIONS = _table({
    "pbrsb_bloom_params_default": ([U32, U32, P], None),
}, with_device={
    "pbrsb_bloom": [P] * 4,
})
GPU_DOF_FUNCTIONS = _table({
    "pbrsf_dof_params_default": ([U32, U32, P], None),
}, with_device={
    "pbrsf_dof": [P] * 6,
})
GPU_MOTION_BLUR_FUNCTIONS = _table({
    "pbrsm_motion_blur_params_default": ([U32, U32, P], None),
}, with_device={
    "pbrsm_motion_blur": [P] * 7,
})
HOST_FUNCTIONS = _table({
    "pbrs_host_scene_build": [P, C.POINTER(P)],
    "pbrs_host_scene_free": [P],
    "pbrs_host_scene_desc": ([P], C.POINTER(SceneDesc)),
    "pbrs_host_scene_camera": ([P], C.POINTER(Camera)),
    "pbrs_host_scene_stack_depth": ([P], U32),
    "pbrs_host_last_error": ([], STR),
    "pbrs_host_load_pbrt": [STR, C.POINTER(P)],
    "pbrs_loaded_scene_spec": ([P], C.POINTER(SceneSpec)),
    "pbrs_loaded_scene_free": [P],
    "pbrs_host_load_error": ([], STR),
    "pbrs_loaded_scene_filter": [P, P],
    "pbrs_host_write_exr": [STR, P, U32, U32],
    "pbrs_host_write_png": [STR, P, U32, U32],
    "pbrs_host_write_png_rgba8": [STR, P, U32, U32],
    "pbrs_host_io_error": ([], STR),
})
GPU_SYMBOLS, HOST_SYMBOLS = list(GPU_FUNCTIONS), list(HOST_FUNCTIONS)
GPU_COMPARE_SYMBOLS = list(GPU_COMPARE_FUNCTIONS)
GPU_DESPECKLE_SYMBOLS = list(GPU_DESPECKLE_FUNCTIONS)
GPU_BLOOM_SYMBOLS = list(GPU_BLOOM_FUNCTIONS)
GPU_DOF_SYMBOLS = list(GPU_DOF_FUNCTIONS)
GPU_MOTION_BLUR_SYMBOLS = list(GPU_MOTION_BLUR_FUNCTIONS)
_host = _gpu = _hip = None


def _load(path, functions):
    L = C.CDLL(path)
    for name, (argtypes, restype) in functions.items():
        fn = getattr(L, name)
        fn.argtypes, fn.restype = argtypes, restype
    return L


def lib_paths():
    return os.path.join(_LIBDIR, "libpbrs_host.so"), os.path.join(_LIBDIR, "libpbrs_gpu.so")


def host_lib():
    global _host
    if _host is None:
        path = os.environ.get("PBRS_HOST_LIB") or lib_paths()[0]
        if not os.path.exists(path):
            raise PbrsError(f"{path} is missing: run `python -c 'import __graft_entry__ as g; g.build()'` (make -C pbrs_amd/csrc)")
        _host = _load(path, HOST_FUNCTIONS)
    return _host


def gpu_lib():
    global _gpu
    if _gpu is None:
        path = os.environ.get("PBRS_GPU_LIB") or lib_paths()[1]
        if not os.path.exists(path):
            raise PbrsError(f"{path} is missing: the HIP extension must be built (make -C pbrs_amd/csrc); there is no CPU fallback")
        _gpu = _load(path, {**GPU_FUNCTIONS, **GPU_COMPARE_FUNCTIONS, **GPU_DESPECKLE_FUNCTIONS, **GPU_BLOOM_FUNCTIONS, **GPU_DOF_FUNCTIONS,
                            **GPU_MOTION_BLUR_FUNCTIONS})
    return _gpu


def hip_runtime():
    global _hip
    if _hip is None:
        gpu_lib()
        path = next(line.split()[-1] for line in open("/proc/self/maps") if "libamdhip64" in line)
        _hip = _load(path, _table({"hipMalloc": [C.POINTER(P), C.c_size_t], "hipMemcpy": [P, P, C.c_size_t, INT], "hipFree": [P]}))
    return _hip
```

Measured before the change: 1743.

## Add per-pixel BVH entry-node table for primary-ray traversal

```diff
diff --git a/include/pbrs_gpu.h b/include/pbrs_gpu.h
--- a/include/pbrs_gpu.h
+++ b/include/pbrs_gpu.h
@@ -203,6 +203,15 @@
 
 int pbrs_set_pass_overlap(pbrs_ctx*, int enabled);
 
+int pbrse_set_entry_nodes(pbrs_ctx*, int enabled);
+typedef struct pbrs_entry_info {
+    uint32_t pixels_with_entries;
+    uint32_t pixels_empty;
+    uint32_t pixels_from_root;
+    uint32_t entries;
+} pbrs_entry_info;
+int pbrse_last_entry_info(pbrs_ctx*, pbrs_entry_info* out);
+
 int pbrs_upload_scene(pbrs_ctx*, const pbrs_scene_desc*);
 
 typedef struct pbrs_render_params {
diff --git a/pbrs_amd/api.py b/pbrs_amd/api.py
--- a/pbrs_amd/api.py
+++ b/pbrs_amd/api.py
@@ -12,7 +12,7 @@
                   TemporalParams, UpsampleParams, _aov_names, _bloom_params, _DenoiseParamsMixin, _despeckle_params, _display_params, _dof_params, _history_clip, _matte_select, _motion_args, _motion_blur_params, _pass_names,
                   _reference_frame, _reference_frames, _temporal_struct, _upscale_params, lens, scaled_camera)
 from .devmem import DeviceBuffers
-from .libs import GPU_BLOOM_SYMBOLS, GPU_COMPARE_SYMBOLS, GPU_DESPECKLE_SYMBOLS, GPU_DOF_SYMBOLS, GPU_MOTION_BLUR_SYMBOLS, GPU_SYMBOLS, HOST_SYMBOLS, PbrsError, gpu_lib, hip_runtime, host_lib, lib_paths
+from .libs import GPU_BLOOM_SYMBOLS, GPU_COMPARE_SYMBOLS, GPU_DESPECKLE_SYMBOLS, GPU_DOF_SYMBOLS, GPU_ENTRY_SYMBOLS, GPU_MOTION_BLUR_SYMBOLS, GPU_SYMBOLS, HOST_SYMBOLS, PbrsError, gpu_lib, hip_runtime, host_lib, lib_paths
 from .spec import SceneSpec
 
 
@@ -216,6 +216,14 @@
 
     def set_pass_overlap(self, enabled):
         self._check(self._L.pbrs_set_pass_overlap(self._h, int(bool(enabled))), "pbrs_set_pass_overlap")
+
+    def set_entry_nodes(self, enabled):
+        self._check(self._L.pbrse_set_entry_nodes(self._h, int(bool(enabled))), "pbrse_set_entry_nodes")
+
+    def last_entry_info(self):
+        v = (C.c_uint32 * 4)()
+        self._check(self._L.pbrse_last_entry_info(self._h, C.addressof(v)), "pbrse_last_entry_info")
+        return {"pixels_with_entries": int(v[0]), "pixels_empty": int(v[1]), "pixels_from_root": int(v[2]), "entries": int(v[3])}
 
     def upload(self, host_scene):
         self._check(self._L.pbrs_upload_scene(self._h, C.addressof(host_scene.desc)), "pbrs_upload_scene")
diff --git a/pbrs_amd/csrc/device/entry_nodes.h b/pbrs_amd/csrc/device/entry_nodes.h
--- /dev/null
+++ b/pbrs_amd/csrc/device/entry_nodes.h
@@ -0,0 +1,126 @@
+#pragma once
+#include <stdint.h>
+
+#include "../../../include/pbrs_gpu.h"
+
+#if defined(__HIPCC__)
+#define PBRS_EN_FN __host__ __device__ static inline
+#else
+#define PBRS_EN_FN static inline
+#endif
+
+#define PBRS_ENTRY_MAX 8u
+#define PBRS_ENTRY_FORKS 3u
+#define PBRS_ENTRY_ROOT 0xfffffffeu
+#define PBRS_ENTRY_UNUSED 0xffffffffu
+#define PBRS_ENTRY_NONE 0xffffffffu
+
+struct pbrs_entry_record {
+    uint32_t e[PBRS_ENTRY_MAX];
+};
+
+PBRS_EN_FN void pbrs_camera_dir(const pbrs_camera& cam, float x, float y, float d[3]) {
+    for (int k = 0; k < 3; ++k) d[k] = cam.c[k] + cam.a[k] * x + cam.b[k] * y;
+}
+
+PBRS_EN_FN uint32_t pbrs_en_bits(float x) {
+    union {
+        float f;
+        uint32_t u;
+    } v;
+    v.f = x;
+    return v.u;
+}
+PBRS_EN_FN bool pbrs_en_dir_in_range(float x) { return ((pbrs_en_bits(x) >> 23) & 0xffu) - (127u - 40u) <= 80u; }
+PBRS_EN_FN bool pbrs_en_origin_in_range(float x) {
+    const uint32_t u = pbrs_en_bits(x) & 0x7fffffffu;
+    return u == 0u || (u >> 23) - (127u - 60u) <= 100u;
+}
+
+struct pbrs_dir_box {
+    float lo[3], hi[3];
+};
+PBRS_EN_FN bool pbrs_entry_dir_box(const pbrs_camera& cam, uint32_t col, uint32_t row, pbrs_dir_box& B) {
+    bool ok = true;
+    for (int i = 0; i < 4; ++i) {
+        float d[3];
+        pbrs_camera_dir(cam, (float)(col + (uint32_t)(i & 1)), (float)(row + (uint32_t)(i >> 1)), d);
+        for (int k = 0; k < 3; ++k) {
+            ok = ok && pbrs_en_dir_in_range(d[k]);
+            B.lo[k] = i == 0 || d[k] < B.lo[k] ? d[k] : B.lo[k];
+            B.hi[k] = i == 0 || d[k] > B.hi[k] ? d[k] : B.hi[k];
+        }
+    }
+    for (int k = 0; k < 3; ++k) ok = ok && ((B.lo[k] > 0.0f) == (B.hi[k] > 0.0f));
+    return ok;
+}
+
+PBRS_EN_FN bool pbrs_entry_beam(const pbrs_node& n, const float o[3], const pbrs_dir_box& B) {
+    float lb = 0.0f, ub = 0.0f;
+    for (int k = 0; k < 3; ++k) {
+        const float n0 = n.min[k] - o[k], n1 = n.max[k] - o[k];
+        const float q[4] = {n0 / B.lo[k], n0 / B.hi[k], n1 / B.lo[k], n1 / B.hi[k]};
+        float mn = q[0], mx = q[0];
+        for (int i = 1; i < 4; ++i) mn = q[i] < mn ? q[i] : mn, mx = q[i] > mx ? q[i] : mx;
+        lb = k == 0 || mn > lb ? mn : lb;
+        ub = k == 0 || mx < ub ? mx : ub;
+    }
+    return (lb > 0.0f ? lb : 0.0f) <= ub;
+}
+
+PBRS_EN_FN uint32_t pbrs_entry_refine(const pbrs_node* nodes, uint32_t root, const float o[3], const pbrs_dir_box& B, uint32_t forks, pbrs_entry_record& rec,
+                                      uint32_t depth[PBRS_ENTRY_MAX]) {
+    uint32_t n = 0;
+    for (uint32_t i = 0; i < PBRS_ENTRY_MAX; ++i) rec.e[i] = PBRS_ENTRY_UNUSED, depth[i] = 0u;
+    if (!pbrs_entry_beam(nodes[root], o, B)) return 0u;
+    uint32_t pend_node[PBRS_ENTRY_FORKS], pend_depth[PBRS_ENTRY_FORKS], pend_forks[PBRS_ENTRY_FORKS], np = 0;
+    uint32_t x = root, dx = 0u, fx = forks < PBRS_ENTRY_FORKS ? forks : PBRS_ENTRY_FORKS;
+    for (;;) {
+        const pbrs_node X = nodes[x];
+        bool emit = (X.b & PBRS_LEAF_FLAG) != 0u, drop = false;
+        if (!emit) {
+            const uint32_t left = x + 1u, right = X.a;
+            const bool pl = pbrs_entry_beam(nodes[left], o, B), pr = pbrs_entry_beam(nodes[right], o, B);
+            if (pl != pr) {
+                x = pl ? left : right;
+                ++dx;
+                continue;
+            }
+            if (!pl) drop = true;
+            else if (fx == 0u) emit = true;
+            else {
+                const bool left_first = B.lo[X.b & 3u] > 0.0f;
+                --fx;
+                pend_node[np] = left_first ? right : left, pend_depth[np] = dx + 1u, pend_forks[np] = fx;
+                ++np;
+                x = left_first ? left : right;
+                ++dx;
+                continue;
+            }
+        }
+        if (emit && !drop) rec.e[n] = x, depth[n] = dx, ++n;
+        if (np == 0u) break;
+        --np;
+        x = pend_node[np], dx = pend_depth[np], fx = pend_forks[np];
+    }
+    return n;
+}
+
+PBRS_EN_FN bool pbrs_entry_fits(uint32_t n, const uint32_t depth[PBRS_ENTRY_MAX], uint32_t height, uint32_t rows) {
+    for (uint32_t i = 0; i < n; ++i)
+        if ((n - 1u - i) + (height > depth[i] ? height - depth[i] : 1u) + 1u > rows) return false;
+    return true;
+}
+
+PBRS_EN_FN uint32_t pbrs_entry_record_of(const pbrs_node* nodes, uint32_t root, const float o[3], const pbrs_dir_box& B, uint32_t max_forks, uint32_t height,
+                                         uint32_t rows, pbrs_entry_record& rec) {
+    uint32_t depth[PBRS_ENTRY_MAX];
+    for (uint32_t f = max_forks < PBRS_ENTRY_FORKS ? max_forks : PBRS_ENTRY_FORKS;; --f) {
+        const uint32_t n = pbrs_entry_refine(nodes, root, o, B, f, rec, depth);
+        if (pbrs_entry_fits(n, depth, height, rows)) return n;
+        if (f == 0u) break;
+    }
+    for (uint32_t i = 0; i < PBRS_ENTRY_MAX; ++i) rec.e[i] = PBRS_ENTRY_UNUSED;
+    rec.e[0] = PBRS_ENTRY_ROOT;
+    return PBRS_ENTRY_ROOT;
+}
diff --git a/pbrs_amd/csrc/device/extend.h b/pbrs_amd/csrc/device/extend.h
--- a/pbrs_amd/csrc/device/extend.h
+++ b/pbrs_amd/csrc/device/extend.h
@@ -182,10 +182,12 @@
     return S;
 }
 
-template <bool STATS, uint32_t FEAT>
+template <bool STATS, uint32_t FEAT, class... ENTRY>
 __global__ void __launch_bounds__(256, STATS ? 3 : (FEAT & PBRS_FEAT_SHADING_CHECK) ? PBRS_TRAV_WAVES : PBRS_LEAN_EXTEND_WAVES)
     k_extend(DevScene G, PathState st, uint32_t set, const uint32_t* count, uint32_t n_direct, uint32_t* next, GlobalCounters* gc, const uint32_t* indirect,
-             uint32_t* slow_list, uint32_t* slow_count, uint32_t split) {
+             uint32_t* slow_list, uint32_t* slow_count, uint32_t split, ENTRY... entry) {
+    static_assert(sizeof...(ENTRY) <= 1, "at most the entry table's arguments");
+    constexpr bool HAS_ENTRY = sizeof...(ENTRY) != 0;
     extern __shared__ __attribute__((aligned(16))) uint32_t lds_stack[];
     const DevScene S = (!STATS && (FEAT & PBRS_FEAT_LDS_SCENE)) ? stage_scene(G, lds_stack) : (!STATS && (FEAT & PBRS_FEAT_LDS_TOP)) ? stage_top(G, lds_stack) : G;
     const uint32_t n = count ? *count : n_direct;
@@ -195,7 +197,8 @@
     Cnt<STATS> cnt;
     cnt.init();
     uint32_t nrays = 0, nhit = 0;
-    ClosestWalk<STATS, (FEAT & (PBRS_FEAT_ALL | PBRS_FEAT_LDS_TOP | PBRS_FEAT_EXTENT))> walk;
+    ClosestWalk<STATS, (FEAT & (PBRS_FEAT_ALL | PBRS_FEAT_LDS_TOP | PBRS_FEAT_EXTENT)), HAS_ENTRY> walk;
+    if constexpr (HAS_ENTRY) walk.a = (entry, ...);
     walk.mode = PBRS_WALK_IDLE;
     PBRS_KP_DECL(walk);
     PBRS_TT_DECL;
diff --git a/pbrs_amd/csrc/device/path_state.h b/pbrs_amd/csrc/device/path_state.h
--- a/pbrs_amd/csrc/device/path_state.h
+++ b/pbrs_amd/csrc/device/path_state.h
@@ -1,4 +1,5 @@
 #pragma once
+#include "entry_nodes.h"
 #include "shapes.h"
 
 struct PathState {
@@ -27,6 +28,11 @@
     uint32_t band_rows, band_count, band_index;
     uint32_t integrator;
     uint64_t seed;
+};
+
+struct EntryArgs {
+    const uint4* table;
+    uint32_t n_pixels, k_count, chunk;
 };
 
 template <class T>
@@ -73,6 +79,13 @@
     return (((y >> 3) * tiles8_per_row + (x >> 3)) << 6) + ((y & 7u) << 3) + (x & 7u);
 }
 
+PD void film_pixel_of_order(const RenderConst& rc, uint32_t q, uint32_t& col, uint32_t& row) {
+    const uint32_t pix = pixel_of_order(q, rc.w, rc.tiles8_per_row);
+    const uint32_t vrow = pix / rc.w;
+    col = rc.x0 + pix % rc.w;
+    row = rc.y0 + (rc.band_count > 1 ? ((vrow / rc.band_rows) * rc.band_count + rc.band_index) * rc.band_rows + vrow % rc.band_rows : vrow);
+}
+
 struct GlobalCounters {
     unsigned long long tlas_nodes, blas_nodes, instances, instance_hits, triangles, tri_shading, spheres, quads, cuboids, disks, rays, hits;
 };
diff --git a/pbrs_amd/csrc/device/raygen.h b/pbrs_amd/csrc/device/raygen.h
--- a/pbrs_amd/csrc/device/raygen.h
+++ b/pbrs_amd/csrc/device/raygen.h
@@ -6,9 +6,8 @@
     if (slot >= rc.n_slots) return;
     uint32_t k, pix;
     sample_of_slot(slot, rc.n_pixels, rc.n_slots / rc.n_pixels, rc.chunk_pixels, k, pix);
-    pix = pixel_of_order(pix, rc.w, rc.tiles8_per_row);
-    uint32_t col = rc.x0 + pix % rc.w, vrow = pix / rc.w;
-    uint32_t row = rc.y0 + (rc.band_count > 1 ? ((vrow / rc.band_rows) * rc.band_count + rc.band_index) * rc.band_rows + vrow % rc.band_rows : vrow);
+    uint32_t col, row;
+    film_pixel_of_order(rc, pix, col, row);
     uint32_t i = rc.pass_first_sample + k;
     uint64_t rng = pn_rng_init(rc.seed, row * rc.cam.width + col, i);
     float r0 = pn_rng_f32(&rng), r1 = pn_rng_f32(&rng);
@@ -17,8 +16,44 @@
     if (rc.integrator >= PBRS_INTEGRATOR_MATERIALS) jx = jy = 0.0f;
     float x = (float)col + pn_fract(jx);
     float y = (float)row + pn_fract(jy);
-    f3 dir = ld3(rc.cam.c) + ld3(rc.cam.a) * x + ld3(rc.cam.b) * y;
+    float dv[3];
+    pbrs_camera_dir(rc.cam, x, y, dv);
+    const f3 dir = ld3(dv);
     st_stream(&st.q[0][0][slot], pack4(ld3(rc.cam.center), slot));
     st_stream(&st.q[0][1][slot], pack4(dir, (uint32_t)rng));
     __builtin_nontemporal_store((uint32_t)(rng >> 32), &rng_hi0[slot]);
 }
+
+__global__ void __launch_bounds__(256) k_entry_nodes(DevScene S, RenderConst rc, uint32_t height, uint32_t rows, uint4* table, uint32_t* info) {
+    const uint32_t q = blockIdx.x * blockDim.x + threadIdx.x;
+    const bool valid = q < rc.n_pixels;
+    uint32_t n = PBRS_ENTRY_ROOT;
+    if (valid) {
+        uint32_t col, row;
+        film_pixel_of_order(rc, q, col, row);
+        const pbrs_instance& in = S.inst[S.entry_inst];
+        f3 o = ld3(rc.cam.center);
+        if (!((in.flags & PBRS_INSTANCE_IDENTITY) && o.x != 0.0f && o.y != 0.0f && o.z != 0.0f)) o = xf_apply(in.inv, o, 1.0f);
+        const float ov[3] = {o.x, o.y, o.z};
+        pbrs_dir_box B;
+        pbrs_entry_record rec;
+        if (pbrs_entry_dir_box(rc.cam, col, row, B) && pbrs_en_origin_in_range(o.x) && pbrs_en_origin_in_range(o.y) && pbrs_en_origin_in_range(o.z)) {
+            n = pbrs_entry_record_of(S.nodes, in.blas_root, ov, B, PBRS_ENTRY_FORKS, height, rows, rec);
+        } else {
+            for (uint32_t i = 0; i < PBRS_ENTRY_MAX; ++i) rec.e[i] = PBRS_ENTRY_UNUSED;
+            rec.e[0] = PBRS_ENTRY_ROOT;
+        }
+        table[2u * q] = make_uint4(rec.e[0], rec.e[1], rec.e[2], rec.e[3]);
+        table[2u * q + 1u] = make_uint4(rec.e[4], rec.e[5], rec.e[6], rec.e[7]);
+    }
+    const uint32_t with = (uint32_t)__popcll(__ballot(valid && n != PBRS_ENTRY_ROOT && n != 0u)), empty = (uint32_t)__popcll(__ballot(valid && n == 0u)),
+                   none = (uint32_t)__popcll(__ballot(valid && n == PBRS_ENTRY_ROOT));
+    uint32_t sum = (valid && n != PBRS_ENTRY_ROOT) ? n : 0u;
+    for (int off = 32; off > 0; off >>= 1) sum += __shfl_down(sum, off, 64);
+    if ((threadIdx.x & 63u) == 0u) {
+        if (with) atomicAdd(info + 0, with);
+        if (empty) atomicAdd(info + 1, empty);
+        if (none) atomicAdd(info + 2, none);
+        if (sum) atomicAdd(info + 3, sum);
+    }
+}
diff --git a/pbrs_amd/csrc/device/scene.h b/pbrs_amd/csrc/device/scene.h
--- a/pbrs_amd/csrc/device/scene.h
+++ b/pbrs_amd/csrc/device/scene.h
@@ -28,6 +28,7 @@
     uint32_t features;
     uint32_t refill_below;
     uint32_t refill_below_shadow;
+    uint32_t entry_inst;
     const pbrs_texture* textures;
     const float* tex_floats;
     const uint32_t* tex_words;
diff --git a/pbrs_amd/csrc/device/traverse.h b/pbrs_amd/csrc/device/traverse.h
--- a/pbrs_amd/csrc/device/traverse.h
+++ b/pbrs_amd/csrc/device/traverse.h
@@ -1,5 +1,5 @@
 #pragma once
-#include "shapes.h"
+#include "path_state.h"
 
 #include "probes.h"
 
@@ -217,8 +217,16 @@
     PD static uint32_t run_filter(const DevScene& S, bool fresh, const RaySpace& R, uint32_t& tested) { return scan<Filter>(S, fresh, R, pn_inf(), tested); }
 };
 
-template <bool STATS, uint32_t FEAT>
-struct ClosestWalk {
+template <bool ENTRY>
+struct EntryView {};
+template <>
+struct EntryView<true> {
+    EntryArgs a;
+};
+
+template <bool STATS, uint32_t FEAT, bool ENTRY = false>
+struct ClosestWalk : EntryView<ENTRY> {
+    static_assert(!ENTRY || (!STATS && !(FEAT & (PBRS_FEAT_EXTENT | PBRS_FEAT_LDS_TOP))), "the entry variant: a walk that carries the split-plane cull");
     RaySpace C;
     Hit best;
     float t_max, lt, mt, mb1, mb2;
@@ -463,6 +471,25 @@
         mt = pn_inf();
         if (kind == PBRS_SHAPE_MESH) {
             inst_info = kind | (H.mesh_flags << 3) | (space == PBRS_SPACE_TRANSLATED ? 0x40000000u : 0u);
+            if constexpr (ENTRY) {
+                if (cur_inst == S.entry_inst && C.fast && space != PBRS_SPACE_MOVED) {
+                    uint32_t k, pix;
+                    sample_of_slot(stk.item, this->a.n_pixels, this->a.k_count, this->a.chunk, k, pix);
+                    const uint4 e0 = this->a.table[2u * pix], e1 = this->a.table[2u * pix + 1u];
+                    if (e0.x != PBRS_ENTRY_ROOT) {
+                        if (slab_rs(walk_node<FEAT>(S, H.blas_root), C, lt)) {
+                            const uint32_t e[PBRS_ENTRY_MAX] = {e0.x, e0.y, e0.z, e0.w, e1.x, e1.y, e1.z, e1.w};
+#pragma unroll
+                            for (int i = (int)PBRS_ENTRY_MAX - 1; i >= 0; --i) {
+                                stk.put(sp, e[i]);
+                                sp += e[i] != PBRS_ENTRY_UNUSED ? 1 : 0;
+                            }
+                            lt = mt;
+                        }
+                        return;
+                    }
+                }
+            }
             stk.put(sp++, H.blas_root);
         } else if (kind == PBRS_SHAPE_TRIANGLE) {
             inst_info = kind | (PBRS_MESH_SHADING_OK_MASK << 3);
diff --git a/pbrs_amd/csrc/host/kernel_choice.cpp b/pbrs_amd/csrc/host/kernel_choice.cpp
--- a/pbrs_amd/csrc/host/kernel_choice.cpp
+++ b/pbrs_amd/csrc/host/kernel_choice.cpp
@@ -22,6 +22,7 @@
         p.extend[0] = {(f.features & PBRS_FEAT_ALL) | steps | p.lds_staging, staged};
         p.extend[1] = {kStatsKey | PBRS_FEAT_ALL, stack};
     }
+    p.entry_extend = f.entry_nodes && extend_entry_ok(p.extend[0].key);
     const uint32_t shadow_feat = (f.features & PBRS_FEAT_ANALYTIC) | (f.tlas_scanned ? PBRS_FEAT_FLAT_TLAS : 0u) | steps;
     if (p.wide_shadow) {
         p.shadow[0] = {shadow_feat | PBRS_FEAT_WIDE, f.wide_stack_bytes};
diff --git a/pbrs_amd/csrc/host/kernel_choice.h b/pbrs_amd/csrc/host/kernel_choice.h
--- a/pbrs_amd/csrc/host/kernel_choice.h
+++ b/pbrs_amd/csrc/host/kernel_choice.h
@@ -31,6 +31,7 @@
     bool exact_extent = false;
     bool long_walks = false;
     bool full_steps = false;
+    bool entry_nodes = false;
     bool wide_ok = false;
     size_t stack_bytes = 0;
     size_t wide_stack_bytes = 0;
@@ -61,6 +62,16 @@
     if ((f & PBRS_FEAT_LDS_TOP) && (f & (PBRS_FEAT_LDS_SCENE | PBRS_FEAT_FULL_STEPS | PBRS_FEAT_FLAT_TLAS))) return false;
     return true;
 }
+constexpr uint32_t kEntryKeysLosingAWave[] = {PBRS_FEAT_LONG_WALKS | PBRS_FEAT_ANALYTIC, PBRS_FEAT_LONG_WALKS | PBRS_FEAT_SHADING_CHECK | PBRS_FEAT_FLAT_TLAS};
+constexpr bool extend_entry_ok(uint32_t k) {
+    for (uint32_t lost : kEntryKeysLosingAWave)
+        if (k == lost) return false;
+    return k < kTraversalKeys && extend_key_ok(k) &&
+           !(k & (kStatsKey | PBRS_FEAT_EXTENT | PBRS_FEAT_LDS_TOP | PBRS_FEAT_LDS_SCENE | PBRS_FEAT_FULL_STEPS)) && (k & PBRS_FEAT_LONG_WALKS);
+}
+static_assert(extend_entry_ok(13u) && !extend_entry_ok(9u) && !extend_entry_ok(14u) && !extend_entry_ok(45u), "the entry variants' keys");
+constexpr uint32_t kExtendKeys = 2u * kTraversalKeys;
+constexpr uint32_t entry_key(uint32_t k) { return kTraversalKeys + k; }
 constexpr bool shadow_key_ok(uint32_t k) {
     const uint32_t f = k & ~kStatsKey;
     if (k & kStatsKey) return f == kShadowStatsFeatures;
@@ -122,6 +133,7 @@
     TraversalKey shadow[2];
     bool wide_shadow = false;
     TraversalKey shadow_slow;
+    bool entry_extend = false;
     bool split_queue = false;
     uint32_t lds_staging = 0;
     IntegratorChoice integ[PBRS_INTEGRATOR_NORMALS + 1];
diff --git a/pbrs_amd/csrc/host/scene_prepare.cpp b/pbrs_amd/csrc/host/scene_prepare.cpp
--- a/pbrs_amd/csrc/host/scene_prepare.cpp
+++ b/pbrs_amd/csrc/host/scene_prepare.cpp
@@ -7,6 +7,7 @@
 
 #include "../../../include/pbrs_numeric.h"
 #include "../../../include/pbrs_scene_spec.h"
+#include "../device/entry_nodes.h"
 #include "../device/split_planes.h"
 
 namespace pbrs {
@@ -103,6 +104,23 @@
     if (!coord_ok(pbrs_plane_down(qd, step, lo))) qd = 0u;
     if (!coord_ok(pbrs_plane_up(qu, step, hi))) qu = 0u;
     return pbrs_plane_pack(qd, qu);
+}
+
+bool blas_nested(const std::vector<pbrs_node>& nodes, uint32_t root) {
+    std::vector<uint32_t> todo = {root};
+    while (!todo.empty()) {
+        const uint32_t x = todo.back();
+        todo.pop_back();
+        const pbrs_node& X = nodes[x];
+        if (X.b & PBRS_LEAF_FLAG) continue;
+        for (uint32_t c : {x + 1u, X.a}) {
+            const pbrs_node& C = nodes[c];
+            for (int a = 0; a < 3; ++a)
+                if (!(X.min[a] <= C.min[a] && C.min[a] <= C.max[a] && C.max[a] <= X.max[a])) return false;
+            todo.push_back(c);
+        }
+    }
+    return true;
 }
 
 bool is_light_instance(const pbrs_scene_desc& d, const pbrs_area_light& L, const pbrs_instance& in) {
@@ -336,6 +354,21 @@
             S.features |= PBRS_FEAT_ANALYTIC;
         }
     }
+    S.entry_inst = PBRS_ENTRY_NONE;
+    if (S.fast_slab != 0u && !lv.exact_extent) {
+        std::vector<uint32_t> h;
+        tree_heights(nodes.data(), (uint32_t)nodes.size(), h);
+        uint32_t best = PBRS_ENTRY_NONE;
+        for (uint32_t i = 0; i < d.n_instances; ++i)
+            if (inst[i].shape_kind == PBRS_SHAPE_MESH && (best == PBRS_ENTRY_NONE || h[inst[i].blas_root] > h[inst[best].blas_root])) best = i;
+        if (best != PBRS_ENTRY_NONE && h[inst[best].blas_root] >= PBRS_LONG_WALK_HEIGHT && (inst[best].flags & PBRS_INSTANCE_TRANSLATION) &&
+            blas_nested(nodes, inst[best].blas_root)) {
+            S.entry_inst = best;
+            P.entry_height = h[inst[best].blas_root];
+            P.entry_rows = lv.stack - (lv.tlas - 1u);
+        }
+    }
+    f.entry_nodes = S.entry_inst != PBRS_ENTRY_NONE;
     f.features = S.features;
     f.exact_extent = lv.exact_extent;
     f.n_classes = S.n_classes;
diff --git a/pbrs_amd/csrc/host/scene_prepare.h b/pbrs_amd/csrc/host/scene_prepare.h
--- a/pbrs_amd/csrc/host/scene_prepare.h
+++ b/pbrs_amd/csrc/host/scene_prepare.h
@@ -31,6 +31,7 @@
     uint32_t wide_levels = 0;
     SceneFacts facts;
     uint32_t stack_depth = 0;
+    uint32_t entry_height = 0, entry_rows = 0;
     bool has_vis_records = false;
     uint64_t walk_bytes = 0;
 };
diff --git a/pbrs_amd/csrc/kernel_tables.h b/pbrs_amd/csrc/kernel_tables.h
--- a/pbrs_amd/csrc/kernel_tables.h
+++ b/pbrs_amd/csrc/kernel_tables.h
@@ -8,6 +8,7 @@
 namespace pbrs {
 
 typedef void (*extend_fn_t)(DevScene, PathState, uint32_t, const uint32_t*, uint32_t, uint32_t*, GlobalCounters*, const uint32_t*, uint32_t*, uint32_t*, uint32_t);
+typedef void (*extend_entry_fn_t)(DevScene, PathState, uint32_t, const uint32_t*, uint32_t, uint32_t*, GlobalCounters*, const uint32_t*, uint32_t*, uint32_t*, uint32_t, EntryArgs);
 typedef void (*shadow_fn_t)(DevScene, PathState, const uint32_t*, uint32_t*, GlobalCounters*, const uint32_t*, uint32_t*, uint32_t*);
 typedef void (*shade_fn_t)(DevScene, PathState, RenderConst, uint32_t, const uint32_t*, uint32_t, uint32_t*, uint32_t*, unsigned long long*, uint32_t, const uint2*,
                            const uint32_t*);
diff --git a/pbrs_amd/csrc/pbrs_gpu.hip b/pbrs_amd/csrc/pbrs_gpu.hip
--- a/pbrs_amd/csrc/pbrs_gpu.hip
+++ b/pbrs_amd/csrc/pbrs_gpu.hip
@@ -88,6 +88,7 @@
 struct KernelPlan {
     KernelChoice choice;
     extend_fn_t extend[2] = {};
+    extend_entry_fn_t extend_entry = nullptr;
     shadow_fn_t shadow[2] = {};
     shadow_fn_t shadow_slow = nullptr;
     IntegratorPlan integ[PBRS_INTEGRATOR_NORMALS + 1];
@@ -103,6 +104,7 @@
 };
 enum BufferId {
     BUF_AOV_STATE, BUF_AOV_OUT,
+    BUF_ENTRY_TABLE,
     BUF_FILTER_SUM,
     BUF_DENOISE, BUF_DENOISE_VAR, BUF_DENOISE_STAGE, BUF_DENOISE_VAR_STAGE,
     BUF_MOMENT_STATE, BUF_VARIANCE_OUT,
@@ -151,6 +153,11 @@
     int cur_set = 0;
     hipStream_t main_stream = nullptr;
     hipStream_t second_stream = nullptr;
+    bool entry_nodes = true;
+    uint32_t entry_height = 0, entry_rows = 0;
+    const uint4* entry_table = nullptr;
+    bool last_entry = false;
+    uint32_t last_entry_pixels = 0;
     bool overlap_passes = true;
     uint32_t overlap_from = 2;
     size_t cap_pixels = 0;
@@ -487,7 +494,8 @@
         p.shadow[s] = shadow_fns()[ch.shadow[s].key];
     }
     if (ch.wide_shadow) p.shadow_slow = shadow_fns()[ch.shadow_slow.key];
-    bool ok = p.extend[0] && p.extend[1] && p.shadow[0] && p.shadow[1] && (!ch.wide_shadow || p.shadow_slow);
+    if (ch.entry_extend) p.extend_entry = reinterpret_cast<extend_entry_fn_t>(extend_fns()[entry_key(ch.extend[0].key)]);
+    bool ok = p.extend[0] && p.extend[1] && p.shadow[0] && p.shadow[1] && (!ch.wide_shadow || p.shadow_slow) && (!ch.entry_extend || p.extend_entry);
     for (uint32_t i = 0; i <= PBRS_INTEGRATOR_NORMALS; ++i) {
         IntegratorPlan& ip = p.integ[i];
         ip.choice = ch.integ[i];
@@ -557,8 +565,12 @@
         const BouncePlan bp = bounce_plan(rc.integrator, choice.split_queue, ip.choice, c->split_decision, b);
         const uint32_t qsplit = bp.split;
         if (tm.begin(1)) return fail(c, PBRS_E_DEVICE, "event record failed");
-        hipLaunchKernelGGL(plan.extend[stats], dim3(pgrid), dim3(kBlock), xk.lds, c->stream, xS, set.st, b & 1u, cnt_in, N, xhead + b * kHeadWords, c->gcnt, nullptr,
-                           nullptr, nullptr, qsplit);
+        if (b == 0 && c->entry_table && !stats)
+            hipLaunchKernelGGL(plan.extend_entry, dim3(pgrid), dim3(kBlock), xk.lds, c->stream, xS, set.st, b & 1u, cnt_in, N, xhead + b * kHeadWords, c->gcnt, nullptr,
+                               nullptr, nullptr, qsplit, EntryArgs{c->entry_table, P, kc, rc.chunk_pixels});
+        else
+            hipLaunchKernelGGL(plan.extend[stats], dim3(pgrid), dim3(kBlock), xk.lds, c->stream, xS, set.st, b & 1u, cnt_in, N, xhead + b * kHeadWords, c->gcnt, nullptr,
+                               nullptr, nullptr, qsplit);
         c->pending.kernel_features_extend = reported_features(xk);
         tm.end();
         if (b == 0 && t.want_aovs())
@@ -653,6 +665,22 @@
     if (moments) HIPCHK(c, hipMemsetAsync(moments, 0, PBRS_MOMENT_STATE_WORDS * (size_t)P * sizeof(float), c->stream));
     if (matte) HIPCHK(c, hipMemsetAsync(matte, 0, PBRS_MATTE_STATE_WORDS(t.matte->slots) * (size_t)P * sizeof(uint32_t), c->stream));
     if (pass_state) HIPCHK(c, hipMemsetAsync(pass_state, 0, PBRS_PASS_STATE_WORDS * (size_t)P * sizeof(float), c->stream));
+    c->entry_table = nullptr;
+    c->last_entry = false;
+    if (c->entry_nodes && c->plan.extend_entry && !stats && bounce_count(rc.integrator, rc.max_depth) > 0) {
+        DeviceBuffer& eb = c->buf[BUF_ENTRY_TABLE];
+        const size_t table_bytes = (size_t)P * sizeof(pbrs_entry_record);
+        if (eb.grow(c, table_bytes + 4 * sizeof(uint32_t), "the entry-node table") == PBRS_OK) {
+            uint32_t* info = reinterpret_cast<uint32_t*>(static_cast<char*>(eb.p) + table_bytes);
+            HIPCHK(c, hipMemsetAsync(info, 0, 4 * sizeof(uint32_t), c->stream));
+            hipLaunchKernelGGL(k_entry_nodes, dim3((P + kBlock - 1) / kBlock), dim3(kBlock), 0, c->stream, c->S, rc, c->entry_height, c->entry_rows, eb.as<uint4>(), info);
+            c->entry_table = eb.as<uint4>();
+            c->last_entry = true;
+            c->last_entry_pixels = P;
+        } else {
+            c->error.clear();
+        }
+    }
     uint32_t passes = 0;
     bool two = c->overlap_passes && !stats && spp > K;
     if (two && (ensure_work(c, c->pass_set[1], (size_t)P * K, P) || ensure_direct(c, 1, (size_t)P * K, pass_state != nullptr))) {
@@ -665,10 +693,12 @@
         const int rcode = run_pass(c, rc, first, kc, stats, tm, two, t);
         if (rcode) {
             use_pass_set(c, 0);
+            c->entry_table = nullptr;
             return rcode;
         }
         ++passes;
     }
+    c->entry_table = nullptr;
     if (two) {
         const hipEvent_t last = cur(c).accumulated;
         use_pass_set(c, 0);
@@ -745,8 +775,9 @@
     if (c->device < 64 && g_kernel_cfg_done[c->device]) return PBRS_OK;
     const int cap = (int)(kLdsBytesPerCU / 2);
     std::vector<const void*> traversal_kernels = {reinterpret_cast<const void*>(intersect_fn(false)), reinterpret_cast<const void*>(intersect_fn(true))};
+    for (uint32_t k = 0; k < kExtendKeys; ++k)
+        if (extend_fns()[k]) traversal_kernels.push_back(reinterpret_cast<const void*>(extend_fns()[k]));
     for (uint32_t k = 0; k < kTraversalKeys; ++k) {
-        if (extend_fns()[k]) traversal_kernels.push_back(reinterpret_cast<const void*>(extend_fns()[k]));
         if (shadow_fns()[k]) traversal_kernels.push_back(reinterpret_cast<const void*>(shadow_fns()[k]));
     }
     for (const void* k : traversal_kernels) HIPCHK(c, hipFuncSetAttribute(k, hipFuncAttributeMaxDynamicSharedMemorySize, cap));
@@ -936,6 +967,24 @@
 int pbrs_set_pass_overlap(pbrs_ctx* c, int enabled) {
     if (!c) return PBRS_E_INVALID;
     c->overlap_passes = enabled != 0;
+    return PBRS_OK;
+}
+
+int pbrse_set_entry_nodes(pbrs_ctx* c, int enabled) {
+    if (!c) return PBRS_E_INVALID;
+    c->entry_nodes = enabled != 0;
+    return PBRS_OK;
+}
+
+int pbrse_last_entry_info(pbrs_ctx* c, pbrs_entry_info* out) {
+    if (!c || !out) return PBRS_E_INVALID;
+    *out = pbrs_entry_info{};
+    if (!c->last_entry) return PBRS_OK;
+    HIPCHK(c, hipSetDevice(c->device));
+    HIPCHK(c, hipStreamSynchronize(c->main_stream));
+    uint32_t v[4];
+    HIPCHK(c, hipMemcpy(v, static_cast<const char*>(c->buf[BUF_ENTRY_TABLE].p) + (size_t)c->last_entry_pixels * sizeof(pbrs_entry_record), sizeof v, hipMemcpyDeviceToHost));
+    *out = pbrs_entry_info{v[0], v[1], v[2], v[3]};
     return PBRS_OK;
 }
 
@@ -989,6 +1038,10 @@
     c->material_flags.resize(d->n_materials);
     for (uint32_t i = 0; i < d->n_materials; ++i) c->material_flags[i] = d->materials[i].flags;
     c->stack_depth = P.stack_depth;
+    c->entry_height = P.entry_height;
+    c->entry_rows = P.entry_rows;
+    c->entry_table = nullptr;
+    c->last_entry = false;
     c->has_scene = true;
     c->split_decision = 0;
     c->split_probe_in_flight = false;
@@ -2052,6 +2105,7 @@
     k.tiles8_per_row = 0u;
     Timer tm{c, false};
     HIPCHK(c, hipMemsetAsync(c->sum, 0, 3 * (size_t)P * sizeof(float), c->stream));
+    c->entry_table = nullptr;
     rc = run_pass(c, k, sample_index, 1, false, tm, false, RenderTargets{});
     if (rc) return rc;
     hipLaunchKernelGGL(k_export_radiance, dim3((P + kBlock - 1) / kBlock), dim3(kBlock), 0, c->stream, cur(c).st, P, c->rgb_dev);
diff --git a/pbrs_amd/csrc/traverse.hip b/pbrs_amd/csrc/traverse.hip
--- a/pbrs_amd/csrc/traverse.hip
+++ b/pbrs_amd/csrc/traverse.hip
@@ -20,8 +20,11 @@
 namespace {
 
 template <uint32_t K>
-constexpr extend_fn_t extend_fn_of() {
-    if constexpr (extend_key_ok(K)) return &k_extend<(K & kStatsKey) != 0u, (K & ~kStatsKey)>;
+extend_fn_t extend_fn_of() {
+    if constexpr (K >= kTraversalKeys) {
+        if constexpr (extend_entry_ok(K - kTraversalKeys)) return reinterpret_cast<extend_fn_t>(static_cast<extend_entry_fn_t>(&k_extend<false, K - kTraversalKeys, EntryArgs>));
+        else return nullptr;
+    } else if constexpr (extend_key_ok(K)) return &k_extend<(K & kStatsKey) != 0u, (K & ~kStatsKey)>;
     else return nullptr;
 }
 template <uint32_t K>
@@ -44,7 +47,7 @@
 
 namespace pbrs {
 
-const extend_fn_t* extend_fns() { return extend_table(std::make_integer_sequence<uint32_t, kTraversalKeys>{}); }
+const extend_fn_t* extend_fns() { return extend_table(std::make_integer_sequence<uint32_t, kExtendKeys>{}); }
 const shadow_fn_t* shadow_fns() { return shadow_table(std::make_integer_sequence<uint32_t, kTraversalKeys>{}); }
 intersect_fn_t intersect_fn(bool wide_any) { return wide_any ? &k_intersect_rays<true> : &k_intersect_rays<false>; }
 
diff --git a/pbrs_amd/libs.py b/pbrs_amd/libs.py
--- a/pbrs_amd/libs.py
+++ b/pbrs_amd/libs.py
@@ -80,6 +80,10 @@
 }, with_device={
     "pbrsm_motion_blur": [P] * 7,
 })
+GPU_ENTRY_FUNCTIONS = _table({
+    "pbrse_set_entry_nodes": [P, INT],
+    "pbrse_last_entry_info": [P, P],
+})
 HOST_FUNCTIONS = _table({
     "pbrs_host_scene_build": [P, C.POINTER(P)],
     "pbrs_host_scene_free": [P],
@@ -103,6 +107,7 @@
 GPU_BLOOM_SYMBOLS = list(GPU_BLOOM_FUNCTIONS)
 GPU_DOF_SYMBOLS = list(GPU_DOF_FUNCTIONS)
 GPU_MOTION_BLUR_SYMBOLS = list(GPU_MOTION_BLUR_FUNCTIONS)
+GPU_ENTRY_SYMBOLS = list(GPU_ENTRY_FUNCTIONS)
 _host = _gpu = _hip = None
 
 
@@ -135,7 +140,7 @@
         if not os.path.exists(path):
             raise PbrsError(f"{path} is missing: the HIP extension must be built (make -C pbrs_amd/csrc); there is no CPU fallback")
         _gpu = _load(path, {**GPU_FUNCTIONS, **GPU_COMPARE_FUNCTIONS, **GPU_DESPECKLE_FUNCTIONS, **GPU_BLOOM_FUNCTIONS, **GPU_DOF_FUNCTIONS,
-                            **GPU_MOTION_BLUR_FUNCTIONS})
+                            **GPU_MOTION_BLUR_FUNCTIONS, **GPU_ENTRY_FUNCTIONS})
     return _gpu
 
 
```

Measured after the change: 1801 (median of 6 runs). 3.4% higher.
